# renegade-fi/mpc-jellyfish

Measured on AMD Instinct MI355X. Metric: msm_g1_scalar_pairs_per_s, higher is better.
Workload: dtype u32 (381-bit Fq as 14 x 29-bit limbs, Montgomery)

## Files before the change

### include/mzk.h

```cpp
#ifndef MZK_H
#define MZK_H

#include <stdint.h>

#ifdef __cplusplus
extern "C" {
#endif

#if defined(__GNUC__)
#define MZK_API __attribute__((visibility("default")))
#else
#define MZK_API
#endif

#define MZK_OK 0
#define MZK_ERR_INVALID_ARG (-1)
#define MZK_ERR_HIP (-2)
#define MZK_ERR_NO_DEVICE (-3)
#define MZK_ERR_BAD_HANDLE (-4)
#define MZK_ERR_UNSUPPORTED (-5)
#define MZK_ERR_OOM (-6)
#define MZK_ERR_NOT_INIT (-7)
#define MZK_ERR_LOOKUP (-8)

// ... 176 lines not shown
MZK_API int32_t mzk_plonk_perm_product_dev(uint64_t pk_handle, const void* d_wire_values, const uint64_t* beta_mont,
                                           const uint64_t* gamma_mont, void* d_out, void* stream);
MZK_API int32_t mzk_plonk_perm_product(uint64_t pk_handle, const uint64_t* wire_values, const uint64_t* beta_mont,
                                       const uint64_t* gamma_mont, uint64_t* out);

MZK_API int32_t mzk_plonk_gather_witness_dev(const void* d_witness, uint64_t n_vars, const void* d_wire_variables, uint64_t count, void* d_out,
                                             void* stream);

MZK_API int32_t mzk_poly_eval_dev(int32_t curve_id, const void* d_coeffs, uint64_t len, uint32_t batch, uint64_t batch_stride,
                                  const uint64_t* x_mont, uint64_t* out_mont, void* stream);
MZK_API int32_t mzk_poly_eval_many_dev(int32_t curve_id, uint32_t n_jobs, const void* const* d_coeffs, const uint64_t* lens, const uint32_t* batches,
                                       const uint64_t* strides, const uint32_t* which_x, const uint64_t* x_mont, uint64_t* out_mont, void* stream);
MZK_API int32_t mzk_poly_lincomb_dev(int32_t curve_id, uint32_t n_terms, const void* const* d_polys, const uint64_t* lens,
                                     const uint64_t* scalars_mont, void* d_out, uint64_t out_len, void* stream);
MZK_API int32_t mzk_poly_mask_dev(int32_t curve_id, uint32_t n_polys, void* const* d_polys, uint64_t n, uint32_t n_blinders,
                                  const uint64_t* blinders_mont, void* stream);
MZK_API int32_t mzk_poly_split_quotient_dev(int32_t curve_id, const void* d_quot, uint64_t n, uint32_t n_parts, const uint64_t* blinders_mont,
                                            void* d_out, uint64_t out_stride, void* stream);
MZK_API int32_t mzk_poly_div_linear_dev(int32_t curve_id, const void* d_poly, uint64_t len, const uint64_t* z_mont, void* d_out, void* stream);
MZK_API int32_t mzk_poly_div_linear_rem_dev(int32_t curve_id, const void* d_poly, uint64_t len, const uint64_t* z_mont, void* d_out, void* d_rem,
                                            void* stream);
MZK_API int32_t mzk_poly_degree_dev(const void* d_poly, uint64_t len, uint64_t* d_out_len, void* stream);
MZK_API int32_t mzk_poly_div_roots_dev(int32_t curve_id, const void* d_poly, uint64_t len, uint32_t log_order, uint64_t first, uint64_t count,
                                       void* d_out, void* stream);
MZK_API int32_t mzk_kzg_open_batch_dev(uint64_t srs_handle, uint32_t K, const void* const* d_polys, const uint64_t* lens, const uint64_t* points_mont,
                                       uint64_t* out_proofs_xy_mont, uint64_t* out_evals_mont, void* stream);
MZK_API int32_t mzk_kzg_multi_open_rou_dev(uint64_t srs_handle, uint64_t srs_offset, const void* d_poly, uint64_t len, uint32_t log_domain,
                                           uint64_t num_points, uint64_t* out_proofs_xy_mont, uint64_t* out_evals_mont, void* stream);

MZK_API int32_t mzk_sha256(const uint8_t* msg, uint64_t len, uint8_t* out32);
MZK_API int32_t mzk_expand_message_xmd_sha256(const uint8_t* msg, uint64_t len, const uint8_t* dst, uint64_t dst_len, uint32_t z_pad_len, uint8_t* out,
                                              uint64_t out_len);
MZK_API int32_t mzk_hash_to_field_sha256(int32_t curve_id, const uint8_t* msg, uint64_t len, const uint8_t* dst, uint64_t dst_len, uint64_t* out_mont);
MZK_API int32_t mzk_bytes_to_field_dev(int32_t curve_id, const void* d_bytes, uint64_t len, void* d_out_mont, void* stream);
MZK_API int32_t mzk_field_to_bytes_dev(int32_t curve_id, const void* d_elems_mont, uint64_t count, void* d_out_bytes, uint64_t* out_len, void* stream);
MZK_API int32_t mzk_vid_advz_commit_only_dev(uint64_t srs_handle, uint64_t srs_offset, uint64_t srs_len, const void* d_elems_mont, uint64_t n_elems,
                                             uint32_t payload_chunk_size, uint32_t num_storage_nodes, uint32_t log_domain, uint8_t* out_commit32, void* stream);
MZK_API int32_t mzk_vid_advz_disperse_dev(uint64_t srs_handle, uint64_t srs_offset, uint64_t srs_len, const void* d_elems_mont, uint64_t n_elems,
                                          uint32_t payload_chunk_size, uint32_t num_storage_nodes, uint32_t log_domain, uint64_t* out_commits_xy_mont,
                                          uint8_t* out_evals, uint64_t* out_proofs_xy_mont, uint8_t* out_nodes, uint8_t* out_commit32, uint8_t* out_root32,
                                          uint64_t* out_scalar_mont, void* stream);
MZK_API int32_t mzk_vid_advz_verify_shares_dev(int32_t curve_id, uint64_t n_shares, uint64_t evals_per_share, uint32_t num_storage_nodes, const uint64_t* indices,
                                               const uint8_t* evals, const uint8_t* paths, const uint8_t* root32, const uint64_t* scalar_mont, int32_t* out_ok,
                                               uint64_t* out_agg_evals_mont, void* stream);
MZK_API int32_t mzk_vid_advz_recover_dev(int32_t curve_id, uint32_t payload_chunk_size, uint64_t n_polys, uint32_t log_domain, const uint64_t* indices,
                                         const uint64_t* evals_mont, void* d_out_mont, void* stream);

#define MZK_ERR_WRONG_QUOTIENT_DEGREE (-9)
#define MZK_ERR_STATE (-10)
#define MZK_ERR_ENCODING (-11)

typedef struct mzk_comm {
    void* ctx;
    int32_t rank, world;
    int32_t (*all_gather)(void* ctx, const void* send, uint64_t bytes, void* recv);
    int32_t (*barrier)(void* ctx);
    int32_t (*exchange_classes)(void* ctx, void* d_rem, uint64_t class_bytes, uint32_t first_own, uint32_t n_own, uint32_t n_classes);
} mzk_comm;

MZK_API int32_t mzk_prover_create(int32_t curve_id, uint32_t log_n, uint32_t num_wire_types, const uint64_t* selector_coeffs,
                                  const uint64_t* sigma_coeffs, const uint64_t* table_coeffs, uint64_t poly_len, const uint64_t* k_mont,
                                  uint64_t commit_key, uint64_t lagrange_key, const mzk_comm* comm, uint64_t* out_prover);
MZK_API int32_t mzk_prover_create_from_circuit(int32_t curve_id, uint32_t log_n, uint32_t num_wire_types, const uint64_t* selector_values,
                                               const uint32_t* wire_variables, uint64_t n_vars, const uint64_t* table_values, const uint64_t* k_mont,
                                               uint64_t commit_key, uint64_t lagrange_key, const mzk_comm* comm, uint64_t* out_prover);
MZK_API int32_t mzk_prover_create_from_circuit_dev(int32_t curve_id, uint32_t log_n, uint32_t num_wire_types, const void* d_selector_values,
                                                   const void* d_wire_variables, uint64_t n_vars, const void* d_table_values, const uint64_t* k_mont,
                                                   uint64_t commit_key, uint64_t lagrange_key, const mzk_comm* comm, uint64_t* out_prover);
MZK_API int32_t mzk_prover_create_serialized(int32_t curve_id, const uint8_t* bytes, uint64_t len, uint32_t flags, uint64_t commit_key, const mzk_comm* comm,
                                             uint64_t* out_prover, uint64_t* out_commit_key, uint64_t* out_lagrange_key, uint64_t* out_bad);
MZK_API int32_t mzk_prover_serialize_key(uint64_t prover, uint32_t flags, uint64_t num_inputs, const uint8_t* h_bytes, const uint8_t* beta_h_bytes,
                                         int32_t is_merged, uint8_t* out_bytes, uint64_t capacity, uint64_t* out_len);
MZK_API int32_t mzk_prover_serialize_vk(uint64_t prover, uint32_t flags, uint64_t num_inputs, const uint8_t* h_bytes, const uint8_t* beta_h_bytes,
                                        int32_t is_merged, uint8_t* out_bytes, uint64_t capacity, uint64_t* out_len);
MZK_API int32_t mzk_prover_destroy(uint64_t prover);
MZK_API int32_t mzk_prover_fork(uint64_t prover, uint64_t* out_prover);
MZK_API int32_t mzk_prover_vk_commitments(uint64_t prover, uint64_t* out_xy_mont, uint64_t* out_plookup_xy_mont);
MZK_API int32_t mzk_prover_set_wire_variables(uint64_t prover, const uint32_t* wire_variables, uint64_t n_vars);
MZK_API int32_t mzk_prover_derive_wire_variables(uint64_t prover, uint64_t* out_n_vars);
MZK_API int32_t mzk_prover_get_wire_variables(uint64_t prover, uint32_t* out_wire_variables, uint64_t capacity_cells, uint64_t* out_n_vars);
#define MZK_WITNESS_DEV_WIRES 0
#define MZK_WITNESS_HOST_WIRES 1
#define MZK_WITNESS_HOST_VECTOR 2
#define MZK_WITNESS_DEV_VECTOR 3
MZK_API int32_t mzk_prover_round1(uint64_t prover, int32_t witness_kind, const void* witness, uint64_t witness_len, const uint64_t* pub_input_rows,
                                  const uint64_t* pub_input_mont, uint64_t n_pub, const uint64_t* blinders_mont, uint64_t* out_comms_xy);
#define MZK_CHECK_SATISFIED 0
#define MZK_CHECK_GATE 1
#define MZK_CHECK_LOOKUP 2
#define MZK_CHECK_COPY 3
typedef struct mzk_witness_report {
    uint32_t kind;
    uint32_t copy_checked;
    uint64_t gate_failures, gate_row;
    uint64_t lookup_failures, lookup_row;
    uint64_t copy_failures, copy_cell, copy_rep_cell;
    uint64_t row_wires[6 * 4];
    uint64_t gate_residual[4];
} mzk_witness_report;
MZK_API int32_t mzk_prover_check_witness(uint64_t prover, int32_t witness_kind, const void* witness, uint64_t witness_len,
                                         const uint64_t* pub_input_rows, const uint64_t* pub_input_mont, uint64_t n_pub,
                                         mzk_witness_report* out_report);
MZK_API int32_t mzk_prover_round1_5(uint64_t prover, const uint64_t* tau_mont, const uint64_t* blinders_mont, uint64_t* out_comms_xy);
MZK_API int32_t mzk_prover_round2(uint64_t prover, const uint64_t* beta_mont, const uint64_t* gamma_mont, const uint64_t* blinders_mont,
                                  uint64_t* out_comm_xy);
MZK_API int32_t mzk_prover_round2_5(uint64_t prover, const uint64_t* blinders_mont, uint64_t* out_comm_xy);
MZK_API int32_t mzk_prover_round3(const uint64_t* provers, uint32_t n_instances, const uint64_t* alpha_mont, const uint64_t* blinders_mont,
                                  uint64_t* out_comms_xy);
MZK_API int32_t mzk_prover_round4(uint64_t prover, const uint64_t* zeta_mont, uint64_t* out_evals_mont);
MZK_API int32_t mzk_prover_round5(const uint64_t* provers, uint32_t n_instances, const uint64_t* v_mont, uint64_t* out_comms_xy);
MZK_API int32_t mzk_prover_exchange_buffer(uint64_t prover, void** out_dptr, uint64_t* out_bytes);
MZK_API int32_t mzk_prover_set_peer_buffers(uint64_t prover, void* const* peer_dptrs, const int32_t* peer_devices);
MZK_API int32_t mzk_prover_poly_dev(uint64_t prover, uint32_t which, const void** out_dptr, uint64_t* out_len);
MZK_API int32_t mzk_prover_profile(uint64_t prover, int32_t on);
MZK_API int32_t mzk_prover_timings(uint64_t prover, char* buf, uint64_t cap);
MZK_API int32_t mzk_prover_hbm_bytes(uint64_t prover, uint64_t* out_fixed, uint64_t* out_proving_key, uint64_t* out_workspace);
MZK_API int32_t mzk_prover_shared_hbm_bytes(uint64_t prover, uint64_t* out_shared_bytes, uint32_t* out_sharers);

MZK_API int32_t mzk_host_alloc(uint64_t bytes, void** out_ptr);
MZK_API int32_t mzk_host_free(void* ptr);
MZK_API int32_t mzk_host_register(void* ptr, uint64_t bytes);
MZK_API int32_t mzk_host_unregister(void* ptr);

MZK_API int32_t mzk_dev_alloc(uint64_t bytes, void** out_dptr);
MZK_API int32_t mzk_dev_free(void* dptr);
MZK_API int32_t mzk_dev_upload(void* dptr, const void* host, uint64_t bytes);
MZK_API int32_t mzk_dev_download(void* host, const void* dptr, uint64_t bytes);
MZK_API int32_t mzk_dev_sync(void);
MZK_API int32_t mzk_stream_create(void** out_stream);
MZK_API int32_t mzk_stream_destroy(void* stream);
MZK_API int32_t mzk_stream_sync(void* stream);
MZK_API int32_t mzk_stream_wait_stream(void* waiter, void* signaller);
MZK_API int32_t mzk_dev_upload_async(void* dptr, const void* host, uint64_t bytes, void* stream);
MZK_API int32_t mzk_dev_download_async(void* host, const void* dptr, uint64_t bytes, void* stream);
MZK_API int32_t mzk_dev_copy(void* dst, const void* src, uint64_t bytes, void* stream);
MZK_API int32_t mzk_dev_copy_peer(void* dst, int32_t dst_device, const void* src, int32_t src_device, uint64_t bytes, void* stream);
MZK_API int32_t mzk_dev_copy2d(void* dst, uint64_t dst_pitch, const void* src, uint64_t src_pitch, uint64_t width, uint64_t height, void* stream);
MZK_API int32_t mzk_dev_memset(void* dptr, int32_t value, uint64_t bytes, void* stream);
MZK_API int32_t mzk_dev_memset2d(void* dptr, uint64_t pitch, int32_t value, uint64_t width, uint64_t height, void* stream);

MZK_API int32_t mzk_profile_enable(int32_t on);
MZK_API int32_t mzk_profile_get(const char* name, double* out_ms, uint64_t* out_count);
MZK_API int32_t mzk_profile_reset(void);
MZK_API int32_t mzk_msm_set_precompute(int32_t on);
MZK_API int32_t mzk_srs_precompute(uint64_t srs_handle, uint32_t* out_window_bits, uint32_t* out_levels, uint64_t* out_table_bytes,
                                   double* out_build_ms);
MZK_API int32_t mzk_srs_hbm_bytes(uint64_t srs_handle, uint64_t* out_points_bytes, uint64_t* out_table_bytes);
MZK_API int32_t mzk_plonk_pk_hbm_bytes(uint64_t pk_handle, uint64_t* out_bytes);
MZK_API int32_t mzk_workspace_hbm_bytes(uint64_t* out_bytes);
MZK_API int32_t mzk_workspace_release(void);
MZK_API int32_t mzk_launch_count(uint64_t* out_launches);
MZK_API int32_t mzk_msm_last_shape(uint32_t* out_window_bits, uint32_t* out_windows, uint32_t* out_buckets);
MZK_API int32_t mzk_msm_last_rare(uint32_t* out_cap, uint32_t* out_desc_cap, uint32_t* out_h1_cap, uint32_t* out_attempts);

#ifdef __cplusplus
}
#endif
#endif
```

### mpc-jellyfish_amd/csrc/internal.hpp

```cpp
#pragma once
#include <cstdlib>
#include <hip/hip_runtime.h>

#include <atomic>
#include <condition_variable>
#include <cstdint>
#include <cstring>
#include <map>
#include <mutex>
#include <string>
#include <vector>

#include "../../include/mzk.h"

extern "C" int32_t mzk_ctx_prover_stream(uint32_t k, void** out_stream);
namespace mzk { struct WitnessCheckIn; }
extern "C" int32_t mzk_ctx_pk_register_chunked(int32_t curve_id, uint32_t log_n, uint32_t num_wire_types, const void* selector_coeffs, const void* sigma_coeffs,
                                               const void* table_coeffs, uint64_t poly_len, const uint64_t* k_mont, const uint32_t* classes, uint32_t n_classes,
                                               int32_t coeffs_on_device, uint64_t* out_handle);
extern "C" int32_t mzk_ctx_check_witness(uint64_t pk_handle, const mzk::WitnessCheckIn* in, mzk_witness_report* out_report, void* stream);
extern "C" int32_t mzk_ctx_derive_variables(uint64_t pk_handle, const void* d_sigma_coeffs, void* d_out_variables_u32, uint64_t* out_n_vars, void* stream);
extern "C" int32_t mzk_ctx_g1_encode(int32_t curve_id, const uint64_t* xy_mont, uint64_t n_points, uint32_t flags, uint8_t* out_bytes);

namespace mzk {

void set_error(const std::string& s);

int32_t hip_status(hipError_t e, const char* what);

#define HIP_TRY(expr)                                      \
    do {                                                   \
        int32_t _r = ::mzk::hip_status((expr), #expr);     \
        if (_r != MZK_OK) return _r;                       \
    } while (0)

#define MZK_TRY(expr)                \
    do {                             \
        int32_t _r = (expr);         \
        if (_r != MZK_OK) return _r; \
    } while (0)

struct DevBuf {
    void* p = nullptr;
    size_t cap = 0;
    int32_t reserve(size_t bytes);
    void release();
    template <class T> T* as() { return reinterpret_cast<T*>(p); }
};
struct DevOwned {
    void* p = nullptr;
    DevOwned() = default;
    DevOwned(DevOwned&& o) noexcept : p(o.p) { o.p = nullptr; }
    DevOwned& operator=(DevOwned&&) = delete;
    ~DevOwned() { if (p) (void)hipFree(p); }
    int32_t alloc(size_t bytes) { return hip_status(hipMalloc(&p, bytes ? bytes : 4), "hipMalloc"); }
    template <class T> T* as() const { return reinterpret_cast<T*>(p); }
};

struct Workspace {
    DevBuf ntt_scratch, scalars, hist, offs, cursor, sorted, buckets, collect, io, misc, digits, long_desc, long_parts, plonk_polys, plonk_out, pre_cnt, pre_off, pre_ce, pre_cb, poly_tmp, split, link_tmp, occ, vid;
    void* h_collect = nullptr;
    size_t h_collect_cap = 0;
    double heavy_frac = 0.125;
    hipEvent_t last_use = nullptr;
    struct Named { const char* name; DevBuf Workspace::* buf; };
    static const Named bufs[];
    void release();
    size_t bytes();
};

extern std::atomic<uint64_t> g_launches;
#undef hipLaunchKernelGGL
#define hipLaunchKernelGGL(kernelName, ...)                                  \
    do {                                                                     \
        ::mzk::g_launches.fetch_add(1, std::memory_order_relaxed);           \
        hipLaunchKernelGGLInternal((kernelName), __VA_ARGS__);               \
    } while (0)

extern std::atomic<bool> g_prof;
struct ProfRec { std::string name; hipEvent_t a, b; };
struct ProfScope {
    hipEvent_t a = nullptr, b = nullptr;
    hipStream_t st;
    const char* name;
    int logical = -1;
    ProfScope(const char* n, hipStream_t s);
    ProfScope(const char* n, hipStream_t s, int logical_device);
    ~ProfScope();
};
extern std::atomic<bool> g_msm_precompute;

struct Srs {
    int curve = 0;
    uint64_t n = 0;
    uint32_t* d_xy = nullptr;
    uint32_t* d_int = nullptr;
    uint32_t* d_pre = nullptr;
    int pre_c = 0;
    int pre_levels = 0;
    double pre_build_ms = 0;
    uint32_t* d_fk = nullptr;
    uint64_t fk_off = 0, fk_d = 0;
    void free();
};
inline bool valid_curve(int curve) { return curve == MZK_CURVE_BLS12_381 || curve == MZK_CURVE_BN254; }
inline int fq_words(int curve) { return curve == MZK_CURVE_BLS12_381 ? 12 : 8; }
inline size_t srs_point_bytes(int curve) { return (size_t)2 * fq_words(curve) * 4; }
constexpr size_t srs_int_point_bytes(int curve) { return curve == MZK_CURVE_BLS12_381 ? 2 * 14 * 4 : 2 * 9 * 4; }
constexpr size_t ec_ntt_point_bytes(int curve) { return curve == MZK_CURVE_BLS12_381 ? 4 * 14 * 4 : 4 * 9 * 4; }

constexpr int MAX_CTX = 16;
constexpr int IO_SLOTS = 4;
struct IoSlot {
    hipStream_t st = nullptr;
    DevBuf buf;
    bool busy = false;
};
struct Ctx {
    int logical = -1, device = -1;
    std::atomic<bool> init{false};
    std::mutex lock;
    Workspace ws;
    std::vector<ProfRec> prof_recs;
    uint32_t last_c = 0, last_w = 0, last_m = 0;
    uint32_t last_cap = 0, last_desc_cap = 0, last_h1_cap = 0, last_attempts = 0;
    std::map<uint64_t, Srs> srs;
    uint64_t next_handle = 1;
    IoSlot io[IO_SLOTS];
    std::mutex io_lock;
    std::condition_variable io_cv;
};
Ctx& cur();
int32_t ws_acquire(Workspace& ws, hipStream_t st);
void ws_release(Workspace& ws, hipStream_t st);
class WsHold {
    Workspace* ws_ = nullptr;
    hipStream_t st_ = nullptr;
   public:
    WsHold() = default;
    WsHold(const WsHold&) = delete;
    WsHold& operator=(const WsHold&) = delete;
    ~WsHold() { if (ws_) ws_release(*ws_, st_); }
    int32_t acquire(hipStream_t st) {
        Ctx& cx = cur();
        MZK_TRY(ws_acquire(cx.ws, st));
        ws_ = &cx.ws, st_ = st;
        return MZK_OK;
    }
    Workspace* operator->() const { return ws_; }
    Workspace& operator*() const { return *ws_; }
};
inline uint64_t handle_make(int logical, uint64_t counter) { return ((uint64_t)(logical + 1) << 48) | counter; }
inline int handle_ctx(uint64_t h) { return (int)(h >> 48) - 1; }
struct DeviceGuard {
    int32_t prev = -1, rc = MZK_OK;
    bool switched = false;
    explicit DeviceGuard(int device) {
        if (mzk_get_device(&prev) != MZK_OK) prev = -1;
        if (prev != device) { rc = mzk_set_device(device); switched = rc == MZK_OK && prev >= 0; }
    }
    DeviceGuard(const DeviceGuard&) = delete;
    DeviceGuard& operator=(const DeviceGuard&) = delete;
    ~DeviceGuard() { if (switched) (void)mzk_set_device(prev); }
};

int32_t ntt_dispatch(int curve, uint32_t* d_data, uint64_t in_len, int log_n, bool inverse, const uint32_t* coset,
                     uint32_t batch, uint64_t stride, hipStream_t st, int scale = 0, const uint32_t* d_src = nullptr, uint64_t src_stride = 0,
                     const uint32_t* d_patch = nullptr, int skip_batch = -1 );
int32_t ntt_classes_dispatch(int curve, uint32_t* d_data, uint64_t in_len, int log_n, bool inverse, const uint32_t* const* cosets, int n_classes, uint32_t rows,
                             uint64_t stride, hipStream_t st, int scale, const uint32_t* d_src, uint64_t src_stride, const uint32_t* d_patch, int skip_batch);
void ntt_release_plans();
void msm_release_streams();
int32_t ctx_prover_stream(unsigned k, hipStream_t* out);
int32_t msm_dispatch(const Srs& s, uint64_t base_offset, const uint32_t* d_scalars, uint64_t n, int is_mont, uint32_t* out, hipStream_t st);
int32_t msm_batch_dispatch(const Srs& s, uint32_t n_polys, const uint32_t* const* d_scalars, const uint64_t* lens, const uint64_t* base_offsets,
                           int is_mont, uint32_t* out_xyz, hipStream_t st);
int32_t srs_build_internal(Srs& s, hipStream_t st);
int32_t srs_build_pre(Srs& s, hipStream_t st);
int32_t srs_generate_dispatch(int curve, const uint32_t* beta_canon, const uint32_t* g_xy_mont , uint64_t n, uint32_t* d_out);
int32_t srs_lagrange_from_points_dispatch(int curve, const uint32_t* d_xy, int log_n, uint32_t n_extra, uint32_t* d_out);
int32_t ec_ntt_dispatch(int curve, uint32_t* d_a, int log_n, bool inverse, bool scaled, uint32_t* d_tab, uint32_t* d_out_xy, uint64_t n_out, hipStream_t st);
int32_t srs_lagrange_generate_dispatch(int curve, const uint32_t* beta_canon, const uint32_t* g_xy_mont , int log_n, uint32_t n_extra, uint32_t* d_out);
void jac_to_affine_host_dispatch(int curve, const uint64_t* xyz, uint64_t n, uint64_t* xy);
void jac_sum_host_dispatch(int curve, const uint64_t* xyz, uint64_t n, uint64_t* out);

uint64_t srs_record_bytes(int curve, bool compressed);
const char* srs_bad_reason(int k);
int32_t srs_decode_dispatch(int curve, const uint8_t* d_in, uint64_t n, bool compressed, bool validate, uint32_t* d_xy, uint64_t* out_bad, int* out_reason,
                            hipStream_t st);
int32_t srs_encode_dispatch(int curve, const uint32_t* d_xy, uint64_t n, bool compressed, uint8_t* d_out, hipStream_t st);

int32_t fr_decode_dispatch(int curve, const uint8_t* d_image, uint32_t n_seg, const uint64_t* src, const uint64_t* count, const uint32_t* row, uint32_t* d_out,
                           uint64_t row_len, uint32_t* out_bad_seg, uint64_t* out_bad_index, hipStream_t st);
int32_t fr_encode_dispatch(int curve, const uint32_t* d_in, uint64_t n, uint32_t* d_out, hipStream_t st);

int32_t poly_eval_dispatch(int curve, const uint32_t* d_coeffs, uint64_t stride, uint64_t len, uint32_t batch, const uint32_t* x_mont, uint32_t* out_host,
                           hipStream_t st);
struct EvalJob { const uint32_t* d; uint64_t len, stride; uint32_t batch, which_x; };
int32_t poly_eval_many_dispatch(int curve, const EvalJob* jobs, uint32_t n_jobs, const uint32_t* x_mont , uint32_t* out_host, hipStream_t st);
int32_t poly_div_dispatch(int curve, const uint32_t* d_poly, uint64_t len, const uint32_t* z_mont, uint32_t* d_out, uint32_t* d_rem , hipStream_t st);
int32_t kzg_open_batch_dispatch(const Srs& s, uint32_t K, const uint32_t* const* d_polys, const uint64_t* lens, const uint32_t* points_mont, uint64_t* out_xy,
                                uint32_t* out_evals, hipStream_t st);
int32_t poly_div_roots_dispatch(int curve, const uint32_t* d_poly, uint64_t len, uint32_t log_order, uint64_t first, uint64_t count, uint32_t* d_out,
                                hipStream_t st);
constexpr int KZG_MULTI_MAX_LOG = 21;
int32_t kzg_multi_open_dispatch(Srs& s, uint64_t srs_offset, const uint32_t* d_poly, uint64_t len, uint32_t log_domain, uint64_t num_points, uint64_t* out_xy,
                                uint32_t* out_evals, hipStream_t st);
uint64_t vid_field_count(uint64_t len);
int32_t vid_bytes_to_field_dispatch(int curve, const uint8_t* d_bytes, uint64_t len, uint32_t* d_out, hipStream_t st);
int32_t vid_field_to_bytes_dispatch(int curve, const uint32_t* d_elems, uint64_t count, uint8_t* d_out, uint64_t* out_len, hipStream_t st);
int32_t vid_commit_only_dispatch(Srs& s, uint64_t srs_offset, uint64_t srs_len, const uint32_t* d_elems, uint64_t n_elems, uint32_t k, uint32_t n, uint32_t log_domain,
                                 uint8_t* out_commit, hipStream_t st);
int32_t vid_disperse_dispatch(Srs& s, uint64_t srs_offset, uint64_t srs_len, const uint32_t* d_elems, uint64_t n_elems, uint32_t k, uint32_t n, uint32_t log_domain,
                              uint64_t* out_commits_xy, uint8_t* out_evals, uint64_t* out_proofs_xy, uint8_t* out_nodes, uint8_t* out_commit, uint8_t* out_root,
                              uint64_t* out_s_mont, hipStream_t st);
int32_t vid_verify_shares_dispatch(int curve, uint64_t S, uint64_t K, uint32_t n, const uint64_t* index, const uint8_t* evals, const uint8_t* paths, const uint8_t* root,
                                   const uint64_t* s_mont, int32_t* out_ok, uint64_t* out_agg_mont, hipStream_t st);
int32_t vid_recover_dispatch(int curve, uint32_t k, uint64_t K, uint32_t log_domain, const uint64_t* index, const uint64_t* y_mont, uint32_t* d_out, hipStream_t st);
int32_t poly_lincomb_dispatch(int curve, uint32_t n_terms, const uint32_t* const* d_polys, const uint64_t* lens, const uint32_t* scalars, uint32_t* d_out,
                              uint64_t out_len, hipStream_t st);
int32_t poly_degree_dispatch(const uint32_t* d_poly, uint64_t len, unsigned long long* d_out, hipStream_t st);
int32_t wire_gather_dispatch(const uint32_t* d_witness, uint64_t n_vars, const uint32_t* d_vars, uint64_t count, uint32_t* d_out, hipStream_t st);
int32_t poly_split_quotient_dispatch(int curve, const uint32_t* d_q, uint64_t n, uint32_t W, const uint32_t* blind_mont, uint32_t* d_out, uint64_t stride, hipStream_t st);
int32_t poly_mask_dispatch(int curve, uint32_t n_rows, uint32_t* const* d_rows, uint64_t n, uint32_t n_blind, const uint32_t* blind_mont, hipStream_t st);
int32_t plonk_pk_register(int curve, int log_n, int W, const uint32_t* sel, const uint32_t* sig, const uint32_t* tab ,
                          uint64_t poly_len, const uint32_t* k_mont, const uint32_t* classes , uint32_t n_classes,
                          uint64_t* out_handle, bool coeffs_on_device = false );
int32_t plonk_wire_permutation_dev(const uint32_t* d_vars, uint64_t cells, uint64_t n_vars, uint32_t* d_next, hipStream_t st);
int32_t plonk_sigma_values_dev(int curve, int log_n, int W, const uint32_t* d_next, const uint32_t* k_mont, uint32_t* d_out, hipStream_t st);
int32_t plonk_sigma_decode_dev(int curve, int log_n, int W, const uint32_t* d_sigma, const uint32_t* k_mont, uint32_t* d_next, hipStream_t st);
int32_t plonk_variables_from_permutation_dev(const uint32_t* d_next, uint64_t cells, uint32_t* d_vars, uint64_t* out_n_vars, hipStream_t st);
int32_t plonk_derive_variables_dev(uint64_t handle, const uint32_t* d_sigma_coeffs, uint32_t* d_vars, uint64_t* out_n_vars, hipStream_t st);
int32_t plonk_quotient_chunked_dev(uint64_t handle, const uint32_t* d_polys, uint64_t in_stride, uint64_t in_len, uint32_t flags, const uint32_t* tau,
                                   const uint32_t* alpha, const uint32_t* beta, const uint32_t* gamma, uint32_t* d_out, hipStream_t st);
int32_t plonk_quotient_top_dev(uint64_t handle, const uint32_t* d_polys, uint64_t in_stride, uint64_t in_len, const uint32_t* alpha, const uint32_t* beta,
                               const uint32_t* gamma, uint32_t* d_top, uint32_t* out_n_top, hipStream_t st);
int32_t plonk_quotient_combine_dev(int curve, int log_n, const uint32_t* classes , uint32_t n_classes, const uint32_t* d_r,
                                   const uint32_t* d_top , uint32_t n_top, uint32_t* d_out, hipStream_t st);
int32_t plonk_pk_release(uint64_t handle);
void plonk_release_all();
void verifier_release_all();
int32_t plonk_quotient_dev(uint64_t handle, uint32_t* d_polys, uint64_t in_len, const uint32_t* tau , const uint32_t* alpha,
                           const uint32_t* beta, const uint32_t* gamma, uint32_t* d_out, hipStream_t st);
int32_t plookup_sorted_vec_dev(uint64_t handle, const uint32_t* d_wires, const uint32_t* tau, uint32_t* d_table, uint32_t* d_lookup, uint32_t* d_sorted,
                               hipStream_t st);
int32_t plookup_product_dev(uint64_t handle, const uint32_t* d_table, const uint32_t* d_lookup, const uint32_t* d_sorted, const uint32_t* beta,
                            const uint32_t* gamma, uint32_t* d_out, hipStream_t st);
struct WitnessCheckIn {
    const uint32_t* d_sel_coeffs;
    int kind;
    const void* witness;
    const uint32_t* d_vars;
    uint64_t n_vars;
    const uint64_t *pi_rows, *pi;
    uint64_t n_pi;
};
int32_t plonk_check_witness_dev(uint64_t handle, const WitnessCheckIn& in, mzk_witness_report* out, hipStream_t st);
int plonk_pk_is_ultra(uint64_t handle);
int32_t plonk_perm_product_dev(uint64_t handle, const uint32_t* d_wires, const uint32_t* beta, const uint32_t* gamma, uint32_t* d_out, hipStream_t st);
int plonk_pk_log_n(uint64_t handle);
int plonk_pk_curve(uint64_t handle);
int plonk_pk_classes(uint64_t handle, uint32_t* out);
int plonk_pk_wires(uint64_t handle);
uint64_t plonk_pk_bytes(uint64_t handle);

}
```

### mpc-jellyfish_amd/csrc/msm.cuh

```cuda
#pragma once
#include <hip/hip_runtime.h>

#include "ec.cuh"
#include "ecx.cuh"
#include "ecz.cuh"
#include "ec_ntt.cuh"

namespace mzk {

constexpr int MSM_THREADS = 256;
constexpr int MSM_ACC_THREADS = 128;
constexpr uint32_t MSM_HEAVY_PER_THREAD = 16;
constexpr uint32_t MSM_HEAVY_RUN = MSM_ACC_THREADS * MSM_HEAVY_PER_THREAD;
constexpr uint32_t MSM_HEAVY_FANIN = MSM_ACC_THREADS * 32;
constexpr int MSM_HEAVY_COUNTERS = 6;
__host__ __device__ inline bool msm_is_heavy(uint32_t count, uint32_t cap) { return count > cap + MSM_HEAVY_RUN; }

inline int msm_choose_window(unsigned long long n) {
    int lg = 0;
    while ((1ull << (lg + 1)) <= n) lg++;
    int c = lg - 2;
    if (c < 4) c = 4;
    if (c > 16) c = 16;
    return c;
}
inline int msm_num_windows(int scalar_bits, int c) { return (scalar_bits + 1 + c - 1) / c; }

struct DigitIter {
    uint32_t k[8];
    uint32_t carry;
    __device__ __forceinline__ void next(int w, int c, uint32_t& mag, uint32_t& negative) {
        const int off = w * c, word = off >> 5, bit = off & 31;
        uint32_t buf = 0;
        if (word < 8) {
            uint64_t two = k[word];
            if (word + 1 < 8) two |= (uint64_t)k[word + 1] << 32;
            buf = (uint32_t)(two >> bit);
        }
        uint32_t coef = (buf & ((1u << c) - 1)) + carry;
        carry = coef > (1u << (c - 1)) ? 1u : 0u;
        negative = carry;
        mag = carry ? (1u << c) - coef : coef;
    }
};

template <class FR>
__device__ __forceinline__ void load_scalar(DigitIter& it, const uint32_t* __restrict__ scalars, unsigned long long i, int is_mont) {
    Fp<FR> s = load_fp<FR>(scalars + i * 8);
    if (is_mont) s = from_mont(s);
#pragma unroll
    for (int q = 0; q < 8; q++) it.k[q] = s.l[q];
    it.carry = 0;
}

constexpr uint32_t MSM_EMPTY = 0xFFFFu;
constexpr int MSM_RANGE_LOG = 11;
constexpr int MSM_SORT_THREADS = 1024;

template <class FR>
__global__ __launch_bounds__(MSM_THREADS) void msm_digits_kernel(const uint32_t* __restrict__ scalars, unsigned long long n, int is_mont,
                                                                  int c, int n_win, uint16_t* __restrict__ digits, unsigned long long stride) {
    const unsigned long long i = (unsigned long long)blockIdx.x * MSM_THREADS + threadIdx.x;
    if (i >= n) return;
    DigitIter it;
    load_scalar<FR>(it, scalars, i, is_mont);
    for (int w = 0; w < n_win; w++) {
        uint32_t mag, ng;
        it.next(w, c, mag, ng);
        digits[(size_t)w * stride + i] = (uint16_t)(mag ? ((ng << 15) | (mag - 1)) : MSM_EMPTY);
    }
}

template <bool SCATTER>
__global__ __launch_bounds__(MSM_SORT_THREADS) void msm_sort_kernel(const uint16_t* __restrict__ digits, unsigned long long n, unsigned long long stride, uint32_t M,
                                                                     uint32_t* __restrict__ hist, const uint32_t* __restrict__ offs,
                                                                     uint32_t* __restrict__ sorted) {
    __shared__ uint32_t bins[1 << MSM_RANGE_LOG];
    const uint32_t range = blockIdx.x, w = blockIdx.y, tid = threadIdx.x;
    const uint32_t rsize = M < (1u << MSM_RANGE_LOG) ? M : (1u << MSM_RANGE_LOG);
    const uint32_t rbase = range * rsize;
    for (uint32_t j = tid; j < rsize; j += MSM_SORT_THREADS) bins[j] = SCATTER ? offs[(size_t)w * M + rbase + j] : 0u;
    __syncthreads();
    const uint16_t* dw = digits + (size_t)w * stride;
    uint32_t* out = sorted + (size_t)w * n;
    const unsigned long long n8 = n >> 3;
    for (unsigned long long q = tid; q < n8; q += MSM_SORT_THREADS) {
        const uint4 v = reinterpret_cast<const uint4*>(dw)[q];
        const uint32_t wd[4] = {v.x, v.y, v.z, v.w};
#pragma unroll
        for (int k = 0; k < 8; k++) {
            const uint32_t d = (wd[k >> 1] >> ((k & 1) * 16)) & 0xFFFFu;
            const uint32_t b = d & 0x7FFFu;
            if (d != MSM_EMPTY && b - rbase < rsize) {
                if (SCATTER) out[atomicAdd(&bins[b - rbase], 1u)] = (uint32_t)(q * 8 + k) | ((d >> 15) << 31);
                else atomicAdd(&bins[b - rbase], 1u);
            }
        }
    }
    for (unsigned long long i = (n8 << 3) + tid; i < n; i += MSM_SORT_THREADS) {
        const uint32_t d = dw[i], b = d & 0x7FFFu;
        if (d != MSM_EMPTY && b - rbase < rsize) {
            if (SCATTER) out[atomicAdd(&bins[b - rbase], 1u)] = (uint32_t)i | ((d >> 15) << 31);
            else atomicAdd(&bins[b - rbase], 1u);
        }
    }
    if (!SCATTER) {
        __syncthreads();
        for (uint32_t j = tid; j < rsize; j += MSM_SORT_THREADS) hist[(size_t)w * M + rbase + j] = bins[j];
    }
}

__global__ __launch_bounds__(1024) void msm_scan_kernel(const uint32_t* __restrict__ hist, uint32_t* __restrict__ offs, uint32_t M) {
    __shared__ uint32_t part[1024];
    const int w = blockIdx.x, t = threadIdx.x;
    const uint32_t per = (M + 1023) / 1024;
    const uint32_t lo = t * per, hi = min(M, lo + per);
    uint32_t sum = 0;
    for (uint32_t b = lo; b < hi; b++) sum += hist[(size_t)w * M + b];
    part[t] = sum;
    __syncthreads();
    for (int d = 1; d < 1024; d <<= 1) {
        uint32_t v = t >= d ? part[t - d] : 0;
        __syncthreads();
        part[t] += v;
        __syncthreads();
    }
    uint32_t run = part[t] - sum;
    for (uint32_t b = lo; b < hi; b++) {
        offs[(size_t)w * M + b] = run;
        run += hist[(size_t)w * M + b];
    }
}

constexpr uint32_t MSM_ORDER_SLICE = 8192;
__device__ __forceinline__ uint32_t order_key(uint32_t count) { return 1023u - min(count, 1023u); }

__global__ __launch_bounds__(1024) void msm_order_hist_kernel(const uint32_t* __restrict__ hist, uint32_t M, uint32_t* __restrict__ keycnt) {
    __shared__ uint32_t cnt[1024];
    const uint32_t w = blockIdx.y, t = threadIdx.x;
    const uint32_t lo = blockIdx.x * MSM_ORDER_SLICE, hi = min(M, lo + MSM_ORDER_SLICE);
    cnt[t] = 0;
    __syncthreads();
    for (uint32_t b = lo + t; b < hi; b += 1024) atomicAdd(&cnt[order_key(hist[(size_t)w * M + b])], 1u);
    __syncthreads();
    if (cnt[t]) atomicAdd(&keycnt[(size_t)w * 1024 + t], cnt[t]);
}
__global__ __launch_bounds__(1024) void msm_order_scan_kernel(uint32_t* __restrict__ keycnt, uint32_t global_sets) {
    __shared__ uint32_t part[1024];
    const uint32_t w = blockIdx.x, t = threadIdx.x;
    uint32_t mine = keycnt[(size_t)w * 1024 + t];
    for (uint32_t s = 1; s < global_sets; s++) mine += keycnt[(size_t)s * 1024 + t];
    part[t] = mine;
    __syncthreads();
    for (int d = 1; d < 1024; d <<= 1) {
        uint32_t v = t >= (uint32_t)d ? part[t - d] : 0;
        __syncthreads();
        part[t] += v;
        __syncthreads();
    }
    keycnt[(size_t)w * 1024 + t] = part[t] - mine;
}
__global__ __launch_bounds__(1024) void msm_order_scatter_kernel(const uint32_t* __restrict__ hist, uint32_t M, uint32_t* __restrict__ keycur,
                                                                 uint32_t* __restrict__ order, bool global) {
    __shared__ uint32_t cnt[1024];
    const uint32_t w = blockIdx.y, t = threadIdx.x;
    const uint32_t row = global ? 0u : w;
    const uint32_t lo = blockIdx.x * MSM_ORDER_SLICE, hi = min(M, lo + MSM_ORDER_SLICE);
    cnt[t] = 0;
    __syncthreads();
    for (uint32_t b = lo + t; b < hi; b += 1024) atomicAdd(&cnt[order_key(hist[(size_t)w * M + b])], 1u);
    __syncthreads();
    const uint32_t mine = cnt[t];
    __syncthreads();
    cnt[t] = mine ? atomicAdd(&keycur[(size_t)row * 1024 + t], mine) : 0u;
    __syncthreads();
    for (uint32_t b = lo + t; b < hi; b += 1024) {
        const uint32_t pos = atomicAdd(&cnt[order_key(hist[(size_t)w * M + b])], 1u);
        order[(size_t)row * M + pos] = w * M + b;
    }
}

struct LongDesc;
struct HeavyRun;
__device__ __forceinline__ void msm_long_register(uint32_t w, uint32_t b, uint32_t c, uint32_t offs_t, int n_win, uint32_t cap, uint32_t desc_cap,
                                                  LongDesc* __restrict__ desc, uint32_t* __restrict__ desc_count, uint32_t run_cap,
                                                  uint32_t h1_cap, HeavyRun* __restrict__ heavy_runs);
__global__ __launch_bounds__(1024) void msm_order_place_kernel(const uint32_t* __restrict__ hist, const uint32_t* __restrict__ offs, uint32_t M,
                                                               const uint32_t* __restrict__ keycnt, uint32_t* __restrict__ keycur, uint32_t* __restrict__ order,
                                                               int n_win, uint32_t cap, uint32_t desc_cap, LongDesc* __restrict__ desc,
                                                               uint32_t* __restrict__ desc_count, uint32_t run_cap, uint32_t h1_cap, HeavyRun* __restrict__ heavy_runs,
                                                               bool global) {
    __shared__ uint32_t cnt[1024];
    __shared__ uint32_t part[1024];
    const uint32_t w = blockIdx.y, t = threadIdx.x;
    const uint32_t row = global ? 0u : w;
    const uint32_t lo = blockIdx.x * MSM_ORDER_SLICE, hi = min(M, lo + MSM_ORDER_SLICE);
    uint32_t total = 0;
    if (global) for (uint32_t s = 0; s < gridDim.y; s++) total += keycnt[(size_t)s * 1024 + t];
    else total = keycnt[(size_t)w * 1024 + t];
    part[t] = total;
    cnt[t] = 0;
    __syncthreads();
    for (int d = 1; d < 1024; d <<= 1) {
        uint32_t v = t >= (uint32_t)d ? part[t - d] : 0;
        __syncthreads();
        part[t] += v;
        __syncthreads();
    }
    const uint32_t key_start = part[t] - total;
    for (uint32_t b = lo + t; b < hi; b += 1024) atomicAdd(&cnt[order_key(hist[(size_t)w * M + b])], 1u);
    __syncthreads();
    const uint32_t mine = cnt[t];
    __syncthreads();
    cnt[t] = mine ? key_start + atomicAdd(&keycur[(size_t)row * 1024 + t], mine) : 0u;
    __syncthreads();
    for (uint32_t b = lo + t; b < hi; b += 1024) {
        const uint32_t c = hist[(size_t)w * M + b];
        const uint32_t pos = atomicAdd(&cnt[order_key(c)], 1u);
        order[(size_t)row * M + pos] = w * M + b;
        if (desc_count && c > cap) msm_long_register(w, b, c, offs[(size_t)w * M + b], n_win, cap, desc_cap, desc, desc_count, run_cap, h1_cap, heavy_runs);
    }
}

template <class FQ>
__device__ __forceinline__ Affine<Fp<FQ>> load_affine(const uint32_t* __restrict__ bases, unsigned long long idx) {
    Affine<Fp<FQ>> p;
    const uint32_t* src = bases + idx * (2 * FQ::N);
    p.x = load_fp<FQ>(src);
    p.y = load_fp<FQ>(src + FQ::N);
    return p;
}
template <class FQ>
__device__ __forceinline__ XYZZ<Fp<FQ>> load_xyzz(const uint32_t* __restrict__ buf, unsigned long long idx) {
    XYZZ<Fp<FQ>> p;
    const uint32_t* src = buf + idx * (4 * FQ::N);
    p.x = load_fp<FQ>(src);
    p.y = load_fp<FQ>(src + FQ::N);
    p.zz = load_fp<FQ>(src + 2 * FQ::N);
    p.zzz = load_fp<FQ>(src + 3 * FQ::N);
    return p;
}
template <class FQ>
__device__ __forceinline__ void store_xyzz(uint32_t* __restrict__ buf, unsigned long long idx, const XYZZ<Fp<FQ>>& p) {
    uint32_t* dst = buf + idx * (4 * FQ::N);
    store_fp<FQ>(dst, p.x);
    store_fp<FQ>(dst + FQ::N, p.y);
    store_fp<FQ>(dst + 2 * FQ::N, p.zz);
    store_fp<FQ>(dst + 3 * FQ::N, p.zzz);
}

template <class FQ>
struct EcFp {
    using Field = FQ;
    using Aff = Affine<Fp<FQ>>;
    using Pt = XYZZ<Fp<FQ>>;
    static constexpr int AFF_WORDS = 2 * FQ::N, PT_WORDS = 4 * FQ::N;
    static __device__ __forceinline__ Aff load_aff(const uint32_t* __restrict__ bases, unsigned long long idx) { return load_affine<FQ>(bases, idx); }
    static __device__ __forceinline__ Pt load_pt(const uint32_t* __restrict__ buf, unsigned long long idx) { return load_xyzz<FQ>(buf, idx); }
    static __device__ __forceinline__ void store_pt(uint32_t* __restrict__ buf, unsigned long long idx, const Pt& p) { store_xyzz<FQ>(buf, idx, p); }
    static __device__ __forceinline__ Pt inf() { return Pt::inf(); }
    static __device__ __forceinline__ Pt madd(const Pt& a, Aff q, bool negate) {
        if (negate) q.y = neg(q.y);
        return xyzz_madd(a, q);
    }
    static __device__ __forceinline__ Pt add(const Pt& a, const Pt& b) { return xyzz_add(a, b); }
    static __device__ __forceinline__ XYZZ<Fp<FQ>> to_boundary(const Pt& p) { return p; }
};

template <class X>
__device__ __forceinline__ void load_words(uint32_t* dst, const uint32_t* __restrict__ src, int n_words) {
    for (int i = 0; i < n_words / 4; i++) {
        const uint4 v = reinterpret_cast<const uint4*>(src)[i];
        dst[4 * i] = v.x; dst[4 * i + 1] = v.y; dst[4 * i + 2] = v.z; dst[4 * i + 3] = v.w;
    }
}

template <class Z>
struct EcFz {
    using Field = Z;
    using Aff = AffineZ<Z>;
    using Pt = XYZZZ<Z>;
    using Fe = Fz<Z>;
    static constexpr int LIMBS = Z::ZN, SLOT_WORDS = Z::ZN + 1;
    static constexpr int AFF_WORDS = 2 * SLOT_WORDS, PT_WORDS = 4 * SLOT_WORDS;
    static_assert(AFF_WORDS % 4 == 0, "points are whole 16-byte words");
    static __device__ __forceinline__ Aff load_aff(const uint32_t* __restrict__ bases, unsigned long long idx) {
        uint32_t w[AFF_WORDS];
        const uint4* src = reinterpret_cast<const uint4*>(bases + idx * AFF_WORDS);
#pragma unroll
        for (int i = 0; i < AFF_WORDS / 4; i++) {
            const uint4 v = src[i];
            w[4 * i] = v.x; w[4 * i + 1] = v.y; w[4 * i + 2] = v.z; w[4 * i + 3] = v.w;
        }
        Aff p;
#pragma unroll
        for (int i = 0; i < LIMBS; i++) { p.x.l[i] = (int32_t)w[i]; p.y.l[i] = (int32_t)w[SLOT_WORDS + i]; }
        return p;
    }
    static __device__ __forceinline__ void store_aff(uint32_t* __restrict__ bases, unsigned long long idx, const Aff& p) {
        uint32_t w[AFF_WORDS];
#pragma unroll
        for (int i = 0; i < LIMBS; i++) { w[i] = (uint32_t)p.x.l[i]; w[SLOT_WORDS + i] = (uint32_t)p.y.l[i]; }
        w[LIMBS] = 0; w[SLOT_WORDS + LIMBS] = 0;
        uint4* dst = reinterpret_cast<uint4*>(bases + idx * AFF_WORDS);
#pragma unroll
        for (int i = 0; i < AFF_WORDS / 4; i++) dst[i] = make_uint4(w[4 * i], w[4 * i + 1], w[4 * i + 2], w[4 * i + 3]);
    }
    static __device__ __forceinline__ Pt load_pt(const uint32_t* __restrict__ buf, unsigned long long idx) {
        uint32_t w[PT_WORDS];
        const uint4* src = reinterpret_cast<const uint4*>(buf + idx * PT_WORDS);
#pragma unroll
        for (int i = 0; i < PT_WORDS / 4; i++) {
            const uint4 v = src[i];
            w[4 * i] = v.x; w[4 * i + 1] = v.y; w[4 * i + 2] = v.z; w[4 * i + 3] = v.w;
        }
        Pt p;
#pragma unroll
        for (int i = 0; i < LIMBS; i++) {
            p.x.l[i] = (int32_t)w[i]; p.y.l[i] = (int32_t)w[SLOT_WORDS + i];
            p.zz.l[i] = (int32_t)w[2 * SLOT_WORDS + i]; p.zzz.l[i] = (int32_t)w[3 * SLOT_WORDS + i];
        }
        return p;
    }
    static __device__ __forceinline__ void store_pt(uint32_t* __restrict__ buf, unsigned long long idx, const Pt& p) {
        uint32_t w[PT_WORDS];
#pragma unroll
        for (int i = 0; i < LIMBS; i++) {
            w[i] = (uint32_t)p.x.l[i]; w[SLOT_WORDS + i] = (uint32_t)p.y.l[i];
            w[2 * SLOT_WORDS + i] = (uint32_t)p.zz.l[i]; w[3 * SLOT_WORDS + i] = (uint32_t)p.zzz.l[i];
        }
#pragma unroll
        for (int k = 0; k < 4; k++) w[k * SLOT_WORDS + LIMBS] = 0;
        uint4* dst = reinterpret_cast<uint4*>(buf + idx * PT_WORDS);
#pragma unroll
        for (int i = 0; i < PT_WORDS / 4; i++) dst[i] = make_uint4(w[4 * i], w[4 * i + 1], w[4 * i + 2], w[4 * i + 3]);
    }
    static __device__ __forceinline__ Pt inf() { return Pt::inf(); }
    static __device__ __forceinline__ Pt madd(const Pt& a, const Aff& q, bool negate) { return xyzzz_madd(a, q, negate); }
    static __device__ __forceinline__ Pt add(const Pt& a, const Pt& b) { return xyzzz_add(a, b); }
    static __device__ __forceinline__ XYZZ<Fp<Z>> to_boundary(const Pt& p) { return xyzzz_to_boundary(p); }
    static __device__ __forceinline__ Fe add_quad(const Fe& ca, const Fe& cb, int role) { return xyzzz_add_quad<Z>(ca, cb, role); }
};

template <class Z>
__global__ __launch_bounds__(MSM_THREADS) void srs_to_internal_z_kernel(const uint32_t* __restrict__ xy, unsigned long long n, uint32_t* __restrict__ out) {
    const unsigned long long i = (unsigned long long)blockIdx.x * MSM_THREADS + threadIdx.x;
    if (i >= n) return;
    const Fp<Z> x = load_fp<Z>(xy + i * 2 * Z::N), y = load_fp<Z>(xy + i * 2 * Z::N + Z::N);
    AffineZ<Z> p;
    p.x = fz_from_boundary<Z>(x);
    p.y = fz_from_boundary<Z>(y);
    EcFz<Z>::store_aff(out, i, p);
}

template <class X>
__global__ __launch_bounds__(MSM_THREADS) void srs_to_internal_kernel(const uint32_t* __restrict__ xy, unsigned long long n, uint32_t* __restrict__ out) {
    const unsigned long long i = (unsigned long long)blockIdx.x * MSM_THREADS + threadIdx.x;
    if (i >= n) return;
    const Fp<X> x = load_fp<X>(xy + i * 2 * X::N), y = load_fp<X>(xy + i * 2 * X::N + X::N);
    const Fx<X> fx = fx_from_boundary<X>(x), fy = fx_from_boundary<X>(y);
    uint32_t* dst = out + i * 2 * X::XN;
#pragma unroll
    for (int k = 0; k < X::XN; k++) { dst[k] = fx.l[k]; dst[X::XN + k] = fy.l[k]; }
}

template <class EC>
__global__ __launch_bounds__(MSM_ACC_THREADS) void msm_accumulate_kernel(const uint32_t* __restrict__ bases, unsigned long long n,
                                                                          const uint32_t* __restrict__ offs, const uint32_t* __restrict__ hist,
                                                                          const uint32_t* __restrict__ sorted, const uint32_t* __restrict__ order,
                                                                          uint32_t M, int n_win, uint32_t cap, uint32_t* __restrict__ long_count,
                                                                          uint32_t* __restrict__ buckets, uint8_t* __restrict__ occ) {
    if (long_count && blockIdx.x == 0)
        for (unsigned i = threadIdx.x; i < (unsigned)n_win * (1 + MSM_HEAVY_COUNTERS); i += MSM_ACC_THREADS) long_count[i] = 0u;
    const unsigned long long t0 = (unsigned long long)blockIdx.x * MSM_ACC_THREADS + threadIdx.x;
    if (t0 >= (unsigned long long)n_win * M) return;
    const uint32_t tb = order[t0];
    const unsigned long long t = tb, w = tb / M;
    const uint32_t start = offs[t];
    const uint32_t h = hist[t];
    const uint32_t cnt = msm_is_heavy(h, cap) ? 0u : min(h, cap);
    const uint32_t* list = sorted + w * n + start;
    typename EC::Pt acc = EC::inf();
    for (uint32_t k = 0; k < cnt; k++) {
        const uint32_t e = list[k];
        acc = EC::madd(acc, EC::load_aff(bases, e & 0x7fffffffu), (e >> 31) != 0);
    }
    const bool empty = acc.is_inf();
    occ[t] = empty ? 0 : 1;
    if (!empty) EC::store_pt(buckets, t, acc);
}

template <class EC, bool ONE_SET>
__global__ __launch_bounds__(MSM_ACC_THREADS) void msm_accumulate_split_kernel(const uint32_t* __restrict__ bases, unsigned long long n,
                                                                                const uint32_t* __restrict__ offs, const uint32_t* __restrict__ hist,
                                                                                const uint32_t* __restrict__ sorted, const uint32_t* __restrict__ order,
                                                                                uint32_t M, int n_win, uint32_t cap, int log_split, uint32_t* __restrict__ long_count,
                                                                                uint32_t* __restrict__ sub, unsigned long long rank0,
                                                                                uint32_t* __restrict__ buckets, uint8_t* __restrict__ occ) {
    if (long_count && blockIdx.x == 0)
        for (unsigned i = threadIdx.x; i < (unsigned)n_win * (1 + MSM_HEAVY_COUNTERS); i += MSM_ACC_THREADS) long_count[i] = 0u;
    const unsigned long long t1 = (unsigned long long)blockIdx.x * MSM_ACC_THREADS + threadIdx.x;
    const bool whole = t1 < rank0;
    const unsigned long long u = whole ? 0ull : t1 - rank0;
    const unsigned long long t0 = whole ? t1 : rank0 + (u >> log_split);
    if (t0 >= (unsigned long long)n_win * M) return;
    const uint32_t S = whole ? 1u : 1u << log_split, part = whole ? 0u : (uint32_t)(u & (S - 1));
    const uint32_t tb = order[t0];
    const unsigned long long t = tb, w = ONE_SET ? 0ull : tb / M;
    const uint32_t start = offs[t];
    const uint32_t h = hist[t];
    const uint32_t cnt = msm_is_heavy(h, cap) ? 0u : min(h, cap);
    const uint32_t* list = sorted + w * n + start;
    typename EC::Pt acc = EC::inf();
    for (uint32_t k = part; k < cnt; k += S) {
        const uint32_t e = list[k];
        acc = EC::madd(acc, EC::load_aff(bases, e & 0x7fffffffu), (e >> 31) != 0);
    }
    if (whole) {
        const bool empty = acc.is_inf();
        occ[t] = empty ? 0 : 1;
        if (!empty) EC::store_pt(buckets, t, acc);
    } else {
        EC::store_pt(sub, u, acc);
    }
}
template <class EC>
__device__ __forceinline__ void pt_lds_put(uint32_t* lds, int slot, const typename EC::Pt& p) {
    constexpr int N = EC::LIMBS;
#pragma unroll
    for (int i = 0; i < N; i++) {
        lds[i * MSM_ACC_THREADS + slot] = p.x.l[i];
        lds[(N + i) * MSM_ACC_THREADS + slot] = p.y.l[i];
        lds[(2 * N + i) * MSM_ACC_THREADS + slot] = p.zz.l[i];
        lds[(3 * N + i) * MSM_ACC_THREADS + slot] = p.zzz.l[i];
    }
}
template <class EC>
__device__ __forceinline__ typename EC::Pt pt_lds_get(const uint32_t* lds, int slot) {
    constexpr int N = EC::LIMBS;
    typename EC::Pt p;
#pragma unroll
    for (int i = 0; i < N; i++) {
        p.x.l[i] = lds[i * MSM_ACC_THREADS + slot];
        p.y.l[i] = lds[(N + i) * MSM_ACC_THREADS + slot];
        p.zz.l[i] = lds[(2 * N + i) * MSM_ACC_THREADS + slot];
        p.zzz.l[i] = lds[(3 * N + i) * MSM_ACC_THREADS + slot];
    }
    return p;
}
template <class EC, bool ONE_SET>
__global__ __launch_bounds__(MSM_ACC_THREADS) void msm_split_combine_kernel(const uint32_t* __restrict__ sub, unsigned long long n_buckets, int log_split,
                                                                             const uint32_t* __restrict__ order, unsigned long long rank0,
                                                                             uint32_t* __restrict__ buckets, uint8_t* __restrict__ occ) {
    __shared__ uint32_t lds[MSM_ACC_THREADS * EC::PT_WORDS];
    const int tid = threadIdx.x;
    const unsigned long long total = n_buckets << log_split;
    const unsigned long long base = (unsigned long long)blockIdx.x * (2 * MSM_ACC_THREADS);
    typename EC::Pt acc = EC::inf();
#pragma unroll 1
    for (int lvl = 0; lvl < log_split; lvl++) {
        const bool mine = tid < (MSM_ACC_THREADS >> lvl) && base + ((unsigned long long)(2 * tid) << lvl) < total;
        typename EC::Pt a = EC::inf(), b = EC::inf();
        if (lvl == 0) {
            if (mine) { a = EC::load_pt(sub, base + 2ull * tid); b = EC::load_pt(sub, base + 2ull * tid + 1); }
        } else {
            __syncthreads();
            if (mine) { a = pt_lds_get<EC>(lds, 2 * tid); b = pt_lds_get<EC>(lds, 2 * tid + 1); }
            __syncthreads();
        }
        if (mine) {
            acc = EC::add(a, b);
            if (lvl == log_split - 1) {
                const unsigned long long t = order[rank0 + (base >> log_split) + tid];
                const bool empty = acc.is_inf();
                occ[t] = empty ? 0 : 1;
                if (!empty) EC::store_pt(buckets, t, acc);
            } else pt_lds_put<EC>(lds, tid, acc);
        }
    }
}

struct LongDesc { uint32_t bucket, start, len, idx_in_run, run_len; };

struct HeavyRun { uint32_t src, n, dest, p1; };
constexpr uint32_t MSM_HEAVY_DEST_PART = 0x80000000u;
constexpr int MSM_HEAVY_JOBS = 8;
struct HeavyJob {
    const uint32_t* bases;
    const uint32_t* sorted;
    unsigned long long n;
    const HeavyRun* runs;
    const uint32_t* count;
    uint32_t *h1, *h2, *h3, *buckets;
    uint8_t* occ;
    uint32_t run_cap, h1_cap, M;
    const LongDesc* desc;
    const uint32_t* desc_count;
    uint32_t* parts;
    uint32_t desc_cap;
};
struct HeavyJobs { HeavyJob j[MSM_HEAVY_JOBS]; };
__device__ __forceinline__ void msm_heavy_push(uint32_t b, uint32_t start, uint32_t rem, uint32_t run_cap, uint32_t h1_cap, uint32_t* __restrict__ cnt,
                                               HeavyRun* __restrict__ runs0, HeavyRun* __restrict__ runsB, HeavyRun* __restrict__ runsC) {
    const uint32_t n1 = (rem + MSM_HEAVY_RUN - 1) / MSM_HEAVY_RUN;
    const uint32_t need = (rem + MSM_HEAVY_PER_THREAD - 1) / MSM_HEAVY_PER_THREAD + n1;
    const uint32_t p1 = atomicAdd(&cnt[5], need);
    if (p1 + need > h1_cap) return;
    const uint32_t r0 = atomicAdd(&cnt[0], n1);
    if (r0 + n1 > run_cap) return;
    constexpr uint32_t PER_RUN = MSM_HEAVY_RUN / MSM_HEAVY_PER_THREAD;
    const uint32_t p2 = atomicAdd(&cnt[3], n1);
    for (uint32_t i = 0; i < n1; i++)
        runs0[r0 + i] = HeavyRun{start + i * MSM_HEAVY_RUN, min(MSM_HEAVY_RUN, rem - i * MSM_HEAVY_RUN), MSM_HEAVY_DEST_PART | (p2 + i), p1 + i * PER_RUN};
    const uint32_t n2 = (n1 + MSM_HEAVY_FANIN - 1) / MSM_HEAVY_FANIN;
    const uint32_t rb = atomicAdd(&cnt[1], n2);
    if (n2 == 1) { runsB[rb] = HeavyRun{p2, n1, b, 0}; return; }
    const uint32_t p3 = atomicAdd(&cnt[4], n2);
    for (uint32_t j = 0; j < n2; j++)
        runsB[rb + j] = HeavyRun{p2 + j * MSM_HEAVY_FANIN, min(MSM_HEAVY_FANIN, n1 - j * MSM_HEAVY_FANIN), MSM_HEAVY_DEST_PART | (p3 + j), 0};
    runsC[atomicAdd(&cnt[2], 1u)] = HeavyRun{p3, n2, b, 0};
}

__device__ __forceinline__ void msm_long_register(uint32_t w, uint32_t b, uint32_t c, uint32_t offs_t, int n_win, uint32_t cap, uint32_t desc_cap,
                                                  LongDesc* __restrict__ desc, uint32_t* __restrict__ desc_count, uint32_t run_cap,
                                                  uint32_t h1_cap, HeavyRun* __restrict__ heavy_runs);

__global__ __launch_bounds__(256) void msm_long_find_kernel(const uint32_t* __restrict__ hist, const uint32_t* __restrict__ offs, uint32_t M, int n_win,
                                                            uint32_t cap, uint32_t desc_cap, LongDesc* __restrict__ desc,
                                                            uint32_t* __restrict__ desc_count, uint32_t run_cap, uint32_t h1_cap, HeavyRun* __restrict__ heavy_runs) {
    const unsigned long long t = (unsigned long long)blockIdx.x * 256 + threadIdx.x;
    if (t >= (unsigned long long)n_win * M) return;
    const uint32_t c = hist[t];
    if (c <= cap) return;
    msm_long_register((uint32_t)(t / M), (uint32_t)(t % M), c, offs[t], n_win, cap, desc_cap, desc, desc_count, run_cap, h1_cap, heavy_runs);
}
__device__ __forceinline__ void msm_long_register(uint32_t w, uint32_t b, uint32_t c, uint32_t offs_t, int n_win, uint32_t cap, uint32_t desc_cap,
                                                  LongDesc* __restrict__ desc, uint32_t* __restrict__ desc_count, uint32_t run_cap,
                                                  uint32_t h1_cap, HeavyRun* __restrict__ heavy_runs) {
    if (msm_is_heavy(c, cap)) {
        HeavyRun* base = heavy_runs + (size_t)w * 3 * run_cap;
        msm_heavy_push(b, offs_t, c, run_cap, h1_cap, desc_count + n_win + (size_t)w * MSM_HEAVY_COUNTERS, base, base + run_cap, base + 2 * (size_t)run_cap);
        return;
    }
    const uint32_t nch = (c - cap + cap - 1) / cap;
    const uint32_t pos = atomicAdd(&desc_count[w], nch);
    if (pos + nch > desc_cap) {
        for (uint32_t i = pos; i < desc_cap; i++) desc[(size_t)w * desc_cap + i] = LongDesc{b, offs_t, 0u, 1u, 0u};
        return;
    }
    for (uint32_t j = 0; j < nch; j++) {
        LongDesc d;
        d.bucket = b;
        d.start = offs_t + cap * (j + 1);
        d.len = min(cap, c - cap * (j + 1));
        d.idx_in_run = j;
        d.run_len = nch;
        desc[(size_t)w * desc_cap + pos + j] = d;
    }
}

template <class EC>
__global__ __launch_bounds__(MSM_ACC_THREADS) void msm_long_chunk_kernel(const uint32_t* __restrict__ bases, unsigned long long n,
                                                                          const uint32_t* __restrict__ sorted, const LongDesc* __restrict__ desc,
                                                                          const uint32_t* __restrict__ desc_count, uint32_t desc_cap,
                                                                          uint32_t* __restrict__ parts) {
    const uint32_t w = blockIdx.y;
    const uint32_t i = blockIdx.x * MSM_ACC_THREADS + threadIdx.x;
    if (i >= min(desc_count[w], desc_cap)) return;
    const LongDesc d = desc[(size_t)w * desc_cap + i];
    const uint32_t* list = sorted + (size_t)w * n + d.start;
    typename EC::Pt acc = EC::inf();
    for (uint32_t k = 0; k < d.len; k++) {
        const uint32_t e = list[k];
        acc = EC::madd(acc, EC::load_aff(bases, e & 0x7fffffffu), (e >> 31) != 0);
    }
    EC::store_pt(parts, (size_t)w * desc_cap + i, acc);
}

template <class EC>
__global__ __launch_bounds__(MSM_ACC_THREADS) void msm_rare_leaf_kernel(HeavyJobs jobs, uint32_t long_blocks) {
    const HeavyJob& jb = jobs.j[blockIdx.z];
    const uint32_t w = blockIdx.y, t = threadIdx.x;
    const bool is_long = blockIdx.x < long_blocks;
    const uint32_t heavy_cnt = is_long ? 0u : min(jb.count[(size_t)w * MSM_HEAVY_COUNTERS], jb.run_cap);
    const HeavyRun* runs = jb.runs + (size_t)w * 3 * jb.run_cap;
    const uint32_t r_step = is_long ? 1u : gridDim.x - long_blocks;
    uint32_t r = is_long ? 0u : blockIdx.x - long_blocks;
    for (;; r += r_step) {
        const uint32_t* list;
        uint32_t cnt;
        uint32_t* out;
        size_t out_idx;
        if (is_long) {
            if (r) break;
            const uint32_t i = blockIdx.x * MSM_ACC_THREADS + t;
            if (i >= min(jb.desc_count[w], jb.desc_cap)) break;
            const LongDesc d = jb.desc[(size_t)w * jb.desc_cap + i];
            list = jb.sorted + (size_t)w * jb.n + d.start;
            cnt = d.len;
            out = jb.parts;
            out_idx = (size_t)w * jb.desc_cap + i;
        } else {
            if (r >= heavy_cnt) break;
            const HeavyRun run = runs[r];
            const uint32_t lo = t * MSM_HEAVY_PER_THREAD;
            if (lo >= run.n) continue;
            list = jb.sorted + (size_t)w * jb.n + run.src + lo;
            cnt = min(run.n, lo + MSM_HEAVY_PER_THREAD) - lo;
            out = jb.h1;
            out_idx = (size_t)w * jb.h1_cap + run.p1 + t;
        }
        typename EC::Pt acc = EC::inf();
        for (uint32_t k = 0; k < cnt; k++) {
            const uint32_t e = list[k];
            acc = EC::madd(acc, EC::load_aff(jb.bases, e & 0x7fffffffu), (e >> 31) != 0);
        }
        EC::store_pt(out, out_idx, acc);
    }
}

template <class EC>
__global__ __launch_bounds__(MSM_ACC_THREADS) void msm_long_combine_kernel(HeavyJobs jobs) {
    const HeavyJob& jb = jobs.j[blockIdx.z];
    const LongDesc* __restrict__ desc = jb.desc;
    const uint32_t* __restrict__ desc_count = jb.desc_count;
    const uint32_t desc_cap = jb.desc_cap, M = jb.M;
    const uint32_t* __restrict__ parts = jb.parts;
    uint32_t* __restrict__ buckets = jb.buckets;
    uint8_t* __restrict__ occ = jb.occ;
    const uint32_t w = blockIdx.y;
    const uint32_t cnt = min(desc_count[w], desc_cap);
    const LongDesc* dw = desc + (size_t)w * desc_cap;
    const size_t pbase = (size_t)w * desc_cap;
    for (uint32_t i = blockIdx.x * MSM_ACC_THREADS + threadIdx.x; i < cnt; i += gridDim.x * MSM_ACC_THREADS) {
        const LongDesc d = dw[i];
        if (d.idx_in_run != 0) continue;
        const size_t bi = (size_t)w * M + d.bucket;
        typename EC::Pt acc = occ[bi] ? EC::load_pt(buckets, bi) : EC::inf();
        for (uint32_t j = 0; j < d.run_len; j++) acc = EC::add(acc, EC::load_pt(parts, pbase + i + j));
        const bool empty = acc.is_inf();
        occ[bi] = empty ? 0 : 1;
        if (!empty) EC::store_pt(buckets, bi, acc);
    }
}

template <class EC>
__global__ __launch_bounds__(MSM_ACC_THREADS) void msm_heavy_chunk_kernel(HeavyJobs jobs) {
    const HeavyJob& jb = jobs.j[blockIdx.z];
    const uint32_t w = blockIdx.y, t = threadIdx.x, run_cap = jb.run_cap;
    const uint32_t cnt = min(jb.count[(size_t)w * MSM_HEAVY_COUNTERS], run_cap);
    const HeavyRun* runs = jb.runs + (size_t)w * 3 * run_cap;
    for (uint32_t r = blockIdx.x; r < cnt; r += gridDim.x) {
        const HeavyRun run = runs[r];
        const uint32_t lo = t * MSM_HEAVY_PER_THREAD;
        if (lo >= run.n) continue;
        const uint32_t hi = min(run.n, lo + MSM_HEAVY_PER_THREAD);
        const uint32_t* list = jb.sorted + (size_t)w * jb.n + run.src;
        typename EC::Pt acc = EC::inf();
        for (uint32_t k = lo; k < hi; k++) {
            const uint32_t e = list[k];
            acc = EC::madd(acc, EC::load_aff(jb.bases, e & 0x7fffffffu), (e >> 31) != 0);
        }
        EC::store_pt(jb.h1, (size_t)w * jb.h1_cap + run.p1 + t, acc);
    }
}
template <class EC>
__global__ __launch_bounds__(MSM_ACC_THREADS) void msm_heavy_reduce_kernel(HeavyJobs jobs, int level ) {
    __shared__ uint32_t lds[MSM_ACC_THREADS * EC::PT_WORDS];
    const HeavyJob& jb = jobs.j[blockIdx.z];
    const uint32_t w = blockIdx.y, run_cap = jb.run_cap, M = jb.M;
    const int tid = threadIdx.x;
    const uint32_t* parts_in = level == 0 ? jb.h1 : (level == 1 ? jb.h2 : jb.h3);
    uint32_t* parts_out = level == 0 ? jb.h2 : jb.h3;
    uint32_t* buckets = jb.buckets;
    uint8_t* occ = jb.occ;
    const uint32_t cnt = min(jb.count[(size_t)w * MSM_HEAVY_COUNTERS + level], run_cap);
    const HeavyRun* runs = jb.runs + ((size_t)w * 3 + level) * run_cap;
    const size_t in_base = (size_t)w * (level == 0 ? jb.h1_cap : run_cap), out_base = (size_t)w * run_cap;
    for (uint32_t r = blockIdx.x; r < cnt; r += gridDim.x) {
        const HeavyRun run = runs[r];
        const uint32_t n_items = level == 0 ? (run.n + MSM_HEAVY_PER_THREAD - 1) / MSM_HEAVY_PER_THREAD : run.n;
        const size_t src = in_base + (level == 0 ? (size_t)run.p1 : (size_t)run.src);
        const int per = (int)((n_items + MSM_ACC_THREADS - 1) / MSM_ACC_THREADS);
        int log_w = 0;
        while ((1u << log_w) < n_items && log_w < 7) log_w++;
        typename EC::Pt acc = (uint32_t)tid < n_items ? EC::load_pt(parts_in, src + tid) : EC::inf();
        const bool to_bucket = !(run.dest & MSM_HEAVY_DEST_PART);
        const size_t bi = (size_t)w * M + run.dest;
        const int n_steps = (per - 1) + log_w;
#pragma unroll 1
        for (int s = 0; s < n_steps; s++) {
            typename EC::Pt a = EC::inf(), b = EC::inf();
            bool act = false;
            if (s < per - 1) {
                const uint32_t q = (uint32_t)tid + (uint32_t)(s + 1) * MSM_ACC_THREADS;
                if (q < n_items) { a = acc; b = EC::load_pt(parts_in, src + q); act = true; }
            } else {
                const int l = s - (per - 1);
                __syncthreads();
                if (tid < ((1 << log_w) >> l)) pt_lds_put<EC>(lds, tid, acc);
                __syncthreads();
                if (tid < ((1 << log_w) >> (l + 1))) { a = pt_lds_get<EC>(lds, 2 * tid); b = pt_lds_get<EC>(lds, 2 * tid + 1); act = true; }
            }
            if (act) acc = EC::add(a, b);
        }
        if (tid == 0) {
            if (to_bucket) {
                const bool empty = acc.is_inf();
                occ[bi] = empty ? 0 : 1;
                if (!empty) EC::store_pt(buckets, bi, acc);
            } else {
                EC::store_pt(parts_out, out_base + (run.dest & ~MSM_HEAVY_DEST_PART), acc);
            }
        }
    }
}

template <class EC>
__device__ __forceinline__ void fold_one(uint32_t* __restrict__ buckets, uint8_t* __restrict__ occ, unsigned long long ia, unsigned long long ib) {
    if (!occ[ib]) return;
    typename EC::Pt b = EC::load_pt(buckets, ib);
    if (!occ[ia]) {
        EC::store_pt(buckets, ia, b);
        occ[ia] = 1;
        return;
    }
    typename EC::Pt a = EC::load_pt(buckets, ia);
    EC::store_pt(buckets, ia, EC::add(a, b));
}
template <class EC>
__global__ __launch_bounds__(MSM_ACC_THREADS) void msm_fold_kernel(uint32_t* __restrict__ buckets, uint8_t* __restrict__ occ, uint32_t M, uint32_t h, int nseg, int n_win) {
    const unsigned long long t = (unsigned long long)blockIdx.x * MSM_ACC_THREADS + threadIdx.x;
    const unsigned long long per_win = (unsigned long long)nseg * h;
    if (t >= per_win * n_win) return;
    const unsigned long long w = t / per_win, r = t % per_win;
    const uint32_t seg = (uint32_t)(r / h), i = (uint32_t)(r % h);
    const unsigned long long base = w * M + (seg ? (M >> seg) : 0u);
    fold_one<EC>(buckets, occ, base + i, base + h + i);
}

template <class EC>
__global__ __launch_bounds__(MSM_ACC_THREADS) void msm_fold2_kernel(uint32_t* __restrict__ buckets, uint8_t* __restrict__ occ, uint32_t M, uint32_t h, int nseg, int n_win) {
    const uint32_t q = h >> 1;
    const unsigned long long t = (unsigned long long)blockIdx.x * MSM_ACC_THREADS + threadIdx.x;
    const unsigned long long per_win = (unsigned long long)nseg * q;
    if (t >= per_win * n_win) return;
    const unsigned long long w = t / per_win, r = t % per_win;
    const uint32_t seg = (uint32_t)(r / q), i = (uint32_t)(r % q);
    const unsigned long long base = w * M + (seg ? (M >> seg) : 0u);
#pragma unroll 1
    for (int step = 0; step < 4; step++) {
        if (step == 3 && seg) break;
        const unsigned long long ia = base + (step == 1 ? q : (step == 3 ? h : 0u)) + i;
        const unsigned long long ib = step < 2 ? ia + h : ia + q;
        fold_one<EC>(buckets, occ, ia, ib);
    }
}
template <class EC>
__global__ __launch_bounds__(MSM_ACC_THREADS) void msm_fold2_quad_kernel(uint32_t* buckets, uint8_t* occ, uint32_t M, uint32_t h, int nseg, int n_win);

template <class EC>
__device__ __forceinline__ void collect_set(const uint32_t* buckets, const uint8_t* occ, uint32_t M, int log_m, unsigned long long w, uint32_t* out, int j) {
    const unsigned long long slot = w * M + (j ? (M >> j) : 0u);
    typename EC::Pt p = occ[slot] ? EC::load_pt(buckets, slot) : EC::inf();
    store_xyzz<typename EC::Field>(out, (size_t)w * (log_m + 1) + j, EC::to_boundary(p));
}
template <class EC>
__global__ __launch_bounds__(256) void msm_fold_tail_kernel(uint32_t* __restrict__ buckets, uint8_t* __restrict__ occ, uint32_t M, int log_m, int first_lvl,
                                                            uint32_t* __restrict__ collect) {
    const unsigned long long w = blockIdx.x;
    for (int lvl = first_lvl; lvl <= log_m; lvl++) {
        const uint32_t h = M >> lvl;
        const uint32_t items = (uint32_t)lvl * h;
        for (uint32_t r = threadIdx.x; r < items; r += 256) {
            const uint32_t seg = r / h, i = r % h;
            const unsigned long long base = w * M + (seg ? (M >> seg) : 0u);
            fold_one<EC>(buckets, occ, base + i, base + h + i);
        }
        __threadfence_block();
        __syncthreads();
    }
    if (collect && (int)threadIdx.x <= log_m) collect_set<EC>(buckets, occ, M, log_m, w, collect, (int)threadIdx.x);
}

template <class EC>
__device__ __forceinline__ void fold_one_quad(uint32_t* buckets, uint8_t* occ, unsigned long long ia, unsigned long long ib, int role) {
    using Fe = typename EC::Fe;
    constexpr int XN = EC::LIMBS, SLOT = EC::SLOT_WORDS;
    if (!occ[ib]) return;
    uint32_t* pa = buckets + ia * EC::PT_WORDS + role * SLOT;
    const uint32_t* pb = buckets + ib * EC::PT_WORDS + role * SLOT;
    Fe cb;
#pragma unroll
    for (int i = 0; i < XN; i++) cb.l[i] = pb[i];
    if (!occ[ia]) {
#pragma unroll
        for (int i = 0; i < XN; i++) pa[i] = cb.l[i];
        occ[ia] = 1;
        return;
    }
    Fe ca;
#pragma unroll
    for (int i = 0; i < XN; i++) ca.l[i] = pa[i];
    const Fe r = EC::add_quad(ca, cb, role);
#pragma unroll
    for (int i = 0; i < XN; i++) pa[i] = r.l[i];
}
template <class EC>
__global__ __launch_bounds__(MSM_ACC_THREADS) void msm_fold_quad_kernel(uint32_t* buckets, uint8_t* occ, uint32_t M, uint32_t h, int nseg, int n_win) {
    const unsigned long long t = ((unsigned long long)blockIdx.x * MSM_ACC_THREADS + threadIdx.x) >> 2;
    const int role = threadIdx.x & 3;
    const unsigned long long per_win = (unsigned long long)nseg * h;
    if (t >= per_win * n_win) return;
    const unsigned long long w = t / per_win, r = t % per_win;
    const uint32_t seg = (uint32_t)(r / h), i = (uint32_t)(r % h);
    const unsigned long long base = w * M + (seg ? (M >> seg) : 0u);
    fold_one_quad<EC>(buckets, occ, base + i, base + h + i, role);
}
constexpr int MSM_TAIL_QUAD_THREADS = 512;
template <class EC>
__global__ __launch_bounds__(MSM_TAIL_QUAD_THREADS) void msm_fold_tail_quad_kernel(uint32_t* buckets, uint8_t* occ, uint32_t M, int log_m, int first_lvl,
                                                                                    uint32_t* collect) {
    const unsigned long long w = blockIdx.x;
    const uint32_t quad = threadIdx.x >> 2;
    const int role = threadIdx.x & 3;
    for (int lvl = first_lvl; lvl <= log_m; lvl++) {
        const uint32_t h = M >> lvl;
        const uint32_t items = (uint32_t)lvl * h;
        for (uint32_t r = quad; r < items; r += MSM_TAIL_QUAD_THREADS / 4) {
            const uint32_t seg = r / h, i = r % h;
            const unsigned long long base = w * M + (seg ? (M >> seg) : 0u);
            fold_one_quad<EC>(buckets, occ, base + i, base + h + i, role);
        }
        __threadfence_block();
        __syncthreads();
    }
    if (collect && (int)threadIdx.x <= log_m) collect_set<EC>(buckets, occ, M, log_m, w, collect, (int)threadIdx.x);
}
template <class EC>
__global__ __launch_bounds__(MSM_ACC_THREADS) void msm_fold2_quad_kernel(uint32_t* buckets, uint8_t* occ, uint32_t M, uint32_t h, int nseg, int n_win) {
    const uint32_t q = h >> 1;
    const unsigned long long t = ((unsigned long long)blockIdx.x * MSM_ACC_THREADS + threadIdx.x) >> 2;
    const int role = threadIdx.x & 3;
    const unsigned long long per_win = (unsigned long long)nseg * q;
    if (t >= per_win * n_win) return;
    const unsigned long long w = t / per_win, r = t % per_win;
    const uint32_t seg = (uint32_t)(r / q), i = (uint32_t)(r % q);
    const unsigned long long base = w * M + (seg ? (M >> seg) : 0u);
#pragma unroll 1
    for (int step = 0; step < 4; step++) {
        if (step == 3 && seg) break;
        const unsigned long long ia = base + (step == 1 ? q : (step == 3 ? h : 0u)) + i;
        const unsigned long long ib = step < 2 ? ia + h : ia + q;
        fold_one_quad<EC>(buckets, occ, ia, ib, role);
    }
}

template <class EC>
__global__ void msm_collect_kernel(const uint32_t* __restrict__ buckets, const uint8_t* __restrict__ occ, uint32_t M, int log_m, int n_win, uint32_t* __restrict__ out) {
    const int t = blockIdx.x * blockDim.x + threadIdx.x;
    const int per = log_m + 1;
    if (t >= n_win * per) return;
    const int w = t / per, j = t % per;
    const unsigned long long slot = (unsigned long long)w * M + (j ? (M >> j) : 0u);
    typename EC::Pt p = occ[slot] ? EC::load_pt(buckets, slot) : EC::inf();
    store_xyzz<typename EC::Field>(out, t, EC::to_boundary(p));
}

template <class FQ>
__global__ void g1_pow2_table_kernel(uint32_t* __restrict__ table_xyzz, const uint32_t* __restrict__ g_xy = nullptr) {
    if (threadIdx.x != 0 || blockIdx.x != 0) return;
    using F = Fp<FQ>;
    Affine<F> g;
    if (g_xy) {
        g.x = load_fp<FQ>(g_xy);
        g.y = load_fp<FQ>(g_xy + FQ::N);
    } else {
        g.x = F::from_const(FQ::GEN_X);
        g.y = F::from_const(FQ::GEN_Y);
    }
    XYZZ<F> cur = XYZZ<F>::from_affine(g);
    for (int k = 0; k < 256; k++) {
        store_xyzz<FQ>(table_xyzz, k, cur);
        cur = xyzz_dbl(cur);
    }
}
template <class FQ>
__global__ void g1_table_to_affine_kernel(const uint32_t* __restrict__ table_xyzz, uint32_t* __restrict__ table_xy, int n) {
    const int k = blockIdx.x * blockDim.x + threadIdx.x;
    if (k >= n) return;
    Affine<Fp<FQ>> a = xyzz_to_affine(load_xyzz<FQ>(table_xyzz, k));
    store_fp<FQ>(table_xy + (size_t)k * 2 * FQ::N, a.x);
    store_fp<FQ>(table_xy + (size_t)k * 2 * FQ::N + FQ::N, a.y);
}
// ... 104 lines not shown
```

### mpc-jellyfish_amd/csrc/msm.hip

```cpp
#include <algorithm>
#include <chrono>
#include <thread>
#include <vector>

#include <cmath>
#include <cstdlib>

#include "internal.hpp"
#include "hostfp.hpp"
#include "host_tail.hpp"
#include "msm.cuh"
#include "msm_pre.cuh"

namespace mzk {
std::atomic<bool> g_msm_precompute{true};
namespace {

struct MsmItem {
    const uint32_t* d_bases;
    const uint32_t* d_scalars;
    uint64_t n;
    uint32_t* out_xyz;
    uint64_t base_off;
};
constexpr unsigned long long MSM_MIN_CAP = 48;
constexpr int32_t MSM_RETRY = 1;
struct PreInfo { int c = 0; uint64_t tab_stride = 0; };

constexpr int SORT_SETS = 6;
struct SortStreams {
    hipStream_t stream = nullptr;
    hipStream_t streams[4] = {};
    hipStream_t prover[2] = {};
    hipEvent_t ev_start = nullptr, ev_sorted[SORT_SETS] = {}, ev_acc[SORT_SETS] = {};
};
SortStreams g_sort[MAX_CTX];
inline int n_sort_streams() {
    static const int n = std::min(4, std::max(1, std::getenv("MZK_MSM_SORT_STREAMS") ? std::atoi(std::getenv("MZK_MSM_SORT_STREAMS")) : 2));
    return n;
}
int32_t sort_stream_init(SortStreams& ss) {
    if (ss.stream) return MZK_OK;
    int prio_least = 0, prio_greatest = 0;
    HIP_TRY(hipDeviceGetStreamPriorityRange(&prio_least, &prio_greatest));
    static const int rot = std::getenv("MZK_STREAM_ROT") ? std::atoi(std::getenv("MZK_STREAM_ROT")) : 1;
    for (int q = 0; q < (cur().logical * rot) % 4; q++) {
        hipStream_t pad = nullptr;
        HIP_TRY(hipStreamCreateWithFlags(&pad, hipStreamNonBlocking));
    }
    for (int q = 0; q < n_sort_streams(); q++)
        HIP_TRY(hipStreamCreateWithPriority(&ss.streams[q], hipStreamNonBlocking, std::getenv("MZK_MSM_SORT_PRIO_LOW") ? prio_least : prio_greatest));
    for (auto& q : ss.prover) HIP_TRY(hipStreamCreateWithFlags(&q, hipStreamNonBlocking));
    ss.stream = ss.streams[0];
    HIP_TRY(hipEventCreateWithFlags(&ss.ev_start, hipEventDisableTiming));
    for (int i = 0; i < SORT_SETS; i++) {
        HIP_TRY(hipEventCreateWithFlags(&ss.ev_sorted[i], hipEventDisableTiming));
        HIP_TRY(hipEventCreateWithFlags(&ss.ev_acc[i], hipEventDisableTiming));
    }
    return MZK_OK;
}

template <class FQ>
void write_infinity(uint32_t* out_xyz) {
    using F64 = Fp64<FQ>;
    F64 one = F64::one(), z = F64::zero();
    one.to_words(out_xyz); one.to_words(out_xyz + FQ::N); z.to_words(out_xyz + 2 * FQ::N);
}

template <class EC>
int32_t launch_rare(const HeavyJobs& jobs, unsigned n_jobs, int sets, uint32_t desc_cap, uint32_t run_cap, bool level_c, bool diet, hipStream_t st) {
    const uint32_t long_blocks = (desc_cap + MSM_ACC_THREADS - 1) / MSM_ACC_THREADS, heavy_blocks = std::min<uint32_t>(run_cap, 2048u);
    const dim3 hg(heavy_blocks, sets, n_jobs);
    if (diet) {
        hipLaunchKernelGGL((msm_rare_leaf_kernel<EC>), dim3(long_blocks + heavy_blocks, sets, n_jobs), dim3(MSM_ACC_THREADS), 0, st, jobs, long_blocks);
    } else {
        for (unsigned q = 0; q < n_jobs; q++) {
            const HeavyJob& jb = jobs.j[q];
            hipLaunchKernelGGL((msm_long_chunk_kernel<EC>), dim3((jb.desc_cap + MSM_ACC_THREADS - 1) / MSM_ACC_THREADS, sets), dim3(MSM_ACC_THREADS), 0, st,
                               jb.bases, jb.n, jb.sorted, jb.desc, jb.desc_count, jb.desc_cap, jb.parts);
        }
        hipLaunchKernelGGL((msm_heavy_chunk_kernel<EC>), hg, dim3(MSM_ACC_THREADS), 0, st, jobs);
    }
    hipLaunchKernelGGL((msm_long_combine_kernel<EC>), dim3(std::min<uint32_t>(long_blocks, 1024u), sets, n_jobs), dim3(MSM_ACC_THREADS), 0, st, jobs);
    hipLaunchKernelGGL((msm_heavy_reduce_kernel<EC>), hg, dim3(MSM_ACC_THREADS), 0, st, jobs, 0);
    hipLaunchKernelGGL((msm_heavy_reduce_kernel<EC>), hg, dim3(MSM_ACC_THREADS), 0, st, jobs, 1);
    if (level_c) hipLaunchKernelGGL((msm_heavy_reduce_kernel<EC>), dim3(64, sets, n_jobs), dim3(MSM_ACC_THREADS), 0, st, jobs, 2);
    HIP_TRY(hipGetLastError());
    return MZK_OK;
}

template <class FR, class EC>
int32_t msm_group_dev(const MsmItem* items, int count, int c, int is_mont, const PreInfo& pre, hipStream_t st) {
    using FQ = typename EC::Field;
    const uint32_t M = 1u << (c - 1);
    const int log_m = c - 1;
    const int n_dig = msm_num_windows(is_mont ? FR::BITS : 256, c);
    const int n_win = pre.c ? 1 : n_dig;
    cur().last_c = c; cur().last_w = n_dig; cur().last_m = M;
    uint64_t n_max = 0, n_min = ~0ull;
    for (int p = 0; p < count; p++) { n_max = std::max<uint64_t>(n_max, items[p].n); n_min = std::min<uint64_t>(n_min, items[p].n); }
    static const bool no_fuse = std::getenv("MZK_MSM_NO_FUSE") != nullptr;
    const int top_bits_all = (is_mont ? FR::BITS : 256) - c * (n_dig - 1);
    const bool fuse = pre.c && count > 1 && count <= PRE_FUSE_MAX && n_max <= (1ull << 17) && top_bits_all >= c - 1 && !no_fuse;
    const int sets = fuse ? count : n_win;
    const int passes = fuse ? 1 : count;
    const size_t wm = (size_t)sets * M;
    static const bool no_sort2 = std::getenv("MZK_MSM_PLAIN_SORT1") != nullptr;
    const bool sort2 = !pre.c && !no_sort2 && n_min >= (1ull << 16) && wm >= (1u << 14) && (wm >> PRE_FINE_LOG) <= 1024;
    const uint64_t sorted_max = pre.c ? n_max * n_dig : n_max;
    WsHold ws; MZK_TRY(ws.acquire(st));
    const bool overlap = passes > 1 && std::getenv("MZK_MSM_NO_OVERLAP") == nullptr;
    const size_t nb = overlap ? (size_t)std::min(passes, SORT_SETS) : 1;
    MZK_TRY(ws->hist.reserve(nb * wm * 4));
    MZK_TRY(ws->offs.reserve(nb * wm * 4));
    MZK_TRY(ws->cursor.reserve(nb * wm * 4));
    const uint32_t desc_cap_worst = (uint32_t)(sorted_max / MSM_MIN_CAP + 1);
    uint32_t desc_cap_max = desc_cap_worst;
    const uint32_t run_cap_max = (uint32_t)(2 * (sorted_max / MSM_HEAVY_RUN) + 2);
    auto h1_cap_of = [](uint64_t entries, uint32_t run_cap_, double frac) {
        const uint64_t worst = entries / MSM_HEAVY_PER_THREAD + 2 * (uint64_t)run_cap_ + 2;
        return (uint32_t)std::min<uint64_t>(worst, (uint64_t)((double)worst * frac) + 2 * (uint64_t)run_cap_ + 4096);
    };
    const uint32_t h1_cap_worst = h1_cap_of(sorted_max, run_cap_max, 1.0);
    uint32_t h1_cap_max = h1_cap_worst;
    const size_t heavy_runs_bytes = (size_t)sets * 3 * run_cap_max * sizeof(HeavyRun);
    bool defer_heavy = passes > 1 && (size_t)passes <= nb && passes <= MSM_HEAVY_JOBS;
    const double heavy_frac = defer_heavy ? ws->heavy_frac : 1.0;
    auto desc_cap_of = [](uint64_t entries, uint64_t cap_, double frac) {
        const uint64_t worst = entries / cap_ + 1;
        return (uint32_t)std::min<uint64_t>(worst, (uint64_t)((double)worst * frac) + 1024);
    };
    if (defer_heavy) { h1_cap_max = h1_cap_of(sorted_max, run_cap_max, heavy_frac); desc_cap_max = desc_cap_of(sorted_max, MSM_MIN_CAP, heavy_frac); }
    size_t desc_slot_bytes = (((size_t)sets * desc_cap_max * sizeof(LongDesc) + (size_t)sets * 4 * (1 + MSM_HEAVY_COUNTERS) + 16 + heavy_runs_bytes) + 255) & ~(size_t)255;
    size_t parts_slot_words = (size_t)sets * desc_cap_max * EC::PT_WORDS + (size_t)sets * ((size_t)h1_cap_max + 2 * (size_t)run_cap_max) * EC::PT_WORDS;
    if (defer_heavy && (size_t)passes * parts_slot_words * 4 > ws->long_parts.cap) {
        size_t free_b = 0, total_b = 0;
        HIP_TRY(hipMemGetInfo(&free_b, &total_b));
        if ((size_t)passes * parts_slot_words * 4 > free_b / 4) {
            defer_heavy = false;
            h1_cap_max = h1_cap_worst;
            desc_cap_max = desc_cap_worst;
            desc_slot_bytes = (((size_t)sets * desc_cap_max * sizeof(LongDesc) + (size_t)sets * 4 * (1 + MSM_HEAVY_COUNTERS) + 16 + heavy_runs_bytes) + 255) & ~(size_t)255;
            parts_slot_words = (size_t)sets * desc_cap_max * EC::PT_WORDS + (size_t)sets * ((size_t)h1_cap_max + 2 * (size_t)run_cap_max) * EC::PT_WORDS;
        }
    }
    const double h1_frac = defer_heavy ? heavy_frac : 1.0;
    const size_t slots = defer_heavy ? (size_t)passes : 1;
    MZK_TRY(ws->long_desc.reserve(slots * desc_slot_bytes));
    MZK_TRY(ws->long_parts.reserve(slots * parts_slot_words * 4));
    const unsigned long long dstride_max = (n_max + 7) & ~7ull;
    const size_t fused_k = fuse ? (size_t)count : 1;
    const size_t digits_bytes = fused_k * n_dig * dstride_max * ((pre.c || sort2) ? 4 : 2), sorted_words = (fused_k * n_dig * n_max + 3) & ~(size_t)3;
    MZK_TRY(ws->digits.reserve(nb * digits_bytes));
    MZK_TRY(ws->sorted.reserve(nb * sorted_words * 4));
    PreBins pb{0, PRE_FINE_LOG, 0, PRE_FINE_LOG};
    if (pre.c && n_dig > 1) {
        const int top_bits = (is_mont ? FR::BITS : 256) - c * (n_dig - 1);
        if (top_bits >= PRE_FINE_LOG && top_bits < c - 1) {
            const double rho = 1.0 + (double)M / ((double)(1ull << top_bits) * (n_dig - 1));
            int shrink = (int)std::lround(std::log2(rho));
            if (shrink > 3) shrink = 3;
            if (shrink > 0) { pb.low = 1u << top_bits; pb.low_log = PRE_FINE_LOG - shrink; pb.low_bins = pb.low >> pb.low_log; }
        }
    }
    if ((pre.c || sort2) && pb.low == 0 && (wm >> PRE_FINE_LOG) < 128) {
        int lg = 0;
        while ((2ull << lg) <= wm) lg++;
        const int L = std::max(5, lg - 8);
        if (L < PRE_FINE_LOG && (wm >> L) >= 2 && (wm >> L) <= 1024 && wm % (1ull << L) == 0) { pb.low = (uint32_t)wm; pb.low_log = (uint32_t)L; pb.low_bins = (uint32_t)(wm >> L); }
    }
    if (pre.c || sort2) {
        const uint64_t rec_max = n_max * (uint64_t)n_dig * (fuse ? (uint64_t)count : 1);
        static const uint64_t per_bin = std::getenv("MZK_PRE_BIN_RECORDS") ? std::strtoull(std::getenv("MZK_PRE_BIN_RECORDS"), nullptr, 10) : 32768;
        while (rec_max / std::max<uint32_t>(1u, pb.count((uint32_t)wm)) > per_bin) {
            PreBins t = pb;
            if (t.low) {
                if (t.low_log <= 5) break;
                t.low_log--; t.low_bins = t.low >> t.low_log;
            }
            if (t.low != (uint32_t)wm) {
                if (t.hi_log <= 5) break;
                t.hi_log--;
            }
            if (t.count((uint32_t)wm) > 1024) break;
            pb = t;
        }
    }
    const uint32_t n_bins = (pre.c || sort2) ? std::max<uint32_t>(1u, pb.count((uint32_t)wm)) : 0u;
    static const bool legacy_launches = std::getenv("MZK_MSM_LEGACY_LAUNCHES") != nullptr;
    const bool diet = (pre.c || sort2) && !legacy_launches;
    static const bool rank_per_set = std::getenv("MZK_MSM_RANK_PER_SET") != nullptr;
    const bool rank_global = sets > 1 && !rank_per_set;
    const size_t cnt_words = 2048 + (size_t)sets * 1024 * (diet ? 2 : 1);
    const bool find_in_sort = diet && (!overlap || defer_heavy);
    MZK_TRY(ws->pre_cnt.reserve(nb * cnt_words * 4));
    if (pre.c || sort2) {
        MZK_TRY(ws->pre_off.reserve(nb * 8192 * 4));
        MZK_TRY(ws->pre_ce.reserve(nb * sorted_words * 8));
    }
    MZK_TRY(ws->buckets.reserve((size_t)passes * wm * EC::PT_WORDS * 4));
    MZK_TRY(ws->occ.reserve((size_t)passes * wm));
    const int n_out_one = n_win * (log_m + 1);
    const int n_out = n_out_one * count;
    const size_t out_bytes = (size_t)n_out * 4 * FQ::N * 4;
    const size_t counts_words = (size_t)sets * (1 + MSM_HEAVY_COUNTERS), host_bytes = out_bytes + (size_t)passes * counts_words * 4;
    MZK_TRY(ws->collect.reserve(out_bytes));
    if (ws->h_collect_cap < host_bytes) {
        if (ws->h_collect) HIP_TRY(hipHostFree(ws->h_collect));
        ws->h_collect = nullptr;
        HIP_TRY(hipHostMalloc(&ws->h_collect, host_bytes, hipHostMallocDefault));
        ws->h_collect_cap = host_bytes;
    }
    std::vector<uint32_t> h1_caps(passes, 0), desc_caps(passes, 0);
    std::vector<const uint32_t*> count_ptrs(passes, nullptr);
    uint32_t* collect = ws->collect.as<uint32_t>();
    HeavyJobs jobs;
    std::memset(&jobs, 0, sizeof jobs);
    uint32_t heavy_run_cap_max = 0, long_desc_cap_max = 0;
    bool heavy_level_c = false;
    SortStreams& ss = g_sort[cur().logical];
    if (overlap) {
        MZK_TRY(sort_stream_init(ss));
        HIP_TRY(hipEventRecord(ss.ev_start, st));
        for (int q = 0; q < n_sort_streams(); q++) HIP_TRY(hipStreamWaitEvent(ss.streams[q], ss.ev_start, 0));
    }

    {
        ProfScope total("msm_total", st);
        const unsigned n_ranges = M >> MSM_RANGE_LOG ? M >> MSM_RANGE_LOG : 1u;
        for (int p = 0; p < passes; p++) {
            const size_t b = overlap ? (size_t)p % nb : 0;
            const hipStream_t sst = overlap ? ss.streams[p % n_sort_streams()] : st;
            uint32_t* hist = ws->hist.as<uint32_t>() + b * wm;
            uint32_t* offs = ws->offs.as<uint32_t>() + b * wm;
            uint32_t* order = ws->cursor.as<uint32_t>() + b * wm;
            uint32_t* sorted = ws->sorted.as<uint32_t>() + b * sorted_words;
            const uint64_t n = fuse ? n_max : items[p].n;
            const uint32_t* d_scalars = items[p].d_scalars;
            const uint32_t* d_bases = items[p].d_bases;
            uint32_t* buckets = ws->buckets.as<uint32_t>() + (size_t)p * wm * EC::PT_WORDS;
            uint8_t* occ = ws->occ.as<uint8_t>() + (size_t)p * wm;
            const uint64_t n_sorted = pre.c ? n * (uint64_t)n_dig : n;
            unsigned long long peak = n_sorted / M + 1;
            if (pre.c) {
                const int top_bits = (is_mont ? FR::BITS : 256) - c * (n_dig - 1);
                unsigned long long top_range = 1ull << (top_bits > 0 ? top_bits : 0);
                if (top_bits > 0 && top_bits < 32) {
                    const int sh = c * (n_dig - 1), wi = sh >> 5, bo = sh & 31;
                    unsigned long long v = FR::MOD[wi] >> bo;
                    if (bo && wi + 1 < FR::N) v |= (unsigned long long)FR::MOD[wi + 1] << (32 - bo);
                    v &= (1ull << top_bits) - 1;
                    if (v + 1 < top_range) top_range = v + 1;
                }
                const unsigned long long extra = top_bits < c - 1 ? n / top_range : 0;
                if (extra <= 4 * peak) peak += extra;
            }
            const uint32_t cap = (uint32_t)std::max<unsigned long long>(MSM_MIN_CAP, peak + 6 * (unsigned long long)std::sqrt((double)peak) + 8);
            const uint32_t desc_cap = std::min(desc_cap_max, desc_cap_of(n_sorted, cap, h1_frac));
            desc_caps[p] = desc_cap;
            const size_t slot = defer_heavy ? (size_t)p : 0;
            LongDesc* desc = reinterpret_cast<LongDesc*>(ws->long_desc.as<char>() + slot * desc_slot_bytes);
            uint32_t* parts = ws->long_parts.as<uint32_t>() + slot * parts_slot_words;
            uint32_t* desc_count = reinterpret_cast<uint32_t*>(desc + (size_t)sets * desc_cap);
            const uint32_t* heavy_count = desc_count + sets;
            const uint32_t run_cap = (uint32_t)(2 * (n_sorted / MSM_HEAVY_RUN) + 2);
            const uint32_t h1_cap = std::min(h1_cap_max, h1_cap_of(n_sorted, run_cap, h1_frac));
            h1_caps[p] = h1_cap;
            cur().last_cap = cap; cur().last_desc_cap = desc_cap; cur().last_h1_cap = h1_cap;
            count_ptrs[p] = desc_count;
            HeavyRun* heavy_runs = reinterpret_cast<HeavyRun*>(desc_count + (((size_t)sets * (1 + MSM_HEAVY_COUNTERS) + 3) & ~(size_t)3));
            uint32_t* h1 = parts + (size_t)sets * desc_cap * EC::PT_WORDS;
            uint32_t* h2 = h1 + (size_t)sets * h1_cap * EC::PT_WORDS;
            uint32_t* h3 = h2 + (size_t)sets * run_cap * EC::PT_WORDS;
            const unsigned long long dstride = (n + 7) & ~7ull;
            const unsigned gs = (unsigned)((n + MSM_THREADS - 1) / MSM_THREADS);
            if (overlap && (size_t)p >= nb) HIP_TRY(hipStreamWaitEvent(sst, ss.ev_acc[b], 0));
            const unsigned long long list_stride = (pre.c || sort2) ? 0ull : n;
            if (!pre.c && !sort2) {
                ProfScope ps("msm_sort", sst);
                uint16_t* digits = reinterpret_cast<uint16_t*>(ws->digits.as<char>() + b * digits_bytes);
                hipLaunchKernelGGL((msm_digits_kernel<FR>), dim3(gs), dim3(MSM_THREADS), 0, sst, d_scalars, n, is_mont, c, sets, digits, dstride);
                hipLaunchKernelGGL((msm_sort_kernel<false>), dim3(n_ranges, sets), dim3(MSM_SORT_THREADS), 0, sst, digits, n, dstride, M, hist, offs, sorted);
                hipLaunchKernelGGL(msm_scan_kernel, dim3(sets), dim3(1024), 0, sst, hist, offs, M);
                hipLaunchKernelGGL((msm_sort_kernel<true>), dim3(n_ranges, sets), dim3(MSM_SORT_THREADS), 0, sst, digits, n, dstride, M, hist, offs, sorted);
            } else {
                ProfScope ps("msm_sort", sst);
                uint32_t* dig32 = reinterpret_cast<uint32_t*>(ws->digits.as<char>() + b * digits_bytes);
                uint32_t* cnt = ws->pre_cnt.as<uint32_t>() + b * cnt_words;
                uint32_t* coff = ws->pre_off.as<uint32_t>() + b * 8192;
                unsigned long long* coarse = ws->pre_ce.as<unsigned long long>() + b * sorted_words;
                const uint32_t chunk = pre_chunk_of(n);
                const uint32_t n_chunks = (uint32_t)((n + chunk - 1) / chunk);
                uint32_t* bin_total = cnt;
                uint32_t* bin_cursor = cnt + 1024;
                uint32_t* bin_start = coff;
                const uint32_t bstride = pre.c ? 0u : M;
                PreMulti multi;
                std::memset(&multi, 0, sizeof multi);
                if (fuse) {
                    multi.count = (uint32_t)count; multi.set_stride = M;
                    PreDigitsMulti dm;
                    std::memset(&dm, 0, sizeof dm);
                    unsigned long long n_max = 0;
                    for (int q = 0; q < count; q++) {
                        multi.n[q] = items[q].n; multi.base_off[q] = items[q].base_off;
                        dm.scalars[q] = items[q].d_scalars; dm.n[q] = items[q].n;
                        n_max = std::max<unsigned long long>(n_max, items[q].n);
                    }
                    static const bool digits_per_msm = std::getenv("MZK_MSM_DIGITS_PER_MSM") != nullptr;
                    if (digits_per_msm) {
                        for (int q = 0; q < count; q++)
                            hipLaunchKernelGGL((pre_digits_kernel<FR>), dim3((unsigned)((items[q].n + MSM_THREADS - 1) / MSM_THREADS)), dim3(MSM_THREADS), 0, sst,
                                               items[q].d_scalars, items[q].n, is_mont, c, n_dig, dig32 + (size_t)q * n_dig * dstride, dstride);
                    } else if (n_max) {
                        hipLaunchKernelGGL((pre_digits_multi_kernel<FR>), dim3((unsigned)((n_max + MSM_THREADS - 1) / MSM_THREADS), (unsigned)count), dim3(MSM_THREADS), 0, sst,
                                           dm, is_mont, c, n_dig, dig32, dstride);
                    }
                } else {
                    hipLaunchKernelGGL((pre_digits_kernel<FR>), dim3(gs), dim3(MSM_THREADS), 0, sst, d_scalars, n, is_mont, c, n_dig, dig32, dstride);
                }
                const dim3 coarse_grid(n_chunks, (unsigned)fused_k);
                HIP_TRY(hipMemsetAsync(cnt, 0, cnt_words * 4, sst));
                hipLaunchKernelGGL(pre_coarse_count_kernel, coarse_grid, dim3(PRE_CTHREADS), 0, sst, dig32, n, dstride, n_dig, (int)n_bins, pb, bstride, chunk, multi, bin_total);
                uint32_t* huge = coff + 1088;
                const uint64_t records = n * (uint64_t)n_dig * fused_k;
                const uint32_t slice = (uint32_t)std::max<uint64_t>(16384, (records + 2047) / 2048);
                const uint32_t slice_grid = (uint32_t)std::min<uint64_t>(PRE_SLICE_CAP, records / slice + PRE_HUGE_MAX + 1);
                const uint32_t huge_grid = (uint32_t)std::min<uint64_t>(PRE_HUGE_MAX, records / PRE_HUGE + 1);
                hipLaunchKernelGGL(pre_bin_scan_kernel, dim3(1), dim3(1024), 0, sst, bin_total, (int)n_bins, bin_start, bin_cursor, slice, huge,
                                   find_in_sort ? desc_count : nullptr, (uint32_t)sets * (1 + MSM_HEAVY_COUNTERS));
                hipLaunchKernelGGL(pre_coarse_scatter_kernel, coarse_grid, dim3(PRE_CTHREADS), 0, sst, dig32, n, dstride, n_dig, (int)n_bins, pb, bstride, chunk,
                                   pre.c ? pre.tab_stride : 0ull, pre.c ? items[p].base_off : 0ull, multi, bin_cursor, coarse);
                uint32_t* keycnt_sort = diet ? cnt + 2048 : nullptr;
                hipLaunchKernelGGL(pre_fine_kernel, dim3(n_bins), dim3(1024), 0, sst, bin_start, coarse, (uint32_t)wm, pb, hist, offs, sorted, huge, M, keycnt_sort);
                if (records > PRE_HUGE) {
                    hipLaunchKernelGGL(pre_huge_count_kernel, dim3(slice_grid), dim3(1024), 0, sst, huge, bin_start, coarse, (uint32_t)wm, pb, slice, hist);
                    hipLaunchKernelGGL(pre_huge_scan_kernel, dim3(huge_grid), dim3(1024), 0, sst, huge, bin_start, (uint32_t)wm, pb, hist, offs, order, M, keycnt_sort);
                    hipLaunchKernelGGL(pre_huge_scatter_kernel, dim3(slice_grid), dim3(1024), 0, sst, huge, bin_start, coarse, (uint32_t)wm, pb, slice, order, sorted);
                }
            }
            {
                ProfScope ps("msm_sort", sst);
                uint32_t* keycnt = ws->pre_cnt.as<uint32_t>() + b * cnt_words + 2048;
                const unsigned slices = (M + MSM_ORDER_SLICE - 1) / MSM_ORDER_SLICE;
                if (!pre.c && !sort2) HIP_TRY(hipMemsetAsync(keycnt, 0, (size_t)sets * 1024 * 4, sst));
                if (diet) {
                    hipLaunchKernelGGL(msm_order_place_kernel, dim3(slices, sets), dim3(1024), 0, sst, hist, offs, M, keycnt, keycnt + (size_t)sets * 1024, order,
                                       sets, cap, desc_cap, desc, find_in_sort ? desc_count : nullptr, run_cap, h1_cap, heavy_runs, rank_global);
                } else {
                    hipLaunchKernelGGL(msm_order_hist_kernel, dim3(slices, sets), dim3(1024), 0, sst, hist, M, keycnt);
                    hipLaunchKernelGGL(msm_order_scan_kernel, dim3(rank_global ? 1 : sets), dim3(1024), 0, sst, keycnt, rank_global ? (uint32_t)sets : 0u);
                    hipLaunchKernelGGL(msm_order_scatter_kernel, dim3(slices, sets), dim3(1024), 0, sst, hist, M, keycnt, order, rank_global);
                }
            }
            if (overlap) {
                HIP_TRY(hipEventRecord(ss.ev_sorted[b], sst));
                HIP_TRY(hipStreamWaitEvent(st, ss.ev_sorted[b], 0));
            }
            {
                int log_split = 0;
                const unsigned long long mean = n_sorted / M;
                static const int max_split = std::getenv("MZK_MSM_MAX_SPLIT") ? std::atoi(std::getenv("MZK_MSM_MAX_SPLIT")) : 3;
                const bool few_rounds = wm < (1ull << 18);
                while (log_split < max_split) {
                    const int nx = log_split + 1;
                    bool stop;
                    if (few_rounds) stop = nx < 3 ? ((wm << nx) > (1ull << 20) || (mean >> nx) < 2) : ((wm << nx) > (1ull << 18) || (mean >> 5) == 0);
                    else stop = ((1ull << nx) - 1) * 32 > mean;
                    if (stop) break;
                    log_split = nx;
                }
                static const int force_split = std::getenv("MZK_MSM_FORCE_SPLIT") ? std::atoi(std::getenv("MZK_MSM_FORCE_SPLIT")) : -1;
                if (force_split >= 0 && force_split <= 3) log_split = force_split;
                static const bool no_tail = std::getenv("MZK_MSM_NO_TAIL_SPLIT") != nullptr;
                static const bool force_tail = std::getenv("MZK_MSM_FORCE_TAIL") != nullptr;
                static const int tail_frac_log = std::getenv("MZK_MSM_TAIL_FRAC_LOG") ? std::atoi(std::getenv("MZK_MSM_TAIL_FRAC_LOG")) : 3;
                static const int tail_split = std::getenv("MZK_MSM_TAIL_SPLIT") ? std::atoi(std::getenv("MZK_MSM_TAIL_SPLIT")) : 2;
                unsigned long long rank0 = 0;
                if (sets > 1 && !no_tail && force_split < 0 && (force_tail || (!few_rounds && log_split == 1 && mean >= 8)) && tail_frac_log >= 1 && tail_frac_log <= 6 && tail_split >= 1 && tail_split <= 3) {
                    rank0 = (wm - (wm >> tail_frac_log)) & ~(unsigned long long)(MSM_ACC_THREADS - 1);
                    log_split = tail_split;
                }
                if (log_split == 0) {
                    ProfScope ps("msm_accumulate", st);
                    hipLaunchKernelGGL((msm_accumulate_kernel<EC>), dim3((unsigned)((wm + MSM_ACC_THREADS - 1) / MSM_ACC_THREADS)), dim3(MSM_ACC_THREADS), 0, st,
                                       d_bases, list_stride, offs, hist, sorted, order, M, sets, cap, find_in_sort ? nullptr : desc_count, buckets, occ);
                } else {
                    const size_t n_split = (size_t)(wm - rank0), split_threads = n_split << log_split, threads = (size_t)rank0 + split_threads;
                    MZK_TRY(ws->split.reserve(split_threads * EC::PT_WORDS * 4));
                    uint32_t* sub = ws->split.as<uint32_t>();
                    const dim3 acc_grid((unsigned)((threads + MSM_ACC_THREADS - 1) / MSM_ACC_THREADS)), cmb_grid((unsigned)((split_threads + 2 * MSM_ACC_THREADS - 1) / (2 * MSM_ACC_THREADS)));
                    {
                        ProfScope ps("msm_accumulate", st);
                        if (sets == 1)
                            hipLaunchKernelGGL((msm_accumulate_split_kernel<EC, true>), acc_grid, dim3(MSM_ACC_THREADS), 0, st, d_bases, list_stride, offs, hist, sorted, order, M, sets,
                                               cap, log_split, find_in_sort ? nullptr : desc_count, sub, rank0, buckets, occ);
                        else
                            hipLaunchKernelGGL((msm_accumulate_split_kernel<EC, false>), acc_grid, dim3(MSM_ACC_THREADS), 0, st, d_bases, list_stride, offs, hist, sorted, order, M, sets,
                                               cap, log_split, find_in_sort ? nullptr : desc_count, sub, rank0, buckets, occ);
                    }
                    ProfScope pc("msm_split_combine", st);
                    if (sets == 1)
                        hipLaunchKernelGGL((msm_split_combine_kernel<EC, true>), cmb_grid, dim3(MSM_ACC_THREADS), 0, st, sub, (unsigned long long)n_split, log_split, order, rank0, buckets, occ);
                    else
                        hipLaunchKernelGGL((msm_split_combine_kernel<EC, false>), cmb_grid, dim3(MSM_ACC_THREADS), 0, st, sub, (unsigned long long)n_split, log_split, order, rank0, buckets, occ);
                }
            }
            {
                ProfScope ps("msm_long", st);
                if (!find_in_sort)
                    hipLaunchKernelGGL(msm_long_find_kernel, dim3((unsigned)((wm + 255) / 256)), dim3(256), 0, st, hist, offs, M, sets, cap, desc_cap, desc, desc_count,
                                       run_cap, h1_cap, heavy_runs);
                HeavyJob& jb = jobs.j[defer_heavy ? p : 0];
                jb.bases = d_bases; jb.sorted = sorted; jb.n = list_stride; jb.runs = heavy_runs; jb.count = heavy_count;
                jb.h1 = h1; jb.h2 = h2; jb.h3 = h3; jb.buckets = buckets; jb.occ = occ; jb.run_cap = run_cap; jb.h1_cap = h1_cap; jb.M = M;
                jb.desc = desc; jb.desc_count = desc_count; jb.parts = parts; jb.desc_cap = desc_cap;
                heavy_run_cap_max = std::max(heavy_run_cap_max, run_cap);
                long_desc_cap_max = std::max(long_desc_cap_max, desc_cap);
                heavy_level_c = heavy_level_c || n_sorted > (uint64_t)MSM_HEAVY_RUN * MSM_HEAVY_FANIN;
                if (!defer_heavy) MZK_TRY((launch_rare<EC>(jobs, 1, sets, desc_cap, run_cap, n_sorted > (uint64_t)MSM_HEAVY_RUN * MSM_HEAVY_FANIN, diet, st)));
            }
            if (overlap) HIP_TRY(hipEventRecord(ss.ev_acc[b], st));
        }
        if (defer_heavy) {
            ProfScope ps("msm_long", st);
            MZK_TRY((launch_rare<EC>(jobs, (unsigned)passes, sets, long_desc_cap_max, heavy_run_cap_max, heavy_level_c, diet, st)));
        }
        {
            ProfScope ps("msm_reduce", st);
            uint32_t* buckets = ws->buckets.as<uint32_t>();
            uint8_t* occ = ws->occ.as<uint8_t>();
            const int nw_all = sets * passes;
            int first_tail = 1;
            while (first_tail <= log_m && (size_t)first_tail * (M >> first_tail) > 256) first_tail++;
            static const size_t quad_max = std::getenv("MZK_MSM_QUAD_MAX") ? (size_t)std::atoll(std::getenv("MZK_MSM_QUAD_MAX")) : 65536;
            for (int lvl = 1; lvl < first_tail; lvl++) {
                const uint32_t h = M >> lvl;
                const size_t threads = (size_t)nw_all * lvl * h;
                static const bool fold2 = std::getenv("MZK_MSM_FOLD2") != nullptr;
                if (fold2 && diet && lvl + 1 < first_tail && h >= 2) {
                    const size_t t2 = (size_t)nw_all * lvl * (h >> 1);
                    if (threads <= quad_max)
                        hipLaunchKernelGGL((msm_fold2_quad_kernel<EC>), dim3((unsigned)((4 * t2 + MSM_ACC_THREADS - 1) / MSM_ACC_THREADS)), dim3(MSM_ACC_THREADS), 0, st,
                                           buckets, occ, M, h, lvl, nw_all);
                    else
                        hipLaunchKernelGGL((msm_fold2_kernel<EC>), dim3((unsigned)((t2 + MSM_ACC_THREADS - 1) / MSM_ACC_THREADS)), dim3(MSM_ACC_THREADS), 0, st,
                                           buckets, occ, M, h, lvl, nw_all);
                    lvl++;
                    continue;
                }
                if (threads <= quad_max)
                    hipLaunchKernelGGL((msm_fold_quad_kernel<EC>), dim3((unsigned)((4 * threads + MSM_ACC_THREADS - 1) / MSM_ACC_THREADS)), dim3(MSM_ACC_THREADS), 0, st,
                                       buckets, occ, M, h, lvl, nw_all);
                else
                    hipLaunchKernelGGL((msm_fold_kernel<EC>), dim3((unsigned)((threads + MSM_ACC_THREADS - 1) / MSM_ACC_THREADS)), dim3(MSM_ACC_THREADS), 0, st,
                                       buckets, occ, M, h, lvl, nw_all);
            }
            uint32_t* tail_collect = diet ? collect : nullptr;
            if (first_tail <= log_m) {
                if (quad_max) hipLaunchKernelGGL((msm_fold_tail_quad_kernel<EC>), dim3(nw_all), dim3(MSM_TAIL_QUAD_THREADS), 0, st, buckets, occ, M, log_m, first_tail, tail_collect);
                else hipLaunchKernelGGL((msm_fold_tail_kernel<EC>), dim3(nw_all), dim3(256), 0, st, buckets, occ, M, log_m, first_tail, tail_collect);
            }
            if (!tail_collect || first_tail > log_m)
                hipLaunchKernelGGL((msm_collect_kernel<EC>), dim3((n_out + 63) / 64), dim3(64), 0, st, buckets, occ, M, log_m, nw_all, collect);
        }
        HIP_TRY(hipGetLastError());
        HIP_TRY(hipMemcpyAsync(ws->h_collect, collect, out_bytes, hipMemcpyDeviceToHost, st));
        if (defer_heavy)
            for (int p = 0; p < passes; p++)
                HIP_TRY(hipMemcpyAsync(static_cast<uint8_t*>(ws->h_collect) + out_bytes + (size_t)p * counts_words * 4, count_ptrs[p], counts_words * 4,
                                       hipMemcpyDeviceToHost, st));
    }
    HIP_TRY(hipStreamSynchronize(st));
    if (defer_heavy) {
        const uint32_t* cw = reinterpret_cast<const uint32_t*>(static_cast<const uint8_t*>(ws->h_collect) + out_bytes);
        double grow = 0;
        for (int p = 0; p < passes; p++)
            for (int w = 0; w < sets; w++) {
                const uint32_t need = cw[(size_t)p * counts_words + sets + (size_t)w * MSM_HEAVY_COUNTERS + 5];
                if (need > h1_caps[p]) grow = std::max(grow, (double)need / (double)h1_cap_worst);
                const uint32_t need_desc = cw[(size_t)p * counts_words + w];
                if (need_desc > desc_caps[p]) grow = std::max(grow, (double)need_desc / (double)desc_cap_worst);
            }
        if (grow > 0) {
            ws->heavy_frac = std::min(1.0, std::max(ws->heavy_frac * 2, grow * 1.25));
            return MSM_RETRY;
        }
    }
    const uint32_t* h = reinterpret_cast<const uint32_t*>(ws->h_collect);
    const size_t per = (size_t)n_out_one * 4 * FQ::N;
    std::vector<uint32_t*> outs(count);
    for (int p = 0; p < count; p++) outs[p] = items[p].out_xyz;
    host_horner_batch<FQ>(h, per, count, n_win, c, outs.data());
    return MZK_OK;
}

constexpr uint64_t PRE_MIN_N = 1ull << 10;
constexpr int MSM_GROUP_MAX = 6;

template <class FR, class EC>
int32_t msm_batch_dev(const MsmItem* items, int count, int is_mont, const PreInfo& pre, const uint32_t* plain_table, size_t aff_words,
                      hipStream_t st) {
    using FQ = typename EC::Field;
    std::vector<MsmItem> run;
    int i = 0;
    while (i < count) {
        if (items[i].n == 0) { write_infinity<FQ>(items[i].out_xyz); i++; continue; }
        if (items[i].n >= (1ull << 27)) { set_error("MSM size must be < 2^27"); return MZK_ERR_INVALID_ARG; }
        auto use_pre = [&](const MsmItem& it) { return pre.c != 0 && it.n >= PRE_MIN_N; };
        auto win_of = [&](const MsmItem& it) { return use_pre(it) ? pre.c : msm_choose_window(it.n); };
        const bool p0 = use_pre(items[i]);
        const int c = win_of(items[i]);
        int j = i + 1;
        while (j < count && j - i < MSM_GROUP_MAX && items[j].n != 0 && items[j].n < (1ull << 27) && use_pre(items[j]) == p0 && win_of(items[j]) == c) j++;
        run.assign(items + i, items + j);
        if (!p0)
            for (auto& it : run) it.d_bases = plain_table + it.base_off * aff_words;
        for (int attempt = 0;; attempt++) {
            const int32_t rc = msm_group_dev<FR, EC>(run.data(), j - i, c, is_mont, p0 ? pre : PreInfo{}, st);
            cur().last_attempts = (uint32_t)attempt + 1;
            if (rc == MSM_RETRY && attempt < 8) continue;
            if (rc == MSM_RETRY) { set_error("MSM heavy-bucket scratch: no fit after 8 attempts"); return MZK_ERR_UNSUPPORTED; }
            MZK_TRY(rc);
            break;
        }
        i = j;
    }
    return MZK_OK;
}

template <class EC>
int32_t srs_build_pre_t(Srs& s, hipStream_t st, void (*next_level)(const uint32_t*, uint32_t*, unsigned long long, int)) {
    int lg = 0;
    while ((2ull << lg) <= s.n) lg++;
    int c;
    if (s.curve == MZK_CURVE_BLS12_381) c = lg <= 17 ? 16 : 20;
    else c = lg <= 15 ? 15 : (lg <= 19 ? 17 : 20);
    if (const char* force = std::getenv("MZK_PRE_C")) {
        const int f = std::atoi(force);
        if (f >= 8 && f <= 22) c = f;
    }
    const int W = msm_num_windows(256, c);
    const size_t level = (size_t)s.n * EC::AFF_WORDS;
    size_t free_b = 0, total_b = 0;
    HIP_TRY(hipMemGetInfo(&free_b, &total_b));
    size_t budget = free_b / 2;
    if (const char* b = std::getenv("MZK_MSM_TABLE_BUDGET")) budget = std::min<size_t>(budget, (size_t)std::strtoull(b, nullptr, 10));
    if ((size_t)W * level * 4 > budget) { s.pre_c = -1; return MZK_OK; }
    HIP_TRY(hipMalloc((void**)&s.d_pre, (size_t)W * level * 4));
    HIP_TRY(hipStreamSynchronize(st));
    const auto t_build = std::chrono::steady_clock::now();
    HIP_TRY(hipMemcpyAsync(s.d_pre, s.d_int, level * 4, hipMemcpyDeviceToDevice, st));
    const unsigned long long threads = (s.n + 3) / 4;
    for (int w = 1; w < W; w++)
        hipLaunchKernelGGL(next_level, dim3((unsigned)((threads + 127) / 128)), dim3(128), 0, st,
                           s.d_pre + (size_t)(w - 1) * level, s.d_pre + (size_t)w * level, (unsigned long long)s.n, c);
    HIP_TRY(hipGetLastError());
    HIP_TRY(hipStreamSynchronize(st));
    s.pre_build_ms = std::chrono::duration<double, std::milli>(std::chrono::steady_clock::now() - t_build).count();
    s.pre_c = c;
    s.pre_levels = W;
    return MZK_OK;
}
}
int32_t srs_build_pre(Srs& s, hipStream_t st) {
    if (s.d_pre || s.pre_c < 0 || !s.d_int) return MZK_OK;
    return s.curve == MZK_CURVE_BLS12_381 ? srs_build_pre_t<EcFz<BlsFqZ>>(s, st, pre_next_level_z_kernel<BlsFqZ>)
                                          : srs_build_pre_t<EcFx<BnFqX>>(s, st, pre_next_level_kernel<BnFqX>);
}

int32_t msm_dispatch(const Srs& s, uint64_t base_offset, const uint32_t* d_scalars, uint64_t n, int is_mont, uint32_t* out, hipStream_t st) {
    const uint32_t* sc[1] = {d_scalars};
    return msm_batch_dispatch(s, 1, sc, &n, &base_offset, is_mont, out, st);
}

int32_t msm_batch_dispatch(const Srs& s, uint32_t n_polys, const uint32_t* const* d_scalars, const uint64_t* lens, const uint64_t* base_offsets,
                           int is_mont, uint32_t* out_xyz, hipStream_t st) {
    const int fw = fq_words(s.curve);
    const bool bls = s.curve == MZK_CURVE_BLS12_381;
    const size_t aff_words = bls ? (size_t)EcFz<BlsFqZ>::AFF_WORDS : (size_t)EcFx<BnFqX>::AFF_WORDS;
    const uint32_t* table = s.d_int;
    if (!table) { set_error("SRS has no internal table"); return MZK_ERR_BAD_HANDLE; }
    std::vector<MsmItem> items(n_polys);
    bool want_pre = false;
    for (uint32_t i = 0; i < n_polys; i++) {
        const uint64_t off = base_offsets ? base_offsets[i] : 0;
        if (off > s.n || lens[i] > s.n - off) {
            set_error("MSM longer than the registered SRS (poly degree larger than allowed)");
            return MZK_ERR_INVALID_ARG;
// ... 218 lines not shown
```

### mpc-jellyfish_amd/csrc/mzk.hip

```cpp
#include <condition_variable>
#include <cstdlib>
#include <map>
#include <mutex>
#include <vector>

#include "internal.hpp"

namespace mzk {

thread_local std::string g_last_error;
std::string g_last_error_global;
std::mutex g_last_error_lock;
void set_error(const std::string& s) {
    g_last_error = s;
    std::lock_guard<std::mutex> g(g_last_error_lock);
    g_last_error_global = s;
}
int32_t hip_status(hipError_t e, const char* what) {
    if (e == hipSuccess) return MZK_OK;
    set_error(std::string(what) + ": " + hipGetErrorString(e));
    return e == hipErrorOutOfMemory ? MZK_ERR_OOM : MZK_ERR_HIP;
}

int32_t DevBuf::reserve(size_t bytes) {
// ... 1177 lines not shown
    *out_stream = st;
    return MZK_OK;
}
int32_t mzk_ctx_check_witness(uint64_t pk_handle, const WitnessCheckIn* in, mzk_witness_report* out_report, void* stream) {
    ENTER_HANDLE(pk_handle);
    return plonk_check_witness_dev(pk_handle, *in, out_report, (hipStream_t)stream);
}
int32_t mzk_ctx_derive_variables(uint64_t pk_handle, const void* d_sigma_coeffs, void* d_out_variables_u32, uint64_t* out_n_vars, void* stream) {
    ENTER_HANDLE(pk_handle);
    return plonk_derive_variables_dev(pk_handle, reinterpret_cast<const uint32_t*>(d_sigma_coeffs), reinterpret_cast<uint32_t*>(d_out_variables_u32), out_n_vars,
                                      (hipStream_t)stream);
}
int32_t mzk_stream_destroy(void* stream) {
    BIND_CUR();
    if (stream) HIP_TRY(hipStreamDestroy((hipStream_t)stream));
    return MZK_OK;
}
int32_t mzk_stream_sync(void* stream) {
    BIND_CUR();
    HIP_TRY(hipStreamSynchronize((hipStream_t)stream));
    return MZK_OK;
}
int32_t mzk_stream_wait_stream(void* waiter, void* signaller) {
    BIND_CUR();
    hipEvent_t ev = nullptr;
    HIP_TRY(hipEventCreateWithFlags(&ev, hipEventDisableTiming));
    hipError_t e = hipEventRecord(ev, (hipStream_t)signaller);
    if (e == hipSuccess) e = hipStreamWaitEvent((hipStream_t)waiter, ev, 0);
    (void)hipEventDestroy(ev);
    if (e != hipSuccess) { set_error(std::string("mzk_stream_wait_stream: ") + hipGetErrorString(e)); return MZK_ERR_HIP; }
    return MZK_OK;
}
int32_t mzk_dev_upload_async(void* dptr, const void* host, uint64_t bytes, void* stream) {
    BIND_CUR();
    if (bytes && (!dptr || !host)) { set_error("null pointer"); return MZK_ERR_INVALID_ARG; }
    if (bytes) HIP_TRY(hipMemcpyAsync(dptr, host, bytes, hipMemcpyHostToDevice, (hipStream_t)stream));
    return MZK_OK;
}
int32_t mzk_dev_download_async(void* host, const void* dptr, uint64_t bytes, void* stream) {
    BIND_CUR();
    if (bytes && (!dptr || !host)) { set_error("null pointer"); return MZK_ERR_INVALID_ARG; }
    if (bytes) HIP_TRY(hipMemcpyAsync(host, dptr, bytes, hipMemcpyDeviceToHost, (hipStream_t)stream));
    return MZK_OK;
}
int32_t mzk_dev_sync(void) {
    ENTER_CUR();
    HIP_TRY(hipDeviceSynchronize());
    return MZK_OK;
}
int32_t mzk_dev_copy(void* dst, const void* src, uint64_t bytes, void* stream) {
    ENTER_CUR();
    if (bytes && (!dst || !src)) { set_error("null pointer"); return MZK_ERR_INVALID_ARG; }
    if (bytes) HIP_TRY(hipMemcpyAsync(dst, src, bytes, hipMemcpyDeviceToDevice, (hipStream_t)stream));
    return MZK_OK;
}
int32_t mzk_dev_copy_peer(void* dst, int32_t dst_device, const void* src, int32_t src_device, uint64_t bytes, void* stream) {
    if (dst_device < 0 || dst_device >= MAX_CTX || src_device < 0 || src_device >= MAX_CTX || !g_ctx[dst_device].init || !g_ctx[src_device].init) {
        set_error("mzk_dev_copy_peer: both devices must have been initialised (mzk_init)");
        return MZK_ERR_NOT_INIT;
    }
    if (bytes && (!dst || !src)) { set_error("null pointer"); return MZK_ERR_INVALID_ARG; }
    Ctx* cx_ = &g_ctx[src_device];
    CtxBind bind_(cx_);
    MZK_TRY(bind_.rc);
    if (!bytes) return MZK_OK;
    const int pd = g_ctx[dst_device].device, ps = cx_->device;
    if (pd == ps) HIP_TRY(hipMemcpyAsync(dst, src, bytes, hipMemcpyDeviceToDevice, (hipStream_t)stream));
    else HIP_TRY(hipMemcpyPeerAsync(dst, pd, src, ps, bytes, (hipStream_t)stream));
    return MZK_OK;
}
int32_t mzk_dev_copy2d(void* dst, uint64_t dst_pitch, const void* src, uint64_t src_pitch, uint64_t width, uint64_t height, void* stream) {
    ENTER_CUR();
    if (width && height && (!dst || !src || width > dst_pitch || width > src_pitch)) { set_error("bad argument"); return MZK_ERR_INVALID_ARG; }
    if (width && height) HIP_TRY(hipMemcpy2DAsync(dst, dst_pitch, src, src_pitch, width, height, hipMemcpyDeviceToDevice, (hipStream_t)stream));
    return MZK_OK;
}
int32_t mzk_dev_memset2d(void* dptr, uint64_t pitch, int32_t value, uint64_t width, uint64_t height, void* stream) {
    ENTER_CUR();
    if (width && height && (!dptr || width > pitch)) { set_error("bad argument"); return MZK_ERR_INVALID_ARG; }
    if (width && height) HIP_TRY(hipMemset2DAsync(dptr, pitch, value, width, height, (hipStream_t)stream));
    return MZK_OK;
}
int32_t mzk_dev_memset(void* dptr, int32_t value, uint64_t bytes, void* stream) {
    ENTER_CUR();
    if (bytes && !dptr) { set_error("null pointer"); return MZK_ERR_INVALID_ARG; }
    if (bytes) HIP_TRY(hipMemsetAsync(dptr, value, bytes, (hipStream_t)stream));
    return MZK_OK;
}

int32_t mzk_profile_enable(int32_t on) {
    g_prof = on != 0;
    return MZK_OK;
}
int32_t mzk_profile_get(const char* name, double* out_ms, uint64_t* out_count) {
    ENTER_CUR();
    if (!name || !out_ms || !out_count) return MZK_ERR_INVALID_ARG;
    double ms = 0;
    uint64_t cnt = 0;
    for (auto& r : cx_->prof_recs) {
        if (r.name != name) continue;
        HIP_TRY(hipEventSynchronize(r.b));
        float t = 0;
        HIP_TRY(hipEventElapsedTime(&t, r.a, r.b));
        ms += t;
        cnt++;
    }
    *out_ms = ms;
    *out_count = cnt;
    return MZK_OK;
}
int32_t mzk_profile_reset(void) {
    std::lock_guard<std::mutex> lk0(g_ctx_lock);
    for (auto& cx : g_ctx) {
        if (!cx.init) continue;
        std::lock_guard<std::mutex> lk(cx.lock);
        for (auto& r : cx.prof_recs) { (void)hipEventDestroy(r.a); (void)hipEventDestroy(r.b); }
        cx.prof_recs.clear();
    }
    return MZK_OK;
}
int32_t mzk_msm_set_precompute(int32_t on) {
    g_msm_precompute = on != 0;
    return MZK_OK;
}
int32_t mzk_srs_precompute(uint64_t srs_handle, uint32_t* out_window_bits, uint32_t* out_levels, uint64_t* out_table_bytes, double* out_build_ms) {
    ENTER_HANDLE(srs_handle);
    Srs* sp = srs_find(*cx_, srs_handle);
    if (!sp) return MZK_ERR_BAD_HANDLE;
    Srs& s = *sp;
    MZK_TRY(srs_build_pre(s, nullptr));
    const bool have = s.d_pre != nullptr && s.pre_c > 0;
    const uint64_t aff_bytes = srs_int_point_bytes(s.curve);
    if (out_window_bits) *out_window_bits = have ? (uint32_t)s.pre_c : 0u;
    if (out_levels) *out_levels = have ? (uint32_t)s.pre_levels : 0u;
    if (out_table_bytes) *out_table_bytes = have ? (uint64_t)s.pre_levels * s.n * aff_bytes : 0u;
    if (out_build_ms) *out_build_ms = have ? s.pre_build_ms : 0.0;
    return MZK_OK;
}
int32_t mzk_msm_last_shape(uint32_t* out_window_bits, uint32_t* out_windows, uint32_t* out_buckets) {
    ENTER_CUR();
    if (out_window_bits) *out_window_bits = cx_->last_c;
    if (out_windows) *out_windows = cx_->last_w;
    if (out_buckets) *out_buckets = cx_->last_m;
    return MZK_OK;
}
int32_t mzk_msm_last_rare(uint32_t* out_cap, uint32_t* out_desc_cap, uint32_t* out_h1_cap, uint32_t* out_attempts) {
    ENTER_CUR();
    if (out_cap) *out_cap = cx_->last_cap;
    if (out_desc_cap) *out_desc_cap = cx_->last_desc_cap;
    if (out_h1_cap) *out_h1_cap = cx_->last_h1_cap;
    if (out_attempts) *out_attempts = cx_->last_attempts;
    return MZK_OK;
}

}
```

### mpc-jellyfish_amd/lib.py

```python
from __future__ import annotations

import ctypes as C
import os

_HERE = os.path.dirname(os.path.abspath(__file__))
_LIB = None


class MzkError(RuntimeError):
    def __init__(self, code: int, where: str, detail: str):
        super().__init__(f"{where}: {detail} (code {code})")
        self.code = code


def lib_path() -> str:
    return os.environ.get("MZK_LIB_PATH") or os.path.join(_HERE, "libmi355zk.so")


class WitnessReport(C.Structure):
    _fields_ = [("kind", C.c_uint32), ("copy_checked", C.c_uint32), ("gate_failures", C.c_uint64), ("gate_row", C.c_uint64),
                ("lookup_failures", C.c_uint64), ("lookup_row", C.c_uint64), ("copy_failures", C.c_uint64), ("copy_cell", C.c_uint64),
                ("copy_rep_cell", C.c_uint64), ("row_wires", C.c_uint64 * 24), ("gate_residual", C.c_uint64 * 4)]


# ... 1 lines not shown
    _fields_ = [("num_wire_types", C.c_uint32), ("num_selectors", C.c_uint32), ("has_plookup", C.c_uint32), ("has_plookup_vk", C.c_uint32),
                ("is_merged", C.c_uint32), ("reserved", C.c_uint32), ("domain_size", C.c_uint64), ("num_inputs", C.c_uint64),
                ("g1_record_bytes", C.c_uint64), ("g2_record_bytes", C.c_uint64), ("sigma_off", C.c_uint64 * 6), ("sigma_len", C.c_uint64 * 6),
                ("selector_off", C.c_uint64 * 14), ("selector_len", C.c_uint64 * 14), ("table_off", C.c_uint64 * 4), ("table_len", C.c_uint64 * 4),
                ("commit_key_off", C.c_uint64), ("commit_key_count", C.c_uint64), ("vk_off", C.c_uint64), ("vk_len", C.c_uint64),
                ("sigma_comms_off", C.c_uint64), ("selector_comms_off", C.c_uint64), ("k_off", C.c_uint64), ("g_off", C.c_uint64), ("h_off", C.c_uint64),
                ("beta_h_off", C.c_uint64), ("plookup_comms_off", C.c_uint64), ("total_len", C.c_uint64)]


MAX_INSTANCES = 64


class BatchProofLayout(C.Structure):
    _fields_ = [("m", C.c_uint32), ("num_wire_types", C.c_uint32), ("ultra", C.c_uint32), ("g1_record_bytes", C.c_uint32), ("total_len", C.c_uint64)] + \
               [(name, C.c_uint64 * MAX_INSTANCES) for name in ("wires_off", "prod_perm_off", "wires_evals_off", "sigma_evals_off", "perm_next_off",
                                                                "plookup_tag_off", "h_off", "prod_lookup_off", "plookup_evals_off")] + \
               [("split_quot_off", C.c_uint64), ("opening_off", C.c_uint64), ("shifted_opening_off", C.c_uint64)]


_SIGS = {
    "mzk_init": [C.c_int32],
    "mzk_set_device": [C.c_int32],
    "mzk_get_device": [C.POINTER(C.c_int32)],
    "mzk_device_count": [C.POINTER(C.c_int32)],
    "mzk_dev_copy_peer": [C.c_void_p, C.c_int32, C.c_void_p, C.c_int32, C.c_uint64, C.c_void_p],
    "mzk_shutdown": [],
    "mzk_srs_register": [C.c_int32, C.c_void_p, C.c_uint64, C.POINTER(C.c_uint64)],
    "mzk_srs_register_dev": [C.c_int32, C.c_void_p, C.c_uint64, C.POINTER(C.c_uint64), C.c_void_p],
    "mzk_srs_release": [C.c_uint64],
    "mzk_srs_generate_for_testing": [C.c_int32, C.c_void_p, C.c_uint64, C.POINTER(C.c_uint64)],
    "mzk_srs_generate_for_testing_g": [C.c_int32, C.c_void_p, C.c_void_p, C.c_uint64, C.POINTER(C.c_uint64)],
    "mzk_srs_lagrange_from_srs": [C.c_uint64, C.c_uint32, C.c_uint32, C.POINTER(C.c_uint64)],
    "mzk_srs_generate_lagrange_for_testing": [C.c_int32, C.c_void_p, C.c_void_p, C.c_uint32, C.c_uint32, C.POINTER(C.c_uint64)],
    "mzk_srs_slice": [C.c_uint64, C.c_uint64, C.c_uint64, C.POINTER(C.c_uint64)],
    "mzk_srs_download": [C.c_uint64, C.c_uint64, C.c_uint64, C.c_void_p],
    "mzk_srs_len": [C.c_uint64, C.POINTER(C.c_uint64)],
    "mzk_key_layout": [C.c_int32, C.c_void_p, C.c_uint64, C.c_uint32, C.POINTER(KeyLayout)],
    "mzk_fr_decode_dev": [C.c_int32, C.c_void_p, C.c_uint64, C.c_uint32, C.c_void_p, C.c_void_p, C.c_void_p, C.c_void_p, C.c_uint32, C.c_uint64,
                          C.POINTER(C.c_uint32), C.POINTER(C.c_uint64), C.c_void_p],
    "mzk_fr_encode_dev": [C.c_int32, C.c_void_p, C.c_uint64, C.c_void_p, C.c_void_p],
    "mzk_g2_decode": [C.c_int32, C.c_void_p, C.c_uint32, C.c_void_p],
    "mzk_g2_mul": [C.c_int32, C.c_void_p, C.c_void_p, C.c_uint32, C.c_void_p],
    "mzk_pairing_product_is_one": [C.c_int32, C.c_void_p, C.c_void_p, C.c_uint64, C.POINTER(C.c_int32)],
    "mzk_pairing_gt": [C.c_int32, C.c_void_p, C.c_void_p, C.c_void_p],
    "mzk_batch_verify_challenge": [C.c_int32, C.c_void_p, C.c_uint64, C.c_void_p],
    "mzk_batch_verify_challenge_t": [C.c_int32, C.c_uint32, C.c_void_p, C.c_uint64, C.c_void_p],
    "mzk_keccak256": [C.c_void_p, C.c_uint64, C.c_void_p],
    "mzk_solidity_challenge": [C.c_int32, C.c_void_p, C.c_void_p, C.c_uint64, C.c_void_p],
    "mzk_verifier_create": [C.c_int32, C.c_void_p, C.c_uint64, C.c_uint32, C.POINTER(C.c_uint64)],
    "mzk_verifier_destroy": [C.c_uint64],
    "mzk_verifier_shape": [C.c_uint64, C.POINTER(C.c_uint32), C.POINTER(C.c_uint32), C.POINTER(C.c_uint64), C.POINTER(C.c_uint64)],
    "mzk_verifier_batch_begin": [C.c_uint64, C.c_void_p, C.c_uint64, C.c_uint64, C.c_void_p, C.c_void_p, C.c_void_p, C.c_void_p, C.c_uint32,
                                 C.POINTER(C.c_uint64), C.c_void_p, C.POINTER(C.c_uint64)],
    "mzk_verifier_batch_challenges": [C.c_uint64, C.c_void_p],
    "mzk_verifier_batch_scalars": [C.c_uint64, C.c_void_p, C.c_void_p, C.c_void_p],
    "mzk_verifier_batch_finish": [C.c_uint64, C.c_void_p, C.c_void_p, C.c_void_p],
    "mzk_verifier_check": [C.c_uint64, C.c_void_p, C.c_void_p, C.c_uint64, C.POINTER(C.c_int32)],
    "mzk_batch_proof_layout": [C.c_int32, C.c_uint32, C.c_uint32, C.c_uint32, C.c_void_p, C.c_uint64, C.POINTER(BatchProofLayout)],
    "mzk_verifier_aggregate_shape": [C.POINTER(C.c_uint64), C.c_uint32, C.POINTER(C.c_uint32), C.POINTER(C.c_uint32), C.POINTER(C.c_uint64),
                                     C.POINTER(C.c_uint64)],
    "mzk_verifier_aggregate_begin": [C.POINTER(C.c_uint64), C.c_uint32, C.c_void_p, C.c_uint64, C.c_uint64, C.c_void_p, C.c_void_p, C.c_void_p, C.c_void_p,
                                     C.c_uint32, C.POINTER(C.c_uint64), C.c_void_p, C.POINTER(C.c_uint64)],
    "mzk_verifier_create_open_key": [C.c_int32, C.c_void_p, C.c_void_p, C.c_void_p, C.c_uint32, C.POINTER(C.c_uint64)],
    "mzk_verifier_link_begin": [C.c_uint64, C.c_void_p, C.c_uint64, C.c_void_p, C.c_void_p, C.c_uint32, C.POINTER(C.c_uint64), C.c_void_p, C.POINTER(C.c_uint64)],
    "mzk_verifier_link_values": [C.c_uint64, C.c_void_p, C.c_void_p],
    "mzk_verifier_link_weights": [C.c_uint64, C.c_void_p, C.c_void_p],
    "mzk_verifier_open_begin": [C.c_uint64, C.c_void_p, C.c_uint64, C.c_void_p, C.c_void_p, C.c_uint32, C.POINTER(C.c_uint64), C.POINTER(C.c_uint64)],
    "mzk_kzg_open_batch_dev": [C.c_uint64, C.c_uint32, C.POINTER(C.c_void_p), C.POINTER(C.c_uint64), C.c_void_p, C.c_void_p, C.c_void_p, C.c_void_p],
    "mzk_kzg_multi_open_rou_dev": [C.c_uint64, C.c_uint64, C.c_void_p, C.c_uint64, C.c_uint32, C.c_uint64, C.c_void_p, C.c_void_p, C.c_void_p],
    "mzk_sha256": [C.c_void_p, C.c_uint64, C.c_void_p],
    "mzk_expand_message_xmd_sha256": [C.c_void_p, C.c_uint64, C.c_void_p, C.c_uint64, C.c_uint32, C.c_void_p, C.c_uint64],
    "mzk_hash_to_field_sha256": [C.c_int32, C.c_void_p, C.c_uint64, C.c_void_p, C.c_uint64, C.c_void_p],
    "mzk_bytes_to_field_dev": [C.c_int32, C.c_void_p, C.c_uint64, C.c_void_p, C.c_void_p],
    "mzk_field_to_bytes_dev": [C.c_int32, C.c_void_p, C.c_uint64, C.c_void_p, C.POINTER(C.c_uint64), C.c_void_p],
    "mzk_vid_advz_commit_only_dev": [C.c_uint64, C.c_uint64, C.c_uint64, C.c_void_p, C.c_uint64, C.c_uint32, C.c_uint32, C.c_uint32, C.c_void_p, C.c_void_p],
    "mzk_vid_advz_disperse_dev": [C.c_uint64, C.c_uint64, C.c_uint64, C.c_void_p, C.c_uint64, C.c_uint32, C.c_uint32, C.c_uint32, C.c_void_p, C.c_void_p,
                                  C.c_void_p, C.c_void_p, C.c_void_p, C.c_void_p, C.c_void_p, C.c_void_p],
    "mzk_vid_advz_verify_shares_dev": [C.c_int32, C.c_uint64, C.c_uint64, C.c_uint32, C.c_void_p, C.c_void_p, C.c_void_p, C.c_void_p, C.c_void_p, C.c_void_p,
                                       C.c_void_p, C.c_void_p],
    "mzk_vid_advz_recover_dev": [C.c_int32, C.c_uint32, C.c_uint64, C.c_uint32, C.c_void_p, C.c_void_p, C.c_void_p, C.c_void_p],
    "mzk_srs_register_serialized": [C.c_int32, C.c_void_p, C.c_uint64, C.c_uint32, C.POINTER(C.c_uint64), C.POINTER(C.c_uint64)],
    "mzk_srs_register_serialized_dev": [C.c_int32, C.c_void_p, C.c_uint64, C.c_uint32, C.POINTER(C.c_uint64), C.POINTER(C.c_uint64), C.c_void_p],
    "mzk_srs_serialize": [C.c_uint64, C.c_uint64, C.c_uint64, C.c_uint32, C.c_void_p],
    "mzk_msm": [C.c_uint64, C.c_uint64, C.c_void_p, C.c_uint64, C.c_int32, C.c_void_p],
    "mzk_msm_dev": [C.c_uint64, C.c_uint64, C.c_void_p, C.c_uint64, C.c_int32, C.c_void_p, C.c_void_p],
    "mzk_msm_batch": [C.c_uint64, C.c_uint32, C.POINTER(C.c_void_p), C.POINTER(C.c_uint64), C.POINTER(C.c_uint64), C.c_int32, C.c_void_p],
    "mzk_msm_batch_dev": [C.c_uint64, C.c_uint32, C.POINTER(C.c_void_p), C.POINTER(C.c_uint64), C.POINTER(C.c_uint64), C.c_int32, C.c_void_p, C.c_void_p],
    "mzk_msm_affine": [C.c_uint64, C.c_uint64, C.c_void_p, C.c_uint64, C.c_int32, C.c_void_p],
    "mzk_g1_jacobian_to_affine": [C.c_int32, C.c_void_p, C.c_uint64, C.c_void_p],
    "mzk_g1_sum_jacobian": [C.c_int32, C.c_void_p, C.c_uint64, C.c_void_p],
    "mzk_ntt": [C.c_int32, C.c_void_p, C.c_uint64, C.c_uint32, C.c_int32, C.c_void_p],
    "mzk_ntt_batch": [C.c_int32, C.c_uint32, C.POINTER(C.c_void_p), C.POINTER(C.c_uint64), C.c_uint32, C.c_int32, C.c_void_p],
    "mzk_ntt_dev": [C.c_int32, C.c_void_p, C.c_uint64, C.c_uint32, C.c_int32, C.c_void_p, C.c_uint32, C.c_uint64, C.c_void_p],
    "mzk_plonk_pk_register": [C.c_int32, C.c_uint32, C.c_uint32, C.c_void_p, C.c_void_p, C.c_uint64, C.c_void_p, C.POINTER(C.c_uint64)],
    "mzk_plonk_pk_release": [C.c_uint64],
    "mzk_plonk_quotient_dev": [C.c_uint64, C.c_void_p, C.c_uint64, C.c_void_p, C.c_void_p, C.c_void_p, C.c_void_p, C.c_void_p],
    "mzk_plonk_quotient": [C.c_uint64, C.c_void_p, C.c_uint64, C.c_void_p, C.c_void_p, C.c_void_p, C.c_void_p],
    "mzk_keccak_f1600": [C.c_void_p],
    "mzk_chacha_blocks": [C.c_void_p, C.c_uint64, C.c_uint32, C.c_uint32, C.c_void_p],
    "mzk_plonk_pk_register_ultra": [C.c_int32, C.c_uint32, C.c_void_p, C.c_void_p, C.c_void_p, C.c_uint64, C.c_void_p, C.POINTER(C.c_uint64)],
    "mzk_plonk_quotient_ultra_dev": [C.c_uint64, C.c_void_p, C.c_uint64, C.c_void_p, C.c_void_p, C.c_void_p, C.c_void_p, C.c_void_p, C.c_void_p],
    "mzk_plonk_pk_register_chunked": [C.c_int32, C.c_uint32, C.c_uint32, C.c_void_p, C.c_void_p, C.c_void_p, C.c_uint64, C.c_void_p, C.c_void_p, C.c_uint32,
                                      C.POINTER(C.c_uint64)],
    "mzk_plonk_quotient_chunked_dev": [C.c_uint64, C.c_void_p, C.c_uint64, C.c_uint64, C.c_void_p, C.c_void_p, C.c_void_p, C.c_void_p, C.c_void_p, C.c_void_p],
    "mzk_plonk_quotient_chunked_flags_dev": [C.c_uint64, C.c_void_p, C.c_uint64, C.c_uint64, C.c_uint32, C.c_void_p, C.c_void_p, C.c_void_p, C.c_void_p, C.c_void_p,
                                             C.c_void_p],
    "mzk_plonk_quotient_combine_dev": [C.c_int32, C.c_uint32, C.c_void_p, C.c_void_p, C.c_void_p],
    "mzk_plonk_quotient_combine_classes_dev": [C.c_int32, C.c_uint32, C.c_void_p, C.c_uint32, C.c_void_p, C.c_void_p, C.c_void_p],
    "mzk_plonk_quotient_top_dev": [C.c_uint64, C.c_void_p, C.c_uint64, C.c_uint64, C.c_void_p, C.c_void_p, C.c_void_p, C.c_void_p, C.POINTER(C.c_uint32), C.c_void_p],
    "mzk_plonk_quotient_combine_top_dev": [C.c_int32, C.c_uint32, C.c_void_p, C.c_uint32, C.c_void_p, C.c_void_p, C.c_uint32, C.c_void_p, C.c_void_p],
    "mzk_plookup_sorted_vec_dev": [C.c_uint64, C.c_void_p, C.c_void_p, C.c_void_p, C.c_void_p, C.c_void_p, C.c_void_p],
    "mzk_plookup_product_dev": [C.c_uint64, C.c_void_p, C.c_void_p, C.c_void_p, C.c_void_p, C.c_void_p, C.c_void_p, C.c_void_p],
    "mzk_plonk_perm_product_dev": [C.c_uint64, C.c_void_p, C.c_void_p, C.c_void_p, C.c_void_p, C.c_void_p],
    "mzk_plonk_perm_product": [C.c_uint64, C.c_void_p, C.c_void_p, C.c_void_p, C.c_void_p],
    "mzk_plonk_wire_permutation_dev": [C.c_void_p, C.c_uint64, C.c_uint64, C.c_void_p, C.c_void_p],
    "mzk_plonk_sigma_values_dev": [C.c_int32, C.c_uint32, C.c_uint32, C.c_void_p, C.c_void_p, C.c_void_p, C.c_void_p],
    "mzk_plonk_sigma_decode_dev": [C.c_int32, C.c_uint32, C.c_uint32, C.c_void_p, C.c_void_p, C.c_void_p, C.c_void_p],
    "mzk_plonk_variables_from_permutation_dev": [C.c_void_p, C.c_uint64, C.c_void_p, C.POINTER(C.c_uint64), C.c_void_p],
    "mzk_plonk_gather_witness_dev": [C.c_void_p, C.c_uint64, C.c_void_p, C.c_uint64, C.c_void_p, C.c_void_p],
    "mzk_poly_eval_dev": [C.c_int32, C.c_void_p, C.c_uint64, C.c_uint32, C.c_uint64, C.c_void_p, C.c_void_p, C.c_void_p],
    "mzk_poly_lincomb_dev": [C.c_int32, C.c_uint32, C.POINTER(C.c_void_p), C.POINTER(C.c_uint64), C.c_void_p, C.c_void_p, C.c_uint64, C.c_void_p],
    "mzk_poly_split_quotient_dev": [C.c_int32, C.c_void_p, C.c_uint64, C.c_uint32, C.c_void_p, C.c_void_p, C.c_uint64, C.c_void_p],
    "mzk_poly_mask_dev": [C.c_int32, C.c_uint32, C.POINTER(C.c_void_p), C.c_uint64, C.c_uint32, C.c_void_p, C.c_void_p],
    "mzk_poly_div_linear_dev": [C.c_int32, C.c_void_p, C.c_uint64, C.c_void_p, C.c_void_p, C.c_void_p],
    "mzk_poly_div_linear_rem_dev": [C.c_int32, C.c_void_p, C.c_uint64, C.c_void_p, C.c_void_p, C.c_void_p, C.c_void_p],
    "mzk_poly_degree_dev": [C.c_void_p, C.c_uint64, C.c_void_p, C.c_void_p],
    "mzk_poly_div_roots_dev": [C.c_int32, C.c_void_p, C.c_uint64, C.c_uint32, C.c_uint64, C.c_uint64, C.c_void_p, C.c_void_p],
    "mzk_dev_alloc": [C.c_uint64, C.POINTER(C.c_void_p)],
    "mzk_dev_free": [C.c_void_p],
    "mzk_dev_upload": [C.c_void_p, C.c_void_p, C.c_uint64],
    "mzk_dev_download": [C.c_void_p, C.c_void_p, C.c_uint64],
    "mzk_dev_sync": [],
    "mzk_stream_create": [C.POINTER(C.c_void_p)],
    "mzk_stream_destroy": [C.c_void_p],
    "mzk_stream_sync": [C.c_void_p],
    "mzk_stream_wait_stream": [C.c_void_p, C.c_void_p],
    "mzk_dev_upload_async": [C.c_void_p, C.c_void_p, C.c_uint64, C.c_void_p],
    "mzk_dev_download_async": [C.c_void_p, C.c_void_p, C.c_uint64, C.c_void_p],
    "mzk_dev_copy": [C.c_void_p, C.c_void_p, C.c_uint64, C.c_void_p],
    "mzk_dev_copy2d": [C.c_void_p, C.c_uint64, C.c_void_p, C.c_uint64, C.c_uint64, C.c_uint64, C.c_void_p],
    "mzk_dev_memset": [C.c_void_p, C.c_int32, C.c_uint64, C.c_void_p],
    "mzk_dev_memset2d": [C.c_void_p, C.c_uint64, C.c_int32, C.c_uint64, C.c_uint64, C.c_void_p],
    "mzk_profile_enable": [C.c_int32],
    "mzk_profile_get": [C.c_char_p, C.POINTER(C.c_double), C.POINTER(C.c_uint64)],
    "mzk_profile_reset": [],
    "mzk_host_alloc": [C.c_uint64, C.POINTER(C.c_void_p)],
    "mzk_host_free": [C.c_void_p],
    "mzk_host_register": [C.c_void_p, C.c_uint64],
    "mzk_host_unregister": [C.c_void_p],
    "mzk_msm_set_precompute": [C.c_int32],
    "mzk_srs_precompute": [C.c_uint64, C.POINTER(C.c_uint32), C.POINTER(C.c_uint32), C.POINTER(C.c_uint64), C.POINTER(C.c_double)],
    "mzk_msm_last_shape": [C.POINTER(C.c_uint32), C.POINTER(C.c_uint32), C.POINTER(C.c_uint32)],
    "mzk_msm_last_rare": [C.POINTER(C.c_uint32), C.POINTER(C.c_uint32), C.POINTER(C.c_uint32), C.POINTER(C.c_uint32)],
    "mzk_srs_hbm_bytes": [C.c_uint64, C.POINTER(C.c_uint64), C.POINTER(C.c_uint64)],
    "mzk_plonk_pk_hbm_bytes": [C.c_uint64, C.POINTER(C.c_uint64)],
    "mzk_workspace_hbm_bytes": [C.POINTER(C.c_uint64)],
    "mzk_workspace_release": [],
    "mzk_launch_count": [C.POINTER(C.c_uint64)],
    "mzk_poly_eval_many_dev": [C.c_int32, C.c_uint32, C.c_void_p, C.c_void_p, C.c_void_p, C.c_void_p, C.c_void_p, C.c_void_p, C.c_void_p, C.c_void_p],
    "mzk_prover_create": [C.c_int32, C.c_uint32, C.c_uint32, C.c_void_p, C.c_void_p, C.c_void_p, C.c_uint64, C.c_void_p, C.c_uint64, C.c_uint64, C.c_void_p,
                          C.POINTER(C.c_uint64)],
    "mzk_prover_create_from_circuit": [C.c_int32, C.c_uint32, C.c_uint32, C.c_void_p, C.c_void_p, C.c_uint64, C.c_void_p, C.c_void_p, C.c_uint64, C.c_uint64,
                                       C.c_void_p, C.POINTER(C.c_uint64)],
    "mzk_prover_create_from_circuit_dev": [C.c_int32, C.c_uint32, C.c_uint32, C.c_void_p, C.c_void_p, C.c_uint64, C.c_void_p, C.c_void_p, C.c_uint64, C.c_uint64,
                                           C.c_void_p, C.POINTER(C.c_uint64)],
    "mzk_prover_create_serialized": [C.c_int32, C.c_void_p, C.c_uint64, C.c_uint32, C.c_uint64, C.c_void_p, C.POINTER(C.c_uint64), C.POINTER(C.c_uint64),
                                     C.POINTER(C.c_uint64), C.POINTER(C.c_uint64)],
    "mzk_prover_serialize_key": [C.c_uint64, C.c_uint32, C.c_uint64, C.c_void_p, C.c_void_p, C.c_int32, C.c_void_p, C.c_uint64, C.POINTER(C.c_uint64)],
    "mzk_prover_serialize_vk": [C.c_uint64, C.c_uint32, C.c_uint64, C.c_void_p, C.c_void_p, C.c_int32, C.c_void_p, C.c_uint64, C.POINTER(C.c_uint64)],
    "mzk_prover_destroy": [C.c_uint64],
    "mzk_prover_fork": [C.c_uint64, C.POINTER(C.c_uint64)],
    "mzk_prover_vk_commitments": [C.c_uint64, C.c_void_p, C.c_void_p],
    "mzk_prover_set_wire_variables": [C.c_uint64, C.c_void_p, C.c_uint64],
    "mzk_prover_derive_wire_variables": [C.c_uint64, C.POINTER(C.c_uint64)],
    "mzk_prover_get_wire_variables": [C.c_uint64, C.c_void_p, C.c_uint64, C.POINTER(C.c_uint64)],
    "mzk_prover_round1": [C.c_uint64, C.c_int32, C.c_void_p, C.c_uint64, C.c_void_p, C.c_void_p, C.c_uint64, C.c_void_p, C.c_void_p],
    "mzk_prover_check_witness": [C.c_uint64, C.c_int32, C.c_void_p, C.c_uint64, C.c_void_p, C.c_void_p, C.c_uint64, C.POINTER(WitnessReport)],
    "mzk_prover_round1_5": [C.c_uint64, C.c_void_p, C.c_void_p, C.c_void_p],
    "mzk_prover_round2": [C.c_uint64, C.c_void_p, C.c_void_p, C.c_void_p, C.c_void_p],
    "mzk_prover_round2_5": [C.c_uint64, C.c_void_p, C.c_void_p],
    "mzk_prover_round3": [C.POINTER(C.c_uint64), C.c_uint32, C.c_void_p, C.c_void_p, C.c_void_p],
    "mzk_prover_round4": [C.c_uint64, C.c_void_p, C.c_void_p],
    "mzk_prover_round5": [C.POINTER(C.c_uint64), C.c_uint32, C.c_void_p, C.c_void_p],
    "mzk_prover_exchange_buffer": [C.c_uint64, C.POINTER(C.c_void_p), C.POINTER(C.c_uint64)],
    "mzk_prover_set_peer_buffers": [C.c_uint64, C.POINTER(C.c_void_p), C.POINTER(C.c_int32)],
    "mzk_prover_poly_dev": [C.c_uint64, C.c_uint32, C.POINTER(C.c_void_p), C.POINTER(C.c_uint64)],
    "mzk_prover_profile": [C.c_uint64, C.c_int32],
    "mzk_prover_timings": [C.c_uint64, C.c_char_p, C.c_uint64],
    "mzk_prover_hbm_bytes": [C.c_uint64, C.POINTER(C.c_uint64), C.POINTER(C.c_uint64), C.POINTER(C.c_uint64)],
    "mzk_prover_shared_hbm_bytes": [C.c_uint64, C.POINTER(C.c_uint64), C.POINTER(C.c_uint32)],
}
_STR_FUNCS = ("mzk_strerror", "mzk_last_error", "mzk_version")
EXPORTS = tuple(_SIGS) + _STR_FUNCS


def load():
    global _LIB
    if _LIB is None:
        path = lib_path()
        if not os.path.exists(path):
            raise FileNotFoundError(f"{path} not found: build it with `python -c 'import __graft_entry__ as g; g.build()'` "
                                    "(hipcc, gfx950). There is no CPU fallback.")
        try:
            import torch
        except ImportError:
            pass
        L = C.CDLL(path)
        for name, args in _SIGS.items():
            f = getattr(L, name)
            f.argtypes = args
            f.restype = C.c_int32
        L.mzk_strerror.argtypes = [C.c_int32]
        for name in _STR_FUNCS:
            getattr(L, name).restype = C.c_char_p
        _LIB = L
    return _LIB


def check(rc: int, where: str):
    if rc != 0:
        L = load()
        raise MzkError(rc, where, f"{L.mzk_strerror(rc).decode()}: {L.mzk_last_error().decode()}")


_INIT_DEV = None


def init(device: int = -1):
    global _INIT_DEV
    L = load()
    check(L.mzk_init(device), "mzk_init")
    _INIT_DEV = device
    return L


def ensure_init():
    return load() if _INIT_DEV is not None else init(-1)


def profile_get(name: str):
    L = ensure_init()
    ms, cnt = C.c_double(), C.c_uint64()
    check(L.mzk_profile_get(name.encode(), C.byref(ms), C.byref(cnt)), "mzk_profile_get")
    return ms.value, cnt.value


def msm_last_shape():
    L = load()
    a, b, c = C.c_uint32(), C.c_uint32(), C.c_uint32()
    L.mzk_msm_last_shape(C.byref(a), C.byref(b), C.byref(c))
    return a.value, b.value, c.value


def msm_last_rare():
    L = load()
    a, b, c, d = C.c_uint32(), C.c_uint32(), C.c_uint32(), C.c_uint32()
    L.mzk_msm_last_rare(C.byref(a), C.byref(b), C.byref(c), C.byref(d))
    return a.value, b.value, c.value, d.value
```

Measured before the change: 336.5 million.

## Pair bucket b with b+M/2 in MSM accumulate to fuse first reduce level

Adds a pair mode in which each accumulate thread walks the lists for bucket b and bucket b+M/2 in a single running sum. It checkpoints the upper bucket's sum and then continues into the lower one, so the first running-sum fold level is folded into accumulation. The order, scatter and long-find kernels now key on the combined count of each pair. A pair list plus a fixup kernel handle pairs where either bucket overflows the cap, and the reduce loop starts at level 2. This removes one fold launch and its memory traffic, at the cost of more complex split/combine indexing, an extra fixup pass, and doubled work per thread that may worsen load balance.

```diff
diff --git a/include/mzk.h b/include/mzk.h
--- a/include/mzk.h
+++ b/include/mzk.h
@@ -352,6 +352,7 @@
 MZK_API int32_t mzk_launch_count(uint64_t* out_launches);
 MZK_API int32_t mzk_msm_last_shape(uint32_t* out_window_bits, uint32_t* out_windows, uint32_t* out_buckets);
 MZK_API int32_t mzk_msm_last_rare(uint32_t* out_cap, uint32_t* out_desc_cap, uint32_t* out_h1_cap, uint32_t* out_attempts);
+MZK_API int32_t mzk_msm_last_schedule(uint32_t* out_pair_mode, uint32_t* out_fold_launches, uint32_t* out_fixup_launches);
 
 #ifdef __cplusplus
 }
diff --git a/mpc-jellyfish_amd/csrc/internal.hpp b/mpc-jellyfish_amd/csrc/internal.hpp
--- a/mpc-jellyfish_amd/csrc/internal.hpp
+++ b/mpc-jellyfish_amd/csrc/internal.hpp
@@ -124,6 +124,7 @@
     std::vector<ProfRec> prof_recs;
     uint32_t last_c = 0, last_w = 0, last_m = 0;
     uint32_t last_cap = 0, last_desc_cap = 0, last_h1_cap = 0, last_attempts = 0;
+    uint32_t last_pair = 0, last_fold_launches = 0, last_fixup_launches = 0;
     std::map<uint64_t, Srs> srs;
     uint64_t next_handle = 1;
     IoSlot io[IO_SLOTS];
diff --git a/mpc-jellyfish_amd/csrc/msm.cuh b/mpc-jellyfish_amd/csrc/msm.cuh
--- a/mpc-jellyfish_amd/csrc/msm.cuh
+++ b/mpc-jellyfish_amd/csrc/msm.cuh
@@ -15,6 +15,8 @@
 constexpr uint32_t MSM_HEAVY_FANIN = MSM_ACC_THREADS * 32;
 constexpr int MSM_HEAVY_COUNTERS = 6;
 __host__ __device__ inline bool msm_is_heavy(uint32_t count, uint32_t cap) { return count > cap + MSM_HEAVY_RUN; }
+__host__ __device__ inline uint32_t msm_count_words(uint32_t sets) { return sets * (1 + MSM_HEAVY_COUNTERS) + 1; }
+__host__ __device__ inline uint32_t msm_pair_counter(uint32_t sets) { return sets * (1 + MSM_HEAVY_COUNTERS); }
 
 inline int msm_choose_window(unsigned long long n) {
     int lg = 0;
@@ -134,14 +136,15 @@
 
 constexpr uint32_t MSM_ORDER_SLICE = 8192;
 __device__ __forceinline__ uint32_t order_key(uint32_t count) { return 1023u - min(count, 1023u); }
-
-__global__ __launch_bounds__(1024) void msm_order_hist_kernel(const uint32_t* __restrict__ hist, uint32_t M, uint32_t* __restrict__ keycnt) {
+__device__ __forceinline__ uint32_t order_load(const uint32_t* __restrict__ hist_w, uint32_t b, uint32_t half) { return hist_w[b] + (half ? hist_w[b + half] : 0u); }
+
+__global__ __launch_bounds__(1024) void msm_order_hist_kernel(const uint32_t* __restrict__ hist, uint32_t M, uint32_t* __restrict__ keycnt, uint32_t half) {
     __shared__ uint32_t cnt[1024];
     const uint32_t w = blockIdx.y, t = threadIdx.x;
-    const uint32_t lo = blockIdx.x * MSM_ORDER_SLICE, hi = min(M, lo + MSM_ORDER_SLICE);
+    const uint32_t lo = blockIdx.x * MSM_ORDER_SLICE, hi = min(half ? half : M, lo + MSM_ORDER_SLICE);
     cnt[t] = 0;
     __syncthreads();
-    for (uint32_t b = lo + t; b < hi; b += 1024) atomicAdd(&cnt[order_key(hist[(size_t)w * M + b])], 1u);
+    for (uint32_t b = lo + t; b < hi; b += 1024) atomicAdd(&cnt[order_key(order_load(hist + (size_t)w * M, b, half))], 1u);
     __syncthreads();
     if (cnt[t]) atomicAdd(&keycnt[(size_t)w * 1024 + t], cnt[t]);
 }
@@ -161,22 +164,24 @@
     keycnt[(size_t)w * 1024 + t] = part[t] - mine;
 }
 __global__ __launch_bounds__(1024) void msm_order_scatter_kernel(const uint32_t* __restrict__ hist, uint32_t M, uint32_t* __restrict__ keycur,
-                                                                 uint32_t* __restrict__ order, bool global) {
+                                                                 uint32_t* __restrict__ order, bool global, uint32_t half) {
     __shared__ uint32_t cnt[1024];
     const uint32_t w = blockIdx.y, t = threadIdx.x;
     const uint32_t row = global ? 0u : w;
-    const uint32_t lo = blockIdx.x * MSM_ORDER_SLICE, hi = min(M, lo + MSM_ORDER_SLICE);
+    const uint32_t items = half ? half : M;
+    const uint32_t lo = blockIdx.x * MSM_ORDER_SLICE, hi = min(items, lo + MSM_ORDER_SLICE);
+    const uint32_t* hist_w = hist + (size_t)w * M;
     cnt[t] = 0;
     __syncthreads();
-    for (uint32_t b = lo + t; b < hi; b += 1024) atomicAdd(&cnt[order_key(hist[(size_t)w * M + b])], 1u);
+    for (uint32_t b = lo + t; b < hi; b += 1024) atomicAdd(&cnt[order_key(order_load(hist_w, b, half))], 1u);
     __syncthreads();
     const uint32_t mine = cnt[t];
     __syncthreads();
     cnt[t] = mine ? atomicAdd(&keycur[(size_t)row * 1024 + t], mine) : 0u;
     __syncthreads();
     for (uint32_t b = lo + t; b < hi; b += 1024) {
-        const uint32_t pos = atomicAdd(&cnt[order_key(hist[(size_t)w * M + b])], 1u);
-        order[(size_t)row * M + pos] = w * M + b;
+        const uint32_t pos = atomicAdd(&cnt[order_key(order_load(hist_w, b, half))], 1u);
+        order[(size_t)row * items + pos] = w * M + b;
     }
 }
 
@@ -189,12 +194,14 @@
                                                                const uint32_t* __restrict__ keycnt, uint32_t* __restrict__ keycur, uint32_t* __restrict__ order,
                                                                int n_win, uint32_t cap, uint32_t desc_cap, LongDesc* __restrict__ desc,
                                                                uint32_t* __restrict__ desc_count, uint32_t run_cap, uint32_t h1_cap, HeavyRun* __restrict__ heavy_runs,
-                                                               bool global) {
+                                                               bool global, uint32_t half, uint32_t* __restrict__ pair_list) {
     __shared__ uint32_t cnt[1024];
     __shared__ uint32_t part[1024];
     const uint32_t w = blockIdx.y, t = threadIdx.x;
     const uint32_t row = global ? 0u : w;
-    const uint32_t lo = blockIdx.x * MSM_ORDER_SLICE, hi = min(M, lo + MSM_ORDER_SLICE);
+    const uint32_t items = half ? half : M;
+    const uint32_t lo = blockIdx.x * MSM_ORDER_SLICE, hi = min(items, lo + MSM_ORDER_SLICE);
+    const uint32_t* hist_w = hist + (size_t)w * M;
     uint32_t total = 0;
     if (global) for (uint32_t s = 0; s < gridDim.y; s++) total += keycnt[(size_t)s * 1024 + t];
     else total = keycnt[(size_t)w * 1024 + t];
@@ -208,17 +215,20 @@
         __syncthreads();
     }
     const uint32_t key_start = part[t] - total;
-    for (uint32_t b = lo + t; b < hi; b += 1024) atomicAdd(&cnt[order_key(hist[(size_t)w * M + b])], 1u);
+    for (uint32_t b = lo + t; b < hi; b += 1024) atomicAdd(&cnt[order_key(order_load(hist_w, b, half))], 1u);
     __syncthreads();
     const uint32_t mine = cnt[t];
     __syncthreads();
     cnt[t] = mine ? key_start + atomicAdd(&keycur[(size_t)row * 1024 + t], mine) : 0u;
     __syncthreads();
     for (uint32_t b = lo + t; b < hi; b += 1024) {
-        const uint32_t c = hist[(size_t)w * M + b];
-        const uint32_t pos = atomicAdd(&cnt[order_key(c)], 1u);
-        order[(size_t)row * M + pos] = w * M + b;
-        if (desc_count && c > cap) msm_long_register(w, b, c, offs[(size_t)w * M + b], n_win, cap, desc_cap, desc, desc_count, run_cap, h1_cap, heavy_runs);
+        const uint32_t c = hist_w[b], c2 = half ? hist_w[b + half] : 0u;
+        const uint32_t pos = atomicAdd(&cnt[order_key(c + c2)], 1u);
+        order[(size_t)row * items + pos] = w * M + b;
+        if (!desc_count) continue;
+        if (c > cap) msm_long_register(w, b, c, offs[(size_t)w * M + b], n_win, cap, desc_cap, desc, desc_count, run_cap, h1_cap, heavy_runs);
+        if (c2 > cap) msm_long_register(w, b + half, c2, offs[(size_t)w * M + b + half], n_win, cap, desc_cap, desc, desc_count, run_cap, h1_cap, heavy_runs);
+        if (half && (c > cap || c2 > cap)) pair_list[atomicAdd(&desc_count[msm_pair_counter((uint32_t)n_win)], 1u)] = w * M + b;
     }
 }
 
@@ -364,18 +374,50 @@
     for (int k = 0; k < X::XN; k++) { dst[k] = fx.l[k]; dst[X::XN + k] = fy.l[k]; }
 }
 
-template <class EC>
+template <class EC, class Ckpt>
+__device__ __forceinline__ typename EC::Pt pair_accumulate(const uint32_t* __restrict__ bases, const uint32_t* __restrict__ lists, uint32_t start_up, uint32_t c_up,
+                                                           uint32_t start_lo, uint32_t c_lo, bool fused, uint32_t part, uint32_t S, Ckpt&& ckpt) {
+    const uint32_t total = c_up + c_lo, lo_base = start_lo - c_up;
+    typename EC::Pt acc = EC::inf();
+    for (uint32_t k = part;; k += S) {
+        if (k - c_up < S) {
+            ckpt(acc);
+            if (!fused) acc = EC::inf();
+        }
+        if (k >= total) break;
+        const uint32_t e = lists[(k < c_up ? start_up : lo_base) + k];
+        acc = EC::madd(acc, EC::load_aff(bases, e & 0x7fffffffu), (e >> 31) != 0);
+    }
+    return acc;
+}
+
+template <class EC, bool PAIR>
 __global__ __launch_bounds__(MSM_ACC_THREADS) void msm_accumulate_kernel(const uint32_t* __restrict__ bases, unsigned long long n,
                                                                           const uint32_t* __restrict__ offs, const uint32_t* __restrict__ hist,
                                                                           const uint32_t* __restrict__ sorted, const uint32_t* __restrict__ order,
                                                                           uint32_t M, int n_win, uint32_t cap, uint32_t* __restrict__ long_count,
                                                                           uint32_t* __restrict__ buckets, uint8_t* __restrict__ occ) {
     if (long_count && blockIdx.x == 0)
-        for (unsigned i = threadIdx.x; i < (unsigned)n_win * (1 + MSM_HEAVY_COUNTERS); i += MSM_ACC_THREADS) long_count[i] = 0u;
+        for (unsigned i = threadIdx.x; i < msm_count_words((uint32_t)n_win); i += MSM_ACC_THREADS) long_count[i] = 0u;
     const unsigned long long t0 = (unsigned long long)blockIdx.x * MSM_ACC_THREADS + threadIdx.x;
-    if (t0 >= (unsigned long long)n_win * M) return;
+    if (t0 >= (unsigned long long)n_win * (PAIR ? M >> 1 : M)) return;
     const uint32_t tb = order[t0];
     const unsigned long long t = tb, w = tb / M;
+    if constexpr (PAIR) {
+        const unsigned long long tu = t + (M >> 1);
+        const uint32_t h_lo = hist[t], h_up = hist[tu];
+        const uint32_t c_lo = msm_is_heavy(h_lo, cap) ? 0u : min(h_lo, cap), c_up = msm_is_heavy(h_up, cap) ? 0u : min(h_up, cap);
+        const typename EC::Pt acc = pair_accumulate<EC>(bases, sorted + w * n, offs[tu], c_up, offs[t], c_lo, h_lo <= cap && h_up <= cap, 0u, 1u,
+            [&](const typename EC::Pt& a) {
+                const bool empty = a.is_inf();
+                occ[tu] = empty ? 0 : 1;
+                if (!empty) EC::store_pt(buckets, tu, a);
+            });
+        const bool empty = acc.is_inf();
+        occ[t] = empty ? 0 : 1;
+        if (!empty) EC::store_pt(buckets, t, acc);
+        return;
+    }
     const uint32_t start = offs[t];
     const uint32_t h = hist[t];
     const uint32_t cnt = msm_is_heavy(h, cap) ? 0u : min(h, cap);
@@ -390,7 +432,7 @@
     if (!empty) EC::store_pt(buckets, t, acc);
 }
 
-template <class EC, bool ONE_SET>
+template <class EC, bool ONE_SET, bool PAIR>
 __global__ __launch_bounds__(MSM_ACC_THREADS) void msm_accumulate_split_kernel(const uint32_t* __restrict__ bases, unsigned long long n,
                                                                                 const uint32_t* __restrict__ offs, const uint32_t* __restrict__ hist,
                                                                                 const uint32_t* __restrict__ sorted, const uint32_t* __restrict__ order,
@@ -398,15 +440,31 @@
                                                                                 uint32_t* __restrict__ sub, unsigned long long rank0,
                                                                                 uint32_t* __restrict__ buckets, uint8_t* __restrict__ occ) {
     if (long_count && blockIdx.x == 0)
-        for (unsigned i = threadIdx.x; i < (unsigned)n_win * (1 + MSM_HEAVY_COUNTERS); i += MSM_ACC_THREADS) long_count[i] = 0u;
+        for (unsigned i = threadIdx.x; i < msm_count_words((uint32_t)n_win); i += MSM_ACC_THREADS) long_count[i] = 0u;
     const unsigned long long t1 = (unsigned long long)blockIdx.x * MSM_ACC_THREADS + threadIdx.x;
     const bool whole = t1 < rank0;
     const unsigned long long u = whole ? 0ull : t1 - rank0;
     const unsigned long long t0 = whole ? t1 : rank0 + (u >> log_split);
-    if (t0 >= (unsigned long long)n_win * M) return;
+    const unsigned long long n_ranks = (unsigned long long)n_win * (PAIR ? M >> 1 : M);
+    if (t0 >= n_ranks) return;
     const uint32_t S = whole ? 1u : 1u << log_split, part = whole ? 0u : (uint32_t)(u & (S - 1));
     const uint32_t tb = order[t0];
     const unsigned long long t = tb, w = ONE_SET ? 0ull : tb / M;
+    if constexpr (PAIR) {
+        const unsigned long long tu = t + (M >> 1);
+        const uint32_t h_lo = hist[t], h_up = hist[tu];
+        const uint32_t c_lo = msm_is_heavy(h_lo, cap) ? 0u : min(h_lo, cap), c_up = msm_is_heavy(h_up, cap) ? 0u : min(h_up, cap);
+        const typename EC::Pt acc = pair_accumulate<EC>(bases, sorted + w * n, offs[tu], c_up, offs[t], c_lo, h_lo <= cap && h_up <= cap, part, S,
+            [&](const typename EC::Pt& a) {
+                const bool empty = a.is_inf();
+                if (whole) occ[tu] = empty ? 0 : 1;
+                if (!whole || !empty) EC::store_pt(whole ? buckets : sub, whole ? tu : u, a);
+            });
+        const bool empty = acc.is_inf();
+        if (whole) occ[t] = empty ? 0 : 1;
+        if (!whole || !empty) EC::store_pt(whole ? buckets : sub, whole ? t : ((n_ranks - rank0) << log_split) + u, acc);
+        return;
+    }
     const uint32_t start = offs[t];
     const uint32_t h = hist[t];
     const uint32_t cnt = msm_is_heavy(h, cap) ? 0u : min(h, cap);
@@ -451,7 +509,7 @@
 template <class EC, bool ONE_SET>
 __global__ __launch_bounds__(MSM_ACC_THREADS) void msm_split_combine_kernel(const uint32_t* __restrict__ sub, unsigned long long n_buckets, int log_split,
                                                                              const uint32_t* __restrict__ order, unsigned long long rank0,
-                                                                             uint32_t* __restrict__ buckets, uint8_t* __restrict__ occ) {
+                                                                             uint32_t* __restrict__ buckets, uint8_t* __restrict__ occ, uint32_t half) {
     __shared__ uint32_t lds[MSM_ACC_THREADS * EC::PT_WORDS];
     const int tid = threadIdx.x;
     const unsigned long long total = n_buckets << log_split;
@@ -471,7 +529,8 @@
         if (mine) {
             acc = EC::add(a, b);
             if (lvl == log_split - 1) {
-                const unsigned long long t = order[rank0 + (base >> log_split) + tid];
+                const unsigned long long r = (base >> log_split) + tid, n_split = n_buckets >> 1;
+                const unsigned long long t = !half ? order[rank0 + r] : (r < n_split ? order[rank0 + r] + half : order[rank0 + r - n_split]);
                 const bool empty = acc.is_inf();
                 occ[t] = empty ? 0 : 1;
                 if (!empty) EC::store_pt(buckets, t, acc);
@@ -498,6 +557,9 @@
     const uint32_t* desc_count;
     uint32_t* parts;
     uint32_t desc_cap;
+    const uint32_t* pair_list;
+    const uint32_t* pair_count;
+    uint32_t pair_half;
 };
 struct HeavyJobs { HeavyJob j[MSM_HEAVY_JOBS]; };
 __device__ __forceinline__ void msm_heavy_push(uint32_t b, uint32_t start, uint32_t rem, uint32_t run_cap, uint32_t h1_cap, uint32_t* __restrict__ cnt,
@@ -527,12 +589,15 @@
 
 __global__ __launch_bounds__(256) void msm_long_find_kernel(const uint32_t* __restrict__ hist, const uint32_t* __restrict__ offs, uint32_t M, int n_win,
                                                             uint32_t cap, uint32_t desc_cap, LongDesc* __restrict__ desc,
-                                                            uint32_t* __restrict__ desc_count, uint32_t run_cap, uint32_t h1_cap, HeavyRun* __restrict__ heavy_runs) {
+                                                            uint32_t* __restrict__ desc_count, uint32_t run_cap, uint32_t h1_cap, HeavyRun* __restrict__ heavy_runs,
+                                                            uint32_t half, uint32_t* __restrict__ pair_list) {
     const unsigned long long t = (unsigned long long)blockIdx.x * 256 + threadIdx.x;
     if (t >= (unsigned long long)n_win * M) return;
     const uint32_t c = hist[t];
     if (c <= cap) return;
-    msm_long_register((uint32_t)(t / M), (uint32_t)(t % M), c, offs[t], n_win, cap, desc_cap, desc, desc_count, run_cap, h1_cap, heavy_runs);
+    const uint32_t b = (uint32_t)(t % M);
+    msm_long_register((uint32_t)(t / M), b, c, offs[t], n_win, cap, desc_cap, desc, desc_count, run_cap, h1_cap, heavy_runs);
+    if (half && (b < half || hist[t - half] <= cap)) pair_list[atomicAdd(&desc_count[msm_pair_counter((uint32_t)n_win)], 1u)] = (uint32_t)(b < half ? t : t - half);
 }
 __device__ __forceinline__ void msm_long_register(uint32_t w, uint32_t b, uint32_t c, uint32_t offs_t, int n_win, uint32_t cap, uint32_t desc_cap,
                                                   LongDesc* __restrict__ desc, uint32_t* __restrict__ desc_count, uint32_t run_cap,
@@ -740,6 +805,16 @@
 }
 
 template <class EC>
+__global__ __launch_bounds__(MSM_ACC_THREADS) void msm_pair_fixup_kernel(HeavyJobs jobs) {
+    const HeavyJob& jb = jobs.j[blockIdx.y];
+    const uint32_t cnt = *jb.pair_count;
+    for (uint32_t i = blockIdx.x * MSM_ACC_THREADS + threadIdx.x; i < cnt; i += gridDim.x * MSM_ACC_THREADS) {
+        const unsigned long long t = jb.pair_list[i];
+        fold_one<EC>(jb.buckets, jb.occ, t, t + jb.pair_half);
+    }
+}
+
+template <class EC>
 __global__ __launch_bounds__(MSM_ACC_THREADS) void msm_fold2_kernel(uint32_t* __restrict__ buckets, uint8_t* __restrict__ occ, uint32_t M, uint32_t h, int nseg, int n_win) {
     const uint32_t q = h >> 1;
     const unsigned long long t = (unsigned long long)blockIdx.x * MSM_ACC_THREADS + threadIdx.x;
diff --git a/mpc-jellyfish_amd/csrc/msm.hip b/mpc-jellyfish_amd/csrc/msm.hip
--- a/mpc-jellyfish_amd/csrc/msm.hip
+++ b/mpc-jellyfish_amd/csrc/msm.hip
@@ -39,6 +39,14 @@
     static const int n = std::min(4, std::max(1, std::getenv("MZK_MSM_SORT_STREAMS") ? std::atoi(std::getenv("MZK_MSM_SORT_STREAMS")) : 2));
     return n;
 }
+inline int msm_tail_frac_log() {
+    static const int v = std::getenv("MZK_MSM_TAIL_FRAC_LOG") ? std::atoi(std::getenv("MZK_MSM_TAIL_FRAC_LOG")) : 3;
+    return v;
+}
+inline int msm_tail_split() {
+    static const int v = std::getenv("MZK_MSM_TAIL_SPLIT") ? std::atoi(std::getenv("MZK_MSM_TAIL_SPLIT")) : 2;
+    return v;
+}
 int32_t sort_stream_init(SortStreams& ss) {
     if (ss.stream) return MZK_OK;
     int prio_least = 0, prio_greatest = 0;
@@ -87,6 +95,13 @@
     if (level_c) hipLaunchKernelGGL((msm_heavy_reduce_kernel<EC>), dim3(64, sets, n_jobs), dim3(MSM_ACC_THREADS), 0, st, jobs, 2);
     HIP_TRY(hipGetLastError());
     return MZK_OK;
+}
+
+template <class EC>
+void launch_pair_fixup(const HeavyJobs& jobs, unsigned n_jobs, hipStream_t st) {
+    ProfScope ps("msm_reduce", st);
+    hipLaunchKernelGGL((msm_pair_fixup_kernel<EC>), dim3(64, n_jobs), dim3(MSM_ACC_THREADS), 0, st, jobs);
+    cur().last_fixup_launches++;
 }
 
 template <class FR, class EC>
@@ -108,6 +123,39 @@
     static const bool no_sort2 = std::getenv("MZK_MSM_PLAIN_SORT1") != nullptr;
     const bool sort2 = !pre.c && !no_sort2 && n_min >= (1ull << 16) && wm >= (1u << 14) && (wm >> PRE_FINE_LOG) <= 1024;
     const uint64_t sorted_max = pre.c ? n_max * n_dig : n_max;
+    struct AccSched { int log_split; bool tail; };
+    auto acc_sched = [&](uint64_t n_sorted) {
+        int log_split = 0;
+        const unsigned long long mean = n_sorted / M;
+        static const int max_split = std::getenv("MZK_MSM_MAX_SPLIT") ? std::atoi(std::getenv("MZK_MSM_MAX_SPLIT")) : 3;
+        const bool few_rounds = wm < (1ull << 18);
+        while (log_split < max_split) {
+            const int nx = log_split + 1;
+            bool stop;
+            if (few_rounds) stop = nx < 3 ? ((wm << nx) > (1ull << 20) || (mean >> nx) < 2) : ((wm << nx) > (1ull << 18) || (mean >> 5) == 0);
+            else stop = ((1ull << nx) - 1) * 32 > mean;
+            if (stop) break;
+            log_split = nx;
+        }
+        static const int force_split = std::getenv("MZK_MSM_FORCE_SPLIT") ? std::atoi(std::getenv("MZK_MSM_FORCE_SPLIT")) : -1;
+        if (force_split >= 0 && force_split <= 3) log_split = force_split;
+        static const bool no_tail = std::getenv("MZK_MSM_NO_TAIL_SPLIT") != nullptr;
+        static const bool force_tail = std::getenv("MZK_MSM_FORCE_TAIL") != nullptr;
+        const bool tail = sets > 1 && !no_tail && force_split < 0 && (force_tail || (!few_rounds && log_split == 1 && mean >= 8)) && msm_tail_frac_log() >= 1 &&
+                          msm_tail_frac_log() <= 6 && msm_tail_split() >= 1 && msm_tail_split() <= 3;
+        return AccSched{tail ? msm_tail_split() : log_split, tail};
+    };
+    static const bool no_pair = std::getenv("MZK_MSM_NO_PAIR") != nullptr, force_pair = std::getenv("MZK_MSM_FORCE_PAIR") != nullptr;
+    bool pair = !no_pair && log_m >= 1 && (force_pair || wm >= (1ull << 19));
+    for (int p = 0; pair && !force_pair && p < passes; p++) {
+        const uint64_t np = fuse ? n_max : items[p].n;
+        const AccSched s = acc_sched(pre.c ? np * (uint64_t)n_dig : np);
+        pair = s.log_split == 0 || s.tail;
+    }
+    const uint32_t pair_half = pair ? M >> 1 : 0u;
+    const size_t n_ranks = pair ? wm >> 1 : wm;
+    const size_t pair_list_bytes = pair ? n_ranks * 4 : 0;
+    cur().last_pair = pair ? 1u : 0u; cur().last_fixup_launches = 0;
     WsHold ws; MZK_TRY(ws.acquire(st));
     const bool overlap = passes > 1 && std::getenv("MZK_MSM_NO_OVERLAP") == nullptr;
     const size_t nb = overlap ? (size_t)std::min(passes, SORT_SETS) : 1;
@@ -131,7 +179,7 @@
         return (uint32_t)std::min<uint64_t>(worst, (uint64_t)((double)worst * frac) + 1024);
     };
     if (defer_heavy) { h1_cap_max = h1_cap_of(sorted_max, run_cap_max, heavy_frac); desc_cap_max = desc_cap_of(sorted_max, MSM_MIN_CAP, heavy_frac); }
-    size_t desc_slot_bytes = (((size_t)sets * desc_cap_max * sizeof(LongDesc) + (size_t)sets * 4 * (1 + MSM_HEAVY_COUNTERS) + 16 + heavy_runs_bytes) + 255) & ~(size_t)255;
+    size_t desc_slot_bytes = (((size_t)sets * desc_cap_max * sizeof(LongDesc) + (size_t)msm_count_words((uint32_t)sets) * 4 + 16 + heavy_runs_bytes + pair_list_bytes) + 255) & ~(size_t)255;
     size_t parts_slot_words = (size_t)sets * desc_cap_max * EC::PT_WORDS + (size_t)sets * ((size_t)h1_cap_max + 2 * (size_t)run_cap_max) * EC::PT_WORDS;
     if (defer_heavy && (size_t)passes * parts_slot_words * 4 > ws->long_parts.cap) {
         size_t free_b = 0, total_b = 0;
@@ -140,7 +188,7 @@
             defer_heavy = false;
             h1_cap_max = h1_cap_worst;
             desc_cap_max = desc_cap_worst;
-            desc_slot_bytes = (((size_t)sets * desc_cap_max * sizeof(LongDesc) + (size_t)sets * 4 * (1 + MSM_HEAVY_COUNTERS) + 16 + heavy_runs_bytes) + 255) & ~(size_t)255;
+            desc_slot_bytes = (((size_t)sets * desc_cap_max * sizeof(LongDesc) + (size_t)msm_count_words((uint32_t)sets) * 4 + 16 + heavy_runs_bytes + pair_list_bytes) + 255) & ~(size_t)255;
             parts_slot_words = (size_t)sets * desc_cap_max * EC::PT_WORDS + (size_t)sets * ((size_t)h1_cap_max + 2 * (size_t)run_cap_max) * EC::PT_WORDS;
         }
     }
@@ -268,7 +316,8 @@
             h1_caps[p] = h1_cap;
             cur().last_cap = cap; cur().last_desc_cap = desc_cap; cur().last_h1_cap = h1_cap;
             count_ptrs[p] = desc_count;
-            HeavyRun* heavy_runs = reinterpret_cast<HeavyRun*>(desc_count + (((size_t)sets * (1 + MSM_HEAVY_COUNTERS) + 3) & ~(size_t)3));
+            HeavyRun* heavy_runs = reinterpret_cast<HeavyRun*>(desc_count + (((size_t)msm_count_words((uint32_t)sets) + 3) & ~(size_t)3));
+            uint32_t* pair_list = reinterpret_cast<uint32_t*>(ws->long_desc.as<char>() + (slot + 1) * desc_slot_bytes - pair_list_bytes);
             uint32_t* h1 = parts + (size_t)sets * desc_cap * EC::PT_WORDS;
             uint32_t* h2 = h1 + (size_t)sets * h1_cap * EC::PT_WORDS;
             uint32_t* h3 = h2 + (size_t)sets * run_cap * EC::PT_WORDS;
@@ -328,10 +377,10 @@
                 const uint32_t slice_grid = (uint32_t)std::min<uint64_t>(PRE_SLICE_CAP, records / slice + PRE_HUGE_MAX + 1);
                 const uint32_t huge_grid = (uint32_t)std::min<uint64_t>(PRE_HUGE_MAX, records / PRE_HUGE + 1);
                 hipLaunchKernelGGL(pre_bin_scan_kernel, dim3(1), dim3(1024), 0, sst, bin_total, (int)n_bins, bin_start, bin_cursor, slice, huge,
-                                   find_in_sort ? desc_count : nullptr, (uint32_t)sets * (1 + MSM_HEAVY_COUNTERS));
+                                   find_in_sort ? desc_count : nullptr, msm_count_words((uint32_t)sets));
                 hipLaunchKernelGGL(pre_coarse_scatter_kernel, coarse_grid, dim3(PRE_CTHREADS), 0, sst, dig32, n, dstride, n_dig, (int)n_bins, pb, bstride, chunk,
                                    pre.c ? pre.tab_stride : 0ull, pre.c ? items[p].base_off : 0ull, multi, bin_cursor, coarse);
-                uint32_t* keycnt_sort = diet ? cnt + 2048 : nullptr;
+                uint32_t* keycnt_sort = diet && !pair ? cnt + 2048 : nullptr;
                 hipLaunchKernelGGL(pre_fine_kernel, dim3(n_bins), dim3(1024), 0, sst, bin_start, coarse, (uint32_t)wm, pb, hist, offs, sorted, huge, M, keycnt_sort);
                 if (records > PRE_HUGE) {
                     hipLaunchKernelGGL(pre_huge_count_kernel, dim3(slice_grid), dim3(1024), 0, sst, huge, bin_start, coarse, (uint32_t)wm, pb, slice, hist);
@@ -342,15 +391,16 @@
             {
                 ProfScope ps("msm_sort", sst);
                 uint32_t* keycnt = ws->pre_cnt.as<uint32_t>() + b * cnt_words + 2048;
-                const unsigned slices = (M + MSM_ORDER_SLICE - 1) / MSM_ORDER_SLICE;
+                const unsigned slices = ((pair ? pair_half : M) + MSM_ORDER_SLICE - 1) / MSM_ORDER_SLICE;
                 if (!pre.c && !sort2) HIP_TRY(hipMemsetAsync(keycnt, 0, (size_t)sets * 1024 * 4, sst));
                 if (diet) {
+                    if (pair) hipLaunchKernelGGL(msm_order_hist_kernel, dim3(slices, sets), dim3(1024), 0, sst, hist, M, keycnt, pair_half);
                     hipLaunchKernelGGL(msm_order_place_kernel, dim3(slices, sets), dim3(1024), 0, sst, hist, offs, M, keycnt, keycnt + (size_t)sets * 1024, order,
-                                       sets, cap, desc_cap, desc, find_in_sort ? desc_count : nullptr, run_cap, h1_cap, heavy_runs, rank_global);
+                                       sets, cap, desc_cap, desc, find_in_sort ? desc_count : nullptr, run_cap, h1_cap, heavy_runs, rank_global, pair_half, pair_list);
                 } else {
-                    hipLaunchKernelGGL(msm_order_hist_kernel, dim3(slices, sets), dim3(1024), 0, sst, hist, M, keycnt);
+                    hipLaunchKernelGGL(msm_order_hist_kernel, dim3(slices, sets), dim3(1024), 0, sst, hist, M, keycnt, pair_half);
                     hipLaunchKernelGGL(msm_order_scan_kernel, dim3(rank_global ? 1 : sets), dim3(1024), 0, sst, keycnt, rank_global ? (uint32_t)sets : 0u);
-                    hipLaunchKernelGGL(msm_order_scatter_kernel, dim3(slices, sets), dim3(1024), 0, sst, hist, M, keycnt, order, rank_global);
+                    hipLaunchKernelGGL(msm_order_scatter_kernel, dim3(slices, sets), dim3(1024), 0, sst, hist, M, keycnt, order, rank_global, pair_half);
                 }
             }
             if (overlap) {
@@ -358,83 +408,76 @@
                 HIP_TRY(hipStreamWaitEvent(st, ss.ev_sorted[b], 0));
             }
             {
-                int log_split = 0;
-                const unsigned long long mean = n_sorted / M;
-                static const int max_split = std::getenv("MZK_MSM_MAX_SPLIT") ? std::atoi(std::getenv("MZK_MSM_MAX_SPLIT")) : 3;
-                const bool few_rounds = wm < (1ull << 18);
-                while (log_split < max_split) {
-                    const int nx = log_split + 1;
-                    bool stop;
-                    if (few_rounds) stop = nx < 3 ? ((wm << nx) > (1ull << 20) || (mean >> nx) < 2) : ((wm << nx) > (1ull << 18) || (mean >> 5) == 0);
-                    else stop = ((1ull << nx) - 1) * 32 > mean;
-                    if (stop) break;
-                    log_split = nx;
-                }
-                static const int force_split = std::getenv("MZK_MSM_FORCE_SPLIT") ? std::atoi(std::getenv("MZK_MSM_FORCE_SPLIT")) : -1;
-                if (force_split >= 0 && force_split <= 3) log_split = force_split;
-                static const bool no_tail = std::getenv("MZK_MSM_NO_TAIL_SPLIT") != nullptr;
-                static const bool force_tail = std::getenv("MZK_MSM_FORCE_TAIL") != nullptr;
-                static const int tail_frac_log = std::getenv("MZK_MSM_TAIL_FRAC_LOG") ? std::atoi(std::getenv("MZK_MSM_TAIL_FRAC_LOG")) : 3;
-                static const int tail_split = std::getenv("MZK_MSM_TAIL_SPLIT") ? std::atoi(std::getenv("MZK_MSM_TAIL_SPLIT")) : 2;
-                unsigned long long rank0 = 0;
-                if (sets > 1 && !no_tail && force_split < 0 && (force_tail || (!few_rounds && log_split == 1 && mean >= 8)) && tail_frac_log >= 1 && tail_frac_log <= 6 && tail_split >= 1 && tail_split <= 3) {
-                    rank0 = (wm - (wm >> tail_frac_log)) & ~(unsigned long long)(MSM_ACC_THREADS - 1);
-                    log_split = tail_split;
-                }
+                const AccSched sched = acc_sched(n_sorted);
+                const int log_split = sched.log_split;
+                const unsigned long long rank0 = sched.tail ? (n_ranks - (n_ranks >> msm_tail_frac_log())) & ~(unsigned long long)(MSM_ACC_THREADS - 1) : 0ull;
+                uint32_t* const long_count = find_in_sort ? nullptr : desc_count;
                 if (log_split == 0) {
                     ProfScope ps("msm_accumulate", st);
-                    hipLaunchKernelGGL((msm_accumulate_kernel<EC>), dim3((unsigned)((wm + MSM_ACC_THREADS - 1) / MSM_ACC_THREADS)), dim3(MSM_ACC_THREADS), 0, st,
-                                       d_bases, list_stride, offs, hist, sorted, order, M, sets, cap, find_in_sort ? nullptr : desc_count, buckets, occ);
+                    const dim3 acc_grid((unsigned)((n_ranks + MSM_ACC_THREADS - 1) / MSM_ACC_THREADS));
+                    if (pair)
+                        hipLaunchKernelGGL((msm_accumulate_kernel<EC, true>), acc_grid, dim3(MSM_ACC_THREADS), 0, st,
+                                           d_bases, list_stride, offs, hist, sorted, order, M, sets, cap, long_count, buckets, occ);
+                    else
+                        hipLaunchKernelGGL((msm_accumulate_kernel<EC, false>), acc_grid, dim3(MSM_ACC_THREADS), 0, st,
+                                           d_bases, list_stride, offs, hist, sorted, order, M, sets, cap, long_count, buckets, occ);
                 } else {
-                    const size_t n_split = (size_t)(wm - rank0), split_threads = n_split << log_split, threads = (size_t)rank0 + split_threads;
-                    MZK_TRY(ws->split.reserve(split_threads * EC::PT_WORDS * 4));
+                    const size_t n_split = (size_t)(n_ranks - rank0), split_threads = n_split << log_split, threads = (size_t)rank0 + split_threads;
+                    const size_t n_sums = pair ? 2 * n_split : n_split, partials = n_sums << log_split;
+                    MZK_TRY(ws->split.reserve(partials * EC::PT_WORDS * 4));
                     uint32_t* sub = ws->split.as<uint32_t>();
-                    const dim3 acc_grid((unsigned)((threads + MSM_ACC_THREADS - 1) / MSM_ACC_THREADS)), cmb_grid((unsigned)((split_threads + 2 * MSM_ACC_THREADS - 1) / (2 * MSM_ACC_THREADS)));
+                    const dim3 acc_grid((unsigned)((threads + MSM_ACC_THREADS - 1) / MSM_ACC_THREADS)), cmb_grid((unsigned)((partials + 2 * MSM_ACC_THREADS - 1) / (2 * MSM_ACC_THREADS)));
                     {
                         ProfScope ps("msm_accumulate", st);
-                        if (sets == 1)
-                            hipLaunchKernelGGL((msm_accumulate_split_kernel<EC, true>), acc_grid, dim3(MSM_ACC_THREADS), 0, st, d_bases, list_stride, offs, hist, sorted, order, M, sets,
-                                               cap, log_split, find_in_sort ? nullptr : desc_count, sub, rank0, buckets, occ);
-                        else
-                            hipLaunchKernelGGL((msm_accumulate_split_kernel<EC, false>), acc_grid, dim3(MSM_ACC_THREADS), 0, st, d_bases, list_stride, offs, hist, sorted, order, M, sets,
-                                               cap, log_split, find_in_sort ? nullptr : desc_count, sub, rank0, buckets, occ);
+                        auto launch_split = [&](auto kernel) {
+                            hipLaunchKernelGGL(kernel, acc_grid, dim3(MSM_ACC_THREADS), 0, st, d_bases, list_stride, offs, hist, sorted, order, M, sets,
+                                               cap, log_split, long_count, sub, rank0, buckets, occ);
+                        };
+                        if (sets == 1) { if (pair) launch_split(msm_accumulate_split_kernel<EC, true, true>); else launch_split(msm_accumulate_split_kernel<EC, true, false>); }
+                        else { if (pair) launch_split(msm_accumulate_split_kernel<EC, false, true>); else launch_split(msm_accumulate_split_kernel<EC, false, false>); }
                     }
                     ProfScope pc("msm_split_combine", st);
                     if (sets == 1)
-                        hipLaunchKernelGGL((msm_split_combine_kernel<EC, true>), cmb_grid, dim3(MSM_ACC_THREADS), 0, st, sub, (unsigned long long)n_split, log_split, order, rank0, buckets, occ);
+                        hipLaunchKernelGGL((msm_split_combine_kernel<EC, true>), cmb_grid, dim3(MSM_ACC_THREADS), 0, st, sub, (unsigned long long)n_sums, log_split, order, rank0, buckets, occ, pair_half);
                     else
-                        hipLaunchKernelGGL((msm_split_combine_kernel<EC, false>), cmb_grid, dim3(MSM_ACC_THREADS), 0, st, sub, (unsigned long long)n_split, log_split, order, rank0, buckets, occ);
+                        hipLaunchKernelGGL((msm_split_combine_kernel<EC, false>), cmb_grid, dim3(MSM_ACC_THREADS), 0, st, sub, (unsigned long long)n_sums, log_split, order, rank0, buckets, occ, pair_half);
                 }
             }
             {
                 ProfScope ps("msm_long", st);
                 if (!find_in_sort)
                     hipLaunchKernelGGL(msm_long_find_kernel, dim3((unsigned)((wm + 255) / 256)), dim3(256), 0, st, hist, offs, M, sets, cap, desc_cap, desc, desc_count,
-                                       run_cap, h1_cap, heavy_runs);
+                                       run_cap, h1_cap, heavy_runs, pair_half, pair_list);
                 HeavyJob& jb = jobs.j[defer_heavy ? p : 0];
                 jb.bases = d_bases; jb.sorted = sorted; jb.n = list_stride; jb.runs = heavy_runs; jb.count = heavy_count;
                 jb.h1 = h1; jb.h2 = h2; jb.h3 = h3; jb.buckets = buckets; jb.occ = occ; jb.run_cap = run_cap; jb.h1_cap = h1_cap; jb.M = M;
                 jb.desc = desc; jb.desc_count = desc_count; jb.parts = parts; jb.desc_cap = desc_cap;
+                jb.pair_list = pair_list; jb.pair_count = desc_count + msm_pair_counter((uint32_t)sets); jb.pair_half = pair_half;
                 heavy_run_cap_max = std::max(heavy_run_cap_max, run_cap);
                 long_desc_cap_max = std::max(long_desc_cap_max, desc_cap);
                 heavy_level_c = heavy_level_c || n_sorted > (uint64_t)MSM_HEAVY_RUN * MSM_HEAVY_FANIN;
                 if (!defer_heavy) MZK_TRY((launch_rare<EC>(jobs, 1, sets, desc_cap, run_cap, n_sorted > (uint64_t)MSM_HEAVY_RUN * MSM_HEAVY_FANIN, diet, st)));
             }
+            if (pair && !defer_heavy) launch_pair_fixup<EC>(jobs, 1, st);
             if (overlap) HIP_TRY(hipEventRecord(ss.ev_acc[b], st));
         }
         if (defer_heavy) {
             ProfScope ps("msm_long", st);
             MZK_TRY((launch_rare<EC>(jobs, (unsigned)passes, sets, long_desc_cap_max, heavy_run_cap_max, heavy_level_c, diet, st)));
         }
+        if (pair && defer_heavy) launch_pair_fixup<EC>(jobs, (unsigned)passes, st);
         {
             ProfScope ps("msm_reduce", st);
             uint32_t* buckets = ws->buckets.as<uint32_t>();
             uint8_t* occ = ws->occ.as<uint8_t>();
             const int nw_all = sets * passes;
-            int first_tail = 1;
+            const int first_lvl = pair ? 2 : 1;
+            int first_tail = first_lvl;
             while (first_tail <= log_m && (size_t)first_tail * (M >> first_tail) > 256) first_tail++;
+            cur().last_fold_launches = 0;
             static const size_t quad_max = std::getenv("MZK_MSM_QUAD_MAX") ? (size_t)std::atoll(std::getenv("MZK_MSM_QUAD_MAX")) : 65536;
-            for (int lvl = 1; lvl < first_tail; lvl++) {
+            for (int lvl = first_lvl; lvl < first_tail; lvl++) {
+                cur().last_fold_launches++;
                 const uint32_t h = M >> lvl;
                 const size_t threads = (size_t)nw_all * lvl * h;
                 static const bool fold2 = std::getenv("MZK_MSM_FOLD2") != nullptr;
diff --git a/mpc-jellyfish_amd/csrc/mzk.hip b/mpc-jellyfish_amd/csrc/mzk.hip
--- a/mpc-jellyfish_amd/csrc/mzk.hip
+++ b/mpc-jellyfish_amd/csrc/mzk.hip
@@ -1353,5 +1353,12 @@
     if (out_attempts) *out_attempts = cx_->last_attempts;
     return MZK_OK;
 }
-
-}
+int32_t mzk_msm_last_schedule(uint32_t* out_pair_mode, uint32_t* out_fold_launches, uint32_t* out_fixup_launches) {
+    ENTER_CUR();
+    if (out_pair_mode) *out_pair_mode = cx_->last_pair;
+    if (out_fold_launches) *out_fold_launches = cx_->last_fold_launches;
+    if (out_fixup_launches) *out_fixup_launches = cx_->last_fixup_launches;
+    return MZK_OK;
+}
+
+}
diff --git a/mpc-jellyfish_amd/lib.py b/mpc-jellyfish_amd/lib.py
--- a/mpc-jellyfish_amd/lib.py
+++ b/mpc-jellyfish_amd/lib.py
@@ -177,6 +177,7 @@
     "mzk_srs_precompute": [C.c_uint64, C.POINTER(C.c_uint32), C.POINTER(C.c_uint32), C.POINTER(C.c_uint64), C.POINTER(C.c_double)],
     "mzk_msm_last_shape": [C.POINTER(C.c_uint32), C.POINTER(C.c_uint32), C.POINTER(C.c_uint32)],
     "mzk_msm_last_rare": [C.POINTER(C.c_uint32), C.POINTER(C.c_uint32), C.POINTER(C.c_uint32), C.POINTER(C.c_uint32)],
+    "mzk_msm_last_schedule": [C.POINTER(C.c_uint32), C.POINTER(C.c_uint32), C.POINTER(C.c_uint32)],
     "mzk_srs_hbm_bytes": [C.c_uint64, C.POINTER(C.c_uint64), C.POINTER(C.c_uint64)],
     "mzk_plonk_pk_hbm_bytes": [C.c_uint64, C.POINTER(C.c_uint64)],
     "mzk_workspace_hbm_bytes": [C.POINTER(C.c_uint64)],
@@ -282,3 +283,10 @@
     a, b, c, d = C.c_uint32(), C.c_uint32(), C.c_uint32(), C.c_uint32()
     L.mzk_msm_last_rare(C.byref(a), C.byref(b), C.byref(c), C.byref(d))
     return a.value, b.value, c.value, d.value
+
+
+def msm_last_schedule():
+    L = load()
+    a, b, c = C.c_uint32(), C.c_uint32(), C.c_uint32()
+    L.mzk_msm_last_schedule(C.byref(a), C.byref(b), C.byref(c))
+    return a.value, b.value, c.value
```

After: 324.6 million. -3.5%, worse.
